# zenithfang/supervised_dispnet

Measured on AMD Instinct MI355X. Metric: images/sec fwd+bwd Disp_vgg_BN 128x416 b32 @1/2/4/8 GPU, higher is better.
Workload: dtype f32 (Winograd forward / input gradient / weight gradient form each f32 product from three exact bf16 pieces per operand on the bf16 matrix cores, six partial products, f32 accumulate; error vs fp64 at or below the f32 matrix instruction's)

## Files before the change

### include/dispnet_hip.h

```cpp
#ifndef DISPNET_HIP_H_
#define DISPNET_HIP_H_

#include <stddef.h>
#include <stdint.h>

#ifdef __cplusplus
extern "C" {
#endif

typedef void* dn_stream_t;

enum dn_status {
  DN_OK = 0,
  DN_ERR_BAD_ARG = -1,
  DN_ERR_UNSUPPORTED = -2,
  DN_ERR_WORKSPACE = -3,
  DN_ERR_LAUNCH = -4
};

void dn_reload_knobs(void);
int dn_version(void);
const char* dn_last_error(void);
const char* dn_last_kernel(void);
int dn_device_arch_ok(void);

#define DN_MAX_OPERANDS 3

enum dn_activation {
  DN_ACT_NONE = 0,
  DN_ACT_RELU = 1,
  DN_ACT_LEAKY = 2,
  DN_ACT_ELU = 3,
  DN_ACT_SIGMOID_AFFINE = 4
};

enum dn_conv_kind {
  DN_CONV_FWD = 0,
  DN_CONV_DGRAD = 1,
  DN_CONVT_FWD = 2,
  DN_CONVT_DGRAD = 3
};

typedef struct dn_operand {
  const float* data;
  int32_t C;
  int32_t up_shift;
  int64_t stride_n, stride_h, stride_w, stride_c;
  const float* scale;
  const float* shift;
} dn_operand;

typedef struct dn_result {
  float* data;
  int32_t C;
  int32_t accumulate;
  int64_t stride_n, stride_h, stride_w;
} dn_result;

typedef struct dn_conv_desc {
  int32_t kind;
  int32_t N;
  int32_t IH, IW;
  int32_t OH, OW;
  int32_t R, S, stride, pad;
  int32_t n_in;
  dn_operand in[DN_MAX_OPERANDS];
  int32_t n_out;
  dn_result out[DN_MAX_OPERANDS];
  const float* w_packed;
  const float* bias;
  int32_t act;
  float act_p0, act_p1;
  float* bn_partial;
  int32_t pad_mode;
  int32_t compute;
  int32_t dilation;
  const float* bnb_y;
  const float* bnb_scale;
  const float* bnb_shift;
  const float* bnb_mean;
  const float* bnb_invstd;
  float* bnb_partial;
  void* splitk_ws;
  int64_t splitk_ws_bytes;
  float* recip_out;
  const float* bnf_gamma;
  const float* bnf_beta;
  float* bnf_running_mean;
  float* bnf_running_var;
  int64_t* bnf_num_batches_tracked;
  float bnf_momentum, bnf_eps;
  float* bnf_mean;
  float* bnf_invstd;
  float* bnf_scale;
  float* bnf_shift;
  float* bnb_dgamma;
  float* bnb_dbeta;
} dn_conv_desc;

enum { DN_COMPUTE_DEFAULT = 0, DN_COMPUTE_BF16 = 1, DN_COMPUTE_F32X3 = 2, DN_COMPUTE_F32 = 3 };

int64_t dn_conv_packed_weight_elems(const dn_conv_desc* d);
int dn_conv_pack_weights(const dn_conv_desc* d, const float* w, float* w_packed, dn_stream_t stream);
int64_t dn_pack_entry_bytes(void);
int dn_pack_entry_fill(const dn_conv_desc* d, const float* w, float* w_packed, void* entry_host);
int dn_pack_many(const void* entries_dev, int32_t n_direct, int32_t n_wino, int32_t n_wino_bf16, int32_t n_wino_x3, dn_stream_t stream);
int32_t dn_conv_weight_layout(const dn_conv_desc* d);
int32_t dn_conv_bn_partial_rows(const dn_conv_desc* d);
int64_t dn_conv_splitk_workspace_bytes(const dn_conv_desc* d);
int32_t dn_conv_fwd_folds_bn_finalize(const dn_conv_desc* d);
int32_t dn_conv_dgrad_folds_bn_sums(const dn_conv_desc* d);
int32_t dn_conv_dgrad_fuses_bn_sums(const dn_conv_desc* d);
int32_t dn_conv_fwd_fuses_reciprocal(const dn_conv_desc* d);
int dn_conv2d_fwd(const dn_conv_desc* d, dn_stream_t stream);
int dn_conv2d_dgrad(const dn_conv_desc* d, dn_stream_t stream);
int dn_convT2d_fwd(const dn_conv_desc* d, dn_stream_t stream);
int dn_convT2d_dgrad(const dn_conv_desc* d, dn_stream_t stream);

size_t dn_conv_wgrad_workspace_bytes(const dn_conv_desc* fwd);
int dn_conv2d_wgrad(const dn_conv_desc* fwd, const float* dy, float* dw, void* workspace, size_t workspace_bytes,
                    dn_stream_t stream);

int dn_bn_finalize(const float* partial, int32_t rows, int32_t C, int64_t count, const float* conv_bias,
                   const float* gamma, const float* beta, float* running_mean, float* running_var, float momentum,
                   float eps, float* mean, float* invstd, float* scale, float* shift, int64_t* num_batches_tracked,
                   dn_stream_t stream);
int dn_bn_eval_affine(int32_t C, const float* gamma, const float* beta, const float* running_mean,
                      const float* running_var, float eps, float* scale, float* shift, dn_stream_t stream);
int dn_bn_relu_pool_fwd(const float* y, const float* scale, const float* shift, int32_t N, int32_t H, int32_t W,
                        int32_t C, float* pooled, uint8_t* idx, dn_stream_t stream);
int dn_bn_relu_pool_bwd(const float* dpooled, const uint8_t* idx, const float* y, const float* mean,
                        const float* invstd, int32_t N, int32_t H, int32_t W, int32_t C, float* dz, float* partial,
                        dn_stream_t stream);
int dn_maxpool2_bwd(const float* dpooled, const uint8_t* idx, int32_t N, int32_t H, int32_t W, int32_t C, float* dx, int32_t accumulate,
                    dn_stream_t stream);
int dn_bn_relu_bwd_reduce(float* da_dz, const float* y, const float* scale, const float* shift, const float* mean,
                          const float* invstd, int64_t rows, int32_t C, float* partial, dn_stream_t stream);
int dn_bn_bwd_apply(float* dz_dy, const float* y, const float* mean, const float* invstd, const float* gamma,
                    const float* partial, int32_t partial_rows, int32_t partial_stride, int32_t partial_offset, int64_t rows,
                    int32_t C, float* dgamma, float* dbeta, dn_stream_t stream);
int dn_bn_relu_bwd_sums(const float* da, const float* y, const float* scale, const float* shift, const float* mean, const float* invstd,
                        int64_t rows, int32_t C, float* partial, dn_stream_t stream);
int dn_bn_relu_pool_bwd_sums(const float* dpooled, const uint8_t* idx, const float* y, const float* mean, const float* invstd, int32_t N,
                             int32_t H, int32_t W, int32_t C, float* partial, dn_stream_t stream);
int dn_bn_bwd_apply_relu(float* da_dy, const float* y, const float* scale, const float* shift, const float* mean, const float* invstd,
                         const float* gamma, const float* partial, int32_t partial_rows, int32_t partial_stride, int32_t partial_offset,
                         int64_t rows, int32_t C, float* dgamma, float* dbeta, dn_stream_t stream);
int dn_bn_bwd_apply_pool(const float* dpooled, const uint8_t* idx, const float* y, const float* mean, const float* invstd, const float* gamma,
                         const float* partial, int32_t partial_rows, int32_t partial_stride, int32_t partial_offset, int32_t N, int32_t H,
                         int32_t W, int32_t C, float* dy, float* dgamma, float* dbeta, dn_stream_t stream);
int32_t dn_reduce_blocks(int64_t rows, int32_t C);

int dn_act_bwd_reduce_from(const float* g_in, float* g_out, const float* y_post, int32_t act, float p0, float p1, int64_t rows, int32_t C,
                           float* partial, dn_stream_t stream);
int dn_act_bwd_reduce(float* g, const float* y_post, int32_t act, float p0, float p1, int64_t rows, int32_t C,
                      float* partial, dn_stream_t stream);
int dn_colsum_finalize(const float* partial, int32_t rows, int32_t C, int32_t stride, int32_t offset, float* out,
                       dn_stream_t stream);
int dn_upsample2x_nearest_bwd(const float* dfull, int32_t N, int32_t h, int32_t w, float* dlow, int32_t accumulate,
                              dn_stream_t stream);
int dn_upsample2x_nearest_bwd_nhwc(const float* dfull, int32_t N, int32_t h, int32_t w, int32_t C, float* dlow, int32_t accumulate,
                                   dn_stream_t stream);
int dn_reflect_fold(const float* dxp, int32_t N, int32_t H, int32_t W, int32_t C, int32_t pad, float* dx, int32_t accumulate,
                    dn_stream_t stream);
int dn_bn_add_relu_fwd(const float* y, const float* scale, const float* shift, const float* r, const float* r_scale, const float* r_shift,
                       int64_t rows, int32_t C, float* out, dn_stream_t stream);
int dn_bn_add_relu_bwd(const float* gout, const float* out, const float* y, const float* mean, const float* invstd, const float* r,
                       const float* r_mean, const float* r_invstd, int64_t rows, int32_t C, float* dz_y, float* dr, int32_t dr_accumulate,
                       float* partial, dn_stream_t stream);
int32_t dn_maxpool3s2_out(int32_t H, int32_t ceil_mode);
int dn_maxpool3s2_fwd(const float* x, int32_t N, int32_t H, int32_t W, int32_t C, int32_t ceil_mode, float* out, uint8_t* idx, dn_stream_t stream);
int dn_maxpool3s2_bwd(const float* dout, const uint8_t* idx, int32_t N, int32_t H, int32_t W, int32_t C, int32_t ceil_mode, float* dx,
                      int32_t accumulate, dn_stream_t stream);
int dn_sub_div(const float* x, int64_t n, float sub, float div, float* out, dn_stream_t stream);
int dn_upsample2x_bilinear_fwd(const float* low, int32_t N, int32_t h, int32_t w, int32_t OH, int32_t OW, float* out,
                               dn_stream_t stream);
int dn_upsample2x_bilinear_bwd(const float* dout, int32_t N, int32_t h, int32_t w, int32_t OH, int32_t OW, float* dlow,
                               int32_t accumulate, dn_stream_t stream);
int32_t dn_bn_stats_rows(int64_t rows);
int dn_bn_stats_partial(const float* x, int64_t rows, int32_t C, float* partial, dn_stream_t stream);
int dn_bn_apply_fwd(const float* y, const float* scale, const float* shift, int64_t rows, int32_t C, float* out, dn_stream_t stream);
int dn_phase_bias_add(float* x, int32_t N, int32_t H2, int32_t W2, int32_t C, const float* bias4, dn_stream_t stream);
size_t dn_phase_colsum_workspace_bytes(int32_t C);
int dn_phase_colsum(const float* g, int32_t N, int32_t H, int32_t W, int32_t C, float* workspace, float* out4, dn_stream_t stream);
int dn_act_fwd(const float* x, int64_t n, int32_t act, float p0, float p1, float* out, dn_stream_t stream);
int dn_resize_bilinear_fwd(const float* in, int32_t N, int32_t IH, int32_t IW, int32_t OH, int32_t OW, int32_t align_corners, float* out,
                           dn_stream_t stream);
int dn_resize_bilinear_bwd(const float* dout, int32_t N, int32_t IH, int32_t IW, int32_t OH, int32_t OW, int32_t align_corners, float* din,
                           int32_t accumulate, dn_stream_t stream);
int dn_spatial_mean_fwd(const float* x, int32_t N, int64_t HW, int32_t C, float scale, float* out, dn_stream_t stream);
int dn_spatial_mean_bwd(const float* dout, int32_t N, int64_t HW, int32_t C, float scale, float* dx, dn_stream_t stream);
int dn_reciprocal_fwd(const float* x, float* y, int64_t n, dn_stream_t stream);
int dn_reciprocal_bwd(const float* dy, const float* y, float* dx, int64_t n, dn_stream_t stream);

enum dn_masked_loss_kind { DN_LOSS_L1 = 0, DN_LOSS_L2 = 1, DN_LOSS_BERHU = 2, DN_LOSS_SCALE_INV = 3 };
#define DN_LOSS_STATS 8
size_t dn_masked_loss_workspace_bytes(int32_t G, int64_t pixels);
int dn_masked_loss_fwd(const float* gt, const float* pred, int32_t G, int64_t pixels, float max_depth, int32_t kind, float weight,
                       int32_t accumulate, float* stats, void* workspace, size_t workspace_bytes, float* loss, dn_stream_t stream);
int dn_masked_loss_fwd_fused(const float* gt, const float* pred, int32_t G, int64_t pixels, float max_depth, int32_t kind, float weight,
                             int32_t accumulate, float* stats, void* workspace, size_t workspace_bytes, float* loss, int32_t* counter,
                             dn_stream_t stream);
int dn_masked_loss_stats(const float* gt, const float* pred, int32_t G, int64_t pixels, float max_depth, int32_t kind, int32_t pass,
                         float* stats, void* workspace, size_t workspace_bytes, dn_stream_t stream);
int dn_masked_loss_finalize(float* stats, int32_t G, int32_t kind, float weight, int32_t accumulate, float* loss, dn_stream_t stream);
int dn_masked_loss_bwd(const float* gt, const float* pred, const float* stats, const float* dloss, int32_t G, int64_t pixels,
                       float max_depth, int32_t kind, float weight, float* dpred, dn_stream_t stream);
int dn_pyramid_down2(const float* in, int32_t N, int32_t H, int32_t W, int32_t mode, float* out, dn_stream_t stream);
int dn_upsample_int_fwd(const float* low, int32_t N, int32_t h, int32_t w, int32_t scale, int32_t mode, float* out, dn_stream_t stream);
int dn_upsample_int_bwd(const float* dout, int32_t N, int32_t h, int32_t w, int32_t scale, int32_t mode, float* dlow, dn_stream_t stream);
int32_t dn_reduce1d_blocks(int64_t n);
int dn_explainability_fwd(const float* mask, int64_t n, float weight, int32_t accumulate, float* partial, float* loss, dn_stream_t stream);
int dn_explainability_bwd(const float* mask, const float* dloss, int64_t n, float* dmask, dn_stream_t stream);
int32_t dn_smooth_blocks(int32_t B, int32_t H, int32_t W);
int dn_smooth2_fwd(const float* map, int32_t B, int32_t H, int32_t W, float weight, float* partial, float* loss,
                   dn_stream_t stream);
int dn_smooth2_bwd(const float* map, const float* dloss, int32_t B, int32_t H, int32_t W, float weight, float* dmap,
                   dn_stream_t stream);
int dn_compute_errors(const float* gt, const float* pred, int32_t B, int32_t H, int32_t W, float max_depth, int32_t y1,
                      int32_t y2, int32_t x1, int32_t x2, int32_t median_scaling, float* scratch, float* out8,
                      dn_stream_t stream);

int dn_pose_proj_fwd(const float* pose, int64_t pose_stride_b, const float* K, const float* Kinv, int32_t B, int32_t rotation_mode,
                     float downscale, float* proj, float* kinv_scaled, dn_stream_t stream);
int32_t dn_warp_blocks(int32_t h, int32_t w);
int dn_pose_proj_bwd(const float* pose, int64_t pose_stride_b, const float* K, int32_t B, int32_t rotation_mode, float downscale,
                     const float* dproj_partial, int32_t nblk, float* dpose, int64_t dpose_stride_b, int32_t accumulate,
                     dn_stream_t stream);
int dn_inverse_warp_fwd(const float* img, const float* depth, const float* proj, const float* kinv, int32_t B, int32_t h, int32_t w,
                        int32_t padding_mode, int32_t align_corners, float* warped, dn_stream_t stream);
// ... 108 lines not shown
```

### supervised_dispnet_amd/_lib.py

```python
import ctypes as C
import os
import pathlib

_PKG = pathlib.Path(__file__).resolve().parent
LIB_PATH = pathlib.Path(os.environ.get("DISPNET_HIP_LIB", _PKG / "libdispnet_hip.so"))

EXPECTED_ABI = 21

DN_MAX_OPERANDS = 3
ACT_NONE, ACT_RELU, ACT_LEAKY, ACT_ELU, ACT_SIGMOID_AFFINE = 0, 1, 2, 3, 4
COMPUTE_DEFAULT, COMPUTE_BF16, COMPUTE_F32X3, COMPUTE_F32 = 0, 1, 2, 3
CONV_FWD, CONV_DGRAD, CONVT_FWD, CONVT_DGRAD = 0, 1, 2, 3
LOSS_L1, LOSS_L2, LOSS_BERHU, LOSS_SCALE_INV = 0, 1, 2, 3
LOSS_STATS = 8

_f32p = C.c_void_p


class Operand(C.Structure):
    _fields_ = [("data", _f32p), ("C", C.c_int32), ("up_shift", C.c_int32),
                ("stride_n", C.c_int64), ("stride_h", C.c_int64), ("stride_w", C.c_int64), ("stride_c", C.c_int64),
                ("scale", _f32p), ("shift", _f32p)]


class Result(C.Structure):
    _fields_ = [("data", _f32p), ("C", C.c_int32), ("accumulate", C.c_int32),
                ("stride_n", C.c_int64), ("stride_h", C.c_int64), ("stride_w", C.c_int64)]


class ConvDesc(C.Structure):
    _fields_ = [("kind", C.c_int32), ("N", C.c_int32), ("IH", C.c_int32), ("IW", C.c_int32), ("OH", C.c_int32),
                ("OW", C.c_int32), ("R", C.c_int32), ("S", C.c_int32), ("stride", C.c_int32), ("pad", C.c_int32),
                ("n_in", C.c_int32), ("in_", Operand * DN_MAX_OPERANDS),
                ("n_out", C.c_int32), ("out", Result * DN_MAX_OPERANDS),
                ("w_packed", _f32p), ("bias", _f32p), ("act", C.c_int32), ("act_p0", C.c_float), ("act_p1", C.c_float),
                ("bn_partial", _f32p), ("pad_mode", C.c_int32), ("compute", C.c_int32), ("dilation", C.c_int32),
                ("bnb_y", _f32p), ("bnb_scale", _f32p), ("bnb_shift", _f32p), ("bnb_mean", _f32p), ("bnb_invstd", _f32p), ("bnb_partial", _f32p),
                ("splitk_ws", _f32p), ("splitk_ws_bytes", C.c_int64), ("recip_out", _f32p),
                ("bnf_gamma", _f32p), ("bnf_beta", _f32p), ("bnf_running_mean", _f32p), ("bnf_running_var", _f32p),
                ("bnf_num_batches_tracked", C.c_void_p), ("bnf_momentum", C.c_float), ("bnf_eps", C.c_float),
                ("bnf_mean", _f32p), ("bnf_invstd", _f32p), ("bnf_scale", _f32p), ("bnf_shift", _f32p),
                ("bnb_dgamma", _f32p), ("bnb_dbeta", _f32p)]


_P = C.POINTER
_i32, _i64, _f, _d, _vp, _sz = C.c_int32, C.c_int64, C.c_float, C.c_double, C.c_void_p, C.c_size_t

SIGNATURES = {
    "dn_version": (C.c_int, []),
    "dn_reload_knobs": (None, []),
    "dn_last_error": (C.c_char_p, []),
    "dn_last_kernel": (C.c_char_p, []),
    "dn_device_arch_ok": (C.c_int, []),
    "dn_conv_packed_weight_elems": (_i64, [_P(ConvDesc)]),
    "dn_conv_pack_weights": (C.c_int, [_P(ConvDesc), _vp, _vp, _vp]),
    "dn_pack_entry_bytes": (_i64, []),
    "dn_pack_entry_fill": (C.c_int, [_P(ConvDesc), _vp, _vp, _vp]),
    "dn_pack_many": (C.c_int, [_vp, _i32, _i32, _i32, _i32, _vp]),
    "dn_conv_weight_layout": (_i32, [_P(ConvDesc)]),
    "dn_conv_bn_partial_rows": (_i32, [_P(ConvDesc)]),
    "dn_conv_dgrad_fuses_bn_sums": (_i32, [_P(ConvDesc)]),
    "dn_conv_fwd_fuses_reciprocal": (_i32, [_P(ConvDesc)]),
    "dn_conv_splitk_workspace_bytes": (_i64, [_P(ConvDesc)]),
    "dn_conv_fwd_folds_bn_finalize": (_i32, [_P(ConvDesc)]),
    "dn_conv_dgrad_folds_bn_sums": (_i32, [_P(ConvDesc)]),
    "dn_conv2d_fwd": (C.c_int, [_P(ConvDesc), _vp]),
    "dn_conv2d_dgrad": (C.c_int, [_P(ConvDesc), _vp]),
    "dn_convT2d_fwd": (C.c_int, [_P(ConvDesc), _vp]),
    "dn_convT2d_dgrad": (C.c_int, [_P(ConvDesc), _vp]),
    "dn_conv_wgrad_workspace_bytes": (_sz, [_P(ConvDesc)]),
    "dn_conv2d_wgrad": (C.c_int, [_P(ConvDesc), _vp, _vp, _vp, _sz, _vp]),
    "dn_bn_finalize": (C.c_int, [_vp, _i32, _i32, _i64, _vp, _vp, _vp, _vp, _vp, _f, _f, _vp, _vp, _vp, _vp, _vp, _vp]),
    "dn_bn_eval_affine": (C.c_int, [_i32, _vp, _vp, _vp, _vp, _f, _vp, _vp, _vp]),
    "dn_bn_relu_pool_fwd": (C.c_int, [_vp, _vp, _vp, _i32, _i32, _i32, _i32, _vp, _vp, _vp]),
    "dn_bn_relu_bwd_sums": (C.c_int, [_vp, _vp, _vp, _vp, _vp, _vp, _i64, _i32, _vp, _vp]),
    "dn_bn_relu_pool_bwd_sums": (C.c_int, [_vp, _vp, _vp, _vp, _vp, _i32, _i32, _i32, _i32, _vp, _vp]),
    "dn_bn_bwd_apply_relu": (C.c_int, [_vp, _vp, _vp, _vp, _vp, _vp, _vp, _vp, _i32, _i32, _i32, _i64, _i32, _vp, _vp, _vp]),
    "dn_bn_bwd_apply_pool": (C.c_int, [_vp, _vp, _vp, _vp, _vp, _vp, _vp, _i32, _i32, _i32, _i32, _i32, _i32, _i32, _vp, _vp, _vp, _vp]),
    "dn_maxpool2_bwd": (C.c_int, [_vp, _vp, _i32, _i32, _i32, _i32, _vp, _i32, _vp]),
    "dn_bn_relu_pool_bwd": (C.c_int, [_vp, _vp, _vp, _vp, _vp, _i32, _i32, _i32, _i32, _vp, _vp, _vp]),
    "dn_bn_relu_bwd_reduce": (C.c_int, [_vp, _vp, _vp, _vp, _vp, _vp, _i64, _i32, _vp, _vp]),
    "dn_bn_bwd_apply": (C.c_int, [_vp, _vp, _vp, _vp, _vp, _vp, _i32, _i32, _i32, _i64, _i32, _vp, _vp, _vp]),
    "dn_reduce_blocks": (_i32, [_i64, _i32]),
    "dn_act_bwd_reduce": (C.c_int, [_vp, _vp, _i32, _f, _f, _i64, _i32, _vp, _vp]),
    "dn_act_bwd_reduce_from": (C.c_int, [_vp, _vp, _vp, _i32, _f, _f, _i64, _i32, _vp, _vp]),
    "dn_colsum_finalize": (C.c_int, [_vp, _i32, _i32, _i32, _i32, _vp, _vp]),
    "dn_upsample2x_nearest_bwd": (C.c_int, [_vp, _i32, _i32, _i32, _vp, _i32, _vp]),
    "dn_upsample2x_nearest_bwd_nhwc": (C.c_int, [_vp, _i32, _i32, _i32, _i32, _vp, _i32, _vp]),
    "dn_reflect_fold": (C.c_int, [_vp, _i32, _i32, _i32, _i32, _i32, _vp, _i32, _vp]),
    "dn_bn_add_relu_fwd": (C.c_int, [_vp, _vp, _vp, _vp, _vp, _vp, _i64, _i32, _vp, _vp]),
    "dn_bn_add_relu_bwd": (C.c_int, [_vp, _vp, _vp, _vp, _vp, _vp, _vp, _vp, _i64, _i32, _vp, _vp, _i32, _vp, _vp]),
    "dn_maxpool3s2_out": (_i32, [_i32, _i32]),
    "dn_maxpool3s2_fwd": (C.c_int, [_vp, _i32, _i32, _i32, _i32, _i32, _vp, _vp, _vp]),
    "dn_maxpool3s2_bwd": (C.c_int, [_vp, _vp, _i32, _i32, _i32, _i32, _i32, _vp, _i32, _vp]),
    "dn_bn_stats_rows": (_i32, [_i64]),
    "dn_bn_stats_partial": (C.c_int, [_vp, _i64, _i32, _vp, _vp]),
    "dn_bn_apply_fwd": (C.c_int, [_vp, _vp, _vp, _i64, _i32, _vp, _vp]),
    "dn_act_fwd": (C.c_int, [_vp, _i64, _i32, _f, _f, _vp, _vp]),
    "dn_phase_bias_add": (C.c_int, [_vp, _i32, _i32, _i32, _i32, _vp, _vp]),
    "dn_phase_colsum_workspace_bytes": (_sz, [_i32]),
    "dn_phase_colsum": (C.c_int, [_vp, _i32, _i32, _i32, _i32, _vp, _vp, _vp]),
    "dn_resize_bilinear_fwd": (C.c_int, [_vp, _i32, _i32, _i32, _i32, _i32, _i32, _vp, _vp]),
    "dn_resize_bilinear_bwd": (C.c_int, [_vp, _i32, _i32, _i32, _i32, _i32, _i32, _vp, _i32, _vp]),
    "dn_sub_div": (C.c_int, [_vp, _i64, _f, _f, _vp, _vp]),
    "dn_spatial_mean_fwd": (C.c_int, [_vp, _i32, _i64, _i32, _f, _vp, _vp]),
    "dn_spatial_mean_bwd": (C.c_int, [_vp, _i32, _i64, _i32, _f, _vp, _vp]),
    "dn_upsample2x_bilinear_fwd": (C.c_int, [_vp, _i32, _i32, _i32, _i32, _i32, _vp, _vp]),
    "dn_upsample2x_bilinear_bwd": (C.c_int, [_vp, _i32, _i32, _i32, _i32, _i32, _vp, _i32, _vp]),
    "dn_reciprocal_fwd": (C.c_int, [_vp, _vp, _i64, _vp]),
    "dn_reciprocal_bwd": (C.c_int, [_vp, _vp, _vp, _i64, _vp]),
    "dn_masked_loss_workspace_bytes": (_sz, [_i32, _i64]),
    "dn_masked_loss_fwd": (C.c_int, [_vp, _vp, _i32, _i64, _f, _i32, _f, _i32, _vp, _vp, _sz, _vp, _vp]),
    "dn_masked_loss_fwd_fused": (C.c_int, [_vp, _vp, _i32, _i64, _f, _i32, _f, _i32, _vp, _vp, _sz, _vp, _vp, _vp]),
    "dn_masked_loss_stats": (C.c_int, [_vp, _vp, _i32, _i64, _f, _i32, _i32, _vp, _vp, _sz, _vp]),
    "dn_masked_loss_finalize": (C.c_int, [_vp, _i32, _i32, _f, _i32, _vp, _vp]),
    "dn_masked_loss_bwd": (C.c_int, [_vp, _vp, _vp, _vp, _i32, _i64, _f, _i32, _f, _vp, _vp]),
    "dn_pyramid_down2": (C.c_int, [_vp, _i32, _i32, _i32, _i32, _vp, _vp]),
    "dn_upsample_int_fwd": (C.c_int, [_vp, _i32, _i32, _i32, _i32, _i32, _vp, _vp]),
    "dn_upsample_int_bwd": (C.c_int, [_vp, _i32, _i32, _i32, _i32, _i32, _vp, _vp]),
    "dn_reduce1d_blocks": (_i32, [_i64]),
    "dn_explainability_fwd": (C.c_int, [_vp, _i64, _f, _i32, _vp, _vp, _vp]),
    "dn_explainability_bwd": (C.c_int, [_vp, _vp, _i64, _vp, _vp]),
    "dn_smooth_blocks": (_i32, [_i32, _i32, _i32]),
    "dn_smooth2_fwd": (C.c_int, [_vp, _i32, _i32, _i32, _f, _vp, _vp, _vp]),
    "dn_smooth2_bwd": (C.c_int, [_vp, _vp, _i32, _i32, _i32, _f, _vp, _vp]),
    "dn_compute_errors": (C.c_int, [_vp, _vp, _i32, _i32, _i32, _f, _i32, _i32, _i32, _i32, _i32, _vp, _vp, _vp]),
    "dn_pose_proj_fwd": (C.c_int, [_vp, _i64, _vp, _vp, _i32, _i32, _f, _vp, _vp, _vp]),
    "dn_warp_blocks": (_i32, [_i32, _i32]),
    "dn_pose_proj_bwd": (C.c_int, [_vp, _i64, _vp, _i32, _i32, _f, _vp, _i32, _vp, _i64, _i32, _vp]),
    "dn_inverse_warp_fwd": (C.c_int, [_vp, _vp, _vp, _vp, _i32, _i32, _i32, _i32, _i32, _vp, _vp]),
    "dn_inverse_warp_bwd": (C.c_int, [_vp, _vp, _vp, _vp, _i32, _i32, _i32, _i32, _i32, _vp, _vp, _i32, _vp, _vp]),
    "dn_photometric_fwd": (C.c_int, [_vp, _vp, _vp, _vp, _vp, _vp, _i64, _i32, _i32, _i32, _i32, _i32, _f, _i32, _vp, _vp, _vp]),
    "dn_photometric_bwd": (C.c_int, [_vp, _vp, _vp, _vp, _vp, _vp, _i64, _i32, _i32, _i32, _i32, _i32, _f, _vp, _vp, _i32, _vp, _vp,
                                     _i64, _vp]),
    "dn_area_down": (C.c_int, [_vp, _i64, _i32, _i32, _i32, _vp, _vp]),
    "dn_ssim_fwd": (C.c_int, [_vp, _vp, _i64, _i32, _i32, _vp, _vp]),
    "dn_ssim_bwd": (C.c_int, [_vp, _vp, _vp, _i64, _i32, _i32, _vp, _vp, _vp, _vp]),
    "dn_edge_smooth_blocks": (_i32, [_i32, _i32, _i32]),
    "dn_edge_smooth_fwd": (C.c_int, [_vp, _vp, _i32, _i32, _i32, _i32, _vp, _vp, _vp]),
    "dn_edge_smooth_bwd": (C.c_int, [_vp, _vp, _vp, _i32, _i32, _i32, _i32, _vp, _vp]),
    "dn_ordinal_fwd": (C.c_int, [_vp, _i64, _i64, _i64, _i32, _i64, _i32, _vp, _vp, _vp]),
    "dn_ordinal_bwd": (C.c_int, [_vp, _i64, _i64, _i64, _vp, _vp, _i32, _i64, _i32, _vp, _vp]),
    "dn_ordinal_loss_blocks": (_i32, [_i32, _i64]),
    "dn_ordinal_loss_fwd": (C.c_int, [_vp, _vp, _vp, _i32, _i64, _i32, _f, _vp, _vp, _vp, _vp]),
    "dn_ordinal_loss_finalize": (C.c_int, [_vp, _vp, _vp]),
    "dn_ordinal_loss_bwd": (C.c_int, [_vp, _vp, _vp, _vp, _vp, _i32, _i64, _i32, _f, _f, _vp, _vp]),
    "dn_ord_head_supported": (_i32, [_i32, _i64, _i32]),
    "dn_ord_head_bwd_blocks": (_i32, [_i32, _i64]),
    "dn_ord_head_fwd": (C.c_int, [_vp, _vp, _vp, _vp, _i32, _i64, _i32, _vp, _vp, _vp]),
    "dn_ord_head_bwd": (C.c_int, [_vp, _vp, _vp, _vp, _vp, _i32, _i64, _i32, _vp, _i32, _vp, _vp, _vp, _vp]),
    "dn_sid_labels": (C.c_int, [_vp, _i64, _f, _f, _vp, _vp]),
    "dn_sid_depth": (C.c_int, [_vp, _i64, _f, _f, _vp, _vp]),
    "dn_channel_scale": (C.c_int, [_vp, _vp, _i32, _i64, _i32, _vp, _vp]),
    "dn_adam_step": (C.c_int, [_vp, _vp, _vp, _vp, _i64, _d, _d, _d, _d, _d, _i32, _d, _vp]),
    "dn_adam_step_dev": (C.c_int, [_vp, _vp, _vp, _vp, _i64, _vp, _d, _d, _vp, _vp, _d, _vp]),
    "dn_adam_tick": (C.c_int, [_vp, _vp, _vp, _vp]),
    "dn_fill": (C.c_int, [_vp, _f, _i64, _vp]),
    "dn_copy": (C.c_int, [_vp, _vp, _i64, _vp]),
    "dn_tape_begin": (_vp, []),
    "dn_tape_end": (C.c_int, [_vp]),
# ... 89 lines not shown
```

### supervised_dispnet_amd/csrc/dn_conv.hip

```cpp
#include <stdlib.h>

#include "dn_internal.h"

namespace dn {

template <auto Launch> static int plan_only(const dn_conv_desc*, IgemmParams& p, hipStream_t s) { return Launch(p, s); }
template <auto Launch> static int with_desc(const dn_conv_desc* d, IgemmParams& p, hipStream_t s) { return Launch(d, p, s); }
static bool heads_off() { return knobs().no_direct; }
constexpr auto x3_upper = conv_x3_splitk_workspace_upper_bytes;
static const ConvFamily kConvFamilies[] = {
    {"head_fwd", head_fwd_eligible, heads_off, plan_only<launch_head_fwd>, nullptr, x3_upper, head_fwd_fuses_reciprocal},
    {"head_dgrad", head_dgrad_eligible, heads_off, plan_only<launch_head_dgrad>, nullptr, x3_upper},
    {"winograd", wino_eligible, nullptr, plan_only<launch_wino_conv>, wino_layout,
     [](const IgemmParams& p) { return wino_layout(p) == 3 ? wino_splitk_workspace_bytes(p) : (size_t)0; }, nullptr,
     [](const dn_conv_desc* d) {
       const dn_result& r = d->out[0];
       return d->kind == DN_CONV_DGRAD && d->n_out == 1 && !r.accumulate && (r.C & 3) == 0 && r.stride_w == r.C &&
              r.stride_h == (int64_t)d->OW * r.C && r.stride_n == (int64_t)d->OH * d->OW * r.C && d->bias == nullptr && d->act == DN_ACT_NONE;
     },
     [](IgemmParams& p) { wino_prepare(p); return wino_folds_bn_finalize(p); }, [](IgemmParams& p) { wino_prepare(p); return wino_folds_bn_sums(p); }},
    {"stem3", stem3_conv_eligible, nullptr, plan_only<launch_stem3_conv>, nullptr, x3_upper},
    {"stemk", stemk_conv_eligible, nullptr, with_desc<launch_stemk_conv>, nullptr, x3_upper},
    {"stem", stem_eligible, nullptr, plan_only<launch_stem>, nullptr, x3_upper},
    {"lds3", lds3_conv_eligible, nullptr, with_desc<launch_lds3_conv>, nullptr, x3_upper},
// ... 8 lines not shown
  return f;
}

static int run_conv(const dn_conv_desc* d, int expect_kind, dn_stream_t stream) {
  DN_REQUIRE(d != nullptr && d->kind == expect_kind, DN_ERR_BAD_ARG, "descriptor kind mismatch (want %d)", expect_kind);
  IgemmParams p;
  int rc = build_plan(d, false, &p);
  if (rc != DN_OK) return rc;
  DN_REQUIRE(p.w != nullptr, DN_ERR_BAD_ARG, "w_packed is null");
  for (int i = 0; i < p.n_in; ++i) DN_REQUIRE(p.in[i].p != nullptr, DN_ERR_BAD_ARG, "operand %d has no data", i);
  for (int i = 0; i < p.n_out; ++i) {
    const dn_result& o = d->out[i];
    DN_REQUIRE(o.stride_h == (int64_t)d->OW * o.stride_w && o.stride_n == (int64_t)d->OH * o.stride_h, DN_ERR_UNSUPPORTED,
               "result %d must be pixel-dense (NHWC with a channel stride)", i);
  }
  return conv_route(d, p)->launch(d, p, as_stream(stream));
}

}

using namespace dn;

static bool wgrad_split_plans(const dn_conv_desc* fwd, dn_conv_desc* d1, dn_conv_desc* d2, IgemmParams* p1, IgemmParams* p2, size_t* w1,
                              size_t* w2) {
  if (fwd->kind != DN_CONV_FWD || fwd->n_in < 2 || fwd->in[fwd->n_in - 1].C != 1) return false;
  *d1 = *fwd;
  d1->n_in = fwd->n_in - 1;
  *d2 = *fwd;
  d2->n_in = 1;
  d2->in[0] = fwd->in[fwd->n_in - 1];
  if (build_plan(d1, true, p1) != DN_OK || build_plan(d2, true, p2) != DN_OK) return false;
  int cin_total = 0;
  for (int i = 0; i < fwd->n_in; ++i) cin_total += fwd->in[i].C;
  if (wino_wgrad_eligible(d1, *p1)) {
    p1->dw_cin_total = cin_total;
    *w1 = (wino_wgrad_workspace_bytes(*p1) + 255) / 256 * 256;
  } else {
    return false;
  }
  p2->in[0].ch_off = cin_total - 1;
  p2->D1 = cin_total;
  choose_splits(p2);
  *w2 = generic_wgrad_workspace_bytes(*p2);
  return true;
}

static int tap_windows(const IgemmParams& p) {
  const int nt = p.ph[0].ntaps;
  if (nt <= 32 || p.reflect || p.nphases != 1 || knobs().no_tap_windows) return 1;
  return (nt + 31) / 32;
}

static void tap_window_plan(const IgemmParams& full, int w, int nw, IgemmParams* q) {
  *q = full;
  const int nt = full.ph[0].ntaps, per = (nt + nw - 1) / nw;
  const int t0 = w * per, t1 = t0 + per < nt ? t0 + per : nt;
  for (int t = t0; t < t1; ++t) {
    q->tdy[t - t0] = full.tdy[full.ph[0].tap0 + t];
    q->tdx[t - t0] = full.tdx[full.ph[0].tap0 + t];
    q->tr[t - t0] = full.tr[full.ph[0].tap0 + t];
    q->ts[t - t0] = full.ts[full.ph[0].tap0 + t];
  }
  q->ph[0].tap0 = 0;
  q->ph[0].ntaps = t1 - t0;
  int nch = 0;
  for (int i = 0; i < q->n_in; ++i) nch += (q->ph[0].ntaps * q->in[i].C + kChunk - 1) / kChunk;
  q->ph[0].nchunks = nch;
  q->uni32 = 1;
  q->wg_uniform = 1;
  for (int i = 0; i < q->n_in; ++i) {
    const KOperand& o = q->in[i];
    if (!o.small) q->uni32 = 0;
    if (!o.small || (!o.vec && o.scale != nullptr) || o.C >= 32768) q->wg_uniform = 0;
  }
}

struct WgradFamily {
  const char* name;
  bool (*eligible)(const dn_conv_desc* fwd, const IgemmParams& p);
  size_t (*workspace_bytes)(const dn_conv_desc* fwd, const IgemmParams& p);
  bool dy_aligned16;
  bool (*switched_off)();
  int (*launch)(const dn_conv_desc* fwd, IgemmParams& p, float* dw, hipStream_t s);
};
static const WgradFamily kWgradFamilies[] = {
    {"head", head_wgrad_eligible, [](const dn_conv_desc*, const IgemmParams& p) { return head_wgrad_workspace_bytes(p); }, false,
     [] { return knobs().no_direct; },
     [](const dn_conv_desc*, IgemmParams& p, float* dw, hipStream_t s) { return launch_head_wgrad(p, dw, p.ws, s); }},
    {"winograd", wino_wgrad_eligible, [](const dn_conv_desc*, const IgemmParams& p) { return wino_wgrad_workspace_bytes(p); }, false, nullptr,
     [](const dn_conv_desc*, IgemmParams& p, float* dw, hipStream_t s) { return launch_wino_wgrad(p, dw, s); }},
    {"lds3", lds3_wgrad_eligible, [](const dn_conv_desc*, const IgemmParams& p) { return lds3_wgrad_workspace_bytes(p); }, true, nullptr,
     launch_lds3_wgrad},
    {"lds3k", lds3k_wgrad_eligible, [](const dn_conv_desc*, const IgemmParams& p) { return lds3k_wgrad_workspace_bytes(p); }, true, nullptr,
     launch_lds3k_wgrad},
    {"stemk", stemk_wgrad_eligible, stemk_wgrad_workspace_bytes, true, nullptr, launch_stemk_wgrad},
    {"thin", thin_wgrad_eligible, [](const dn_conv_desc*, const IgemmParams& p) { return thin_wgrad_workspace_bytes(p); }, false, nullptr,
     [](const dn_conv_desc*, IgemmParams& p, float* dw, hipStream_t s) { return launch_thin_wgrad(p, dw, s); }},
};

extern "C" {

int64_t dn_pack_entry_bytes(void) { return (int64_t)sizeof(PackEntry); }

int dn_pack_entry_fill(const dn_conv_desc* d, const float* w, float* w_packed, void* entry_host) {
  DN_REQUIRE(d && w && w_packed && entry_host, DN_ERR_BAD_ARG, "dn_pack_entry_fill: null pointer");
  PackEntry* e = reinterpret_cast<PackEntry*>(entry_host);
  int rc = build_plan(d, false, &e->p);
  if (rc != DN_OK) return rc;
  e->w = w;
  e->wp = w_packed;
  const ConvFamily* f = conv_route(d, e->p);
  e->wino = f->weight_layout ? f->weight_layout(e->p) : 0;
  if (e->wino) {
    e->total = wino_packed_elems(e->p);
    e->NS = ((e->p.Ntot + 63) / 64 * 64) / 32;
  } else {
    e->total = direct_packed_elems(e->p);
    e->NS = 0;
  }
  return e->wino;
}

int dn_pack_many(const void* entries_dev, int32_t n_direct, int32_t n_wino, int32_t n_wino16, int32_t n_wino_x3, dn_stream_t stream) {
  DN_REQUIRE(entries_dev && n_direct >= 0 && n_wino >= 0 && n_wino16 >= 0 && n_wino_x3 >= 0, DN_ERR_BAD_ARG, "dn_pack_many: bad argument");
  const PackEntry* tab = reinterpret_cast<const PackEntry*>(entries_dev);
  hipStream_t s = as_stream(stream);
  if (n_direct > 0) {
    int rc = launch_direct_pack_many(tab, n_direct, s);
    if (rc != DN_OK) return rc;
  }
  if (n_wino > 0) {
    int rc = launch_wino_pack_many(tab, n_direct, n_wino, s);
    if (rc != DN_OK) return rc;
  }
  if (n_wino16 > 0) {
    int rc = launch_wino_pack16_many(tab, n_direct + n_wino, n_wino16, 1, s);
    if (rc != DN_OK) return rc;
  }
  if (n_wino_x3 > 0) return launch_wino_pack16_many(tab, n_direct + n_wino + n_wino16, n_wino_x3, 3, s);
  return DN_OK;
}

int dn_conv_pack_weights(const dn_conv_desc* d, const float* w, float* w_packed, dn_stream_t stream) {
  IgemmParams p;
  int rc = build_plan(d, false, &p);
  if (rc != DN_OK) return rc;
  DN_REQUIRE(w != nullptr && w_packed != nullptr, DN_ERR_BAD_ARG, "null weight pointer");
  const ConvFamily* f = conv_route(d, p);
  if (const int wl = f->weight_layout ? f->weight_layout(p) : 0)
    return wl == 1 ? launch_wino_pack(p, w, w_packed, as_stream(stream)) : launch_wino_pack16(p, w, w_packed, wl == 3 ? 3 : 1, as_stream(stream));
  return launch_direct_pack(p, w, w_packed, as_stream(stream));
}

int dn_conv2d_fwd(const dn_conv_desc* d, dn_stream_t stream) { return run_conv(d, DN_CONV_FWD, stream); }
int dn_conv2d_dgrad(const dn_conv_desc* d, dn_stream_t stream) { return run_conv(d, DN_CONV_DGRAD, stream); }
int dn_convT2d_fwd(const dn_conv_desc* d, dn_stream_t stream) { return run_conv(d, DN_CONVT_FWD, stream); }
int dn_convT2d_dgrad(const dn_conv_desc* d, dn_stream_t stream) { return run_conv(d, DN_CONVT_DGRAD, stream); }

size_t dn_conv_wgrad_workspace_bytes(const dn_conv_desc* fwd) {
  IgemmParams p;
  if (build_plan(fwd, true, &p) != DN_OK) return 0;
  choose_splits(&p);
  size_t need = generic_wgrad_workspace_bytes(p);
  for (const WgradFamily& f : kWgradFamilies)
    if (f.eligible(fwd, p) && f.workspace_bytes(fwd, p) > need) need = f.workspace_bytes(fwd, p);
  {
    dn_conv_desc d1, d2;
    IgemmParams p1, p2;
    size_t w1 = 0, w2 = 0;
    if (wgrad_split_plans(fwd, &d1, &d2, &p1, &p2, &w1, &w2) && w1 + w2 > need) need = w1 + w2;
  }
  const int nw = tap_windows(p);
  for (int w = 0; w < nw && nw > 1; ++w) {
    IgemmParams q;
    tap_window_plan(p, w, nw, &q);
    choose_splits(&q);
    if (generic_wgrad_workspace_bytes(q) > need) need = generic_wgrad_workspace_bytes(q);
  }
  return need;
}

int dn_conv2d_wgrad(const dn_conv_desc* fwd, const float* dy, float* dw, void* workspace, size_t workspace_bytes,
                    dn_stream_t stream) {
  IgemmParams p;
  int rc = build_plan(fwd, true, &p);
  if (rc != DN_OK) return rc;
  DN_REQUIRE(dy != nullptr && dw != nullptr && workspace != nullptr, DN_ERR_BAD_ARG, "null pointer");
  const hipStream_t s = as_stream(stream);
  for (const WgradFamily& f : kWgradFamilies) {
    if (!f.eligible(fwd, p) || (f.switched_off && f.switched_off()) || workspace_bytes < f.workspace_bytes(fwd, p)) continue;
    if (f.dy_aligned16 && (reinterpret_cast<uintptr_t>(dy) & 15) != 0) continue;
    for (int i = 0; i < p.n_in; ++i) DN_REQUIRE(p.in[i].p != nullptr, DN_ERR_BAD_ARG, "operand %d has no data", i);
    p.g = dy;
    p.ws = reinterpret_cast<float*>(workspace);
    return f.launch(fwd, p, dw, s);
  }
  {
    dn_conv_desc d1, d2;
    IgemmParams p1, p2;
    size_t w1 = 0, w2 = 0;
    if (wgrad_split_plans(fwd, &d1, &d2, &p1, &p2, &w1, &w2) && workspace_bytes >= w1 + w2) {
      for (int i = 0; i < fwd->n_in; ++i) DN_REQUIRE(fwd->in[i].data != nullptr, DN_ERR_BAD_ARG, "operand %d has no data", i);
      if (wino_wgrad_eligible(&d1, p1)) {
        p1.g = dy;
        p1.ws = reinterpret_cast<float*>(workspace);
        rc = launch_wino_wgrad(p1, dw, s);
      } else {
        rc = generic_wgrad(&d1, p1, dy, dw, workspace, w1, s);
      }
      if (rc != DN_OK) return rc;
      return generic_wgrad(&d2, p2, dy, dw, reinterpret_cast<char*>(workspace) + w1, w2, s);
    }
  }
  if (const int nw = tap_windows(p); nw > 1 && fwd->kind == DN_CONV_FWD) {
    for (int w = 0; w < nw; ++w) {
      IgemmParams q;
      tap_window_plan(p, w, nw, &q);
      rc = generic_wgrad(fwd, q, dy, dw, workspace, workspace_bytes, s);
      if (rc != DN_OK) return rc;
    }
    return DN_OK;
  }
  return generic_wgrad(fwd, p, dy, dw, workspace, workspace_bytes, s);
}

}
```

### supervised_dispnet_amd/csrc/dn_internal.h

```cpp
#pragma once
#include <hip/hip_runtime.h>
#include <hip/hip_ext.h>
#include <stdint.h>
#include <stdio.h>

#include <atomic>
#include <functional>
#include <tuple>
#include <type_traits>

#include "dispnet_hip.h"

namespace dn {

void set_error(const char* fmt, ...);
void set_last_kernel(const char* fmt, ...);
int check_launch(const char* what);

static inline hipStream_t as_stream(dn_stream_t s) { return reinterpret_cast<hipStream_t>(s); }

struct LaunchTape;
extern std::atomic<LaunchTape*> g_tape_rec;
void tape_push(LaunchTape* t, std::function<void(hipEvent_t)>&& op, const void* kernel, hipStream_t stream);

template <typename... KArgs, typename... Args>
static inline void launch(void (*kernel)(KArgs...), dim3 grid, dim3 block, size_t lds, hipStream_t stream, Args... args) {
  kernel<<<grid, block, lds, stream>>>(args...);
  if (LaunchTape* t = g_tape_rec.load(std::memory_order_relaxed)) {
    std::tuple<std::decay_t<KArgs>...> held(args...);
    tape_push(t, [=](hipEvent_t stop) mutable {
      if (stop == nullptr) {
        std::apply([&](auto&... a) { kernel<<<grid, block, lds, stream>>>(a...); }, held);
      } else {
        std::apply([&](auto&... a) {
          void* argv[] = {static_cast<void*>(&a)...};
          if (hipExtLaunchKernel(reinterpret_cast<const void*>(kernel), grid, block, argv, lds, stream, nullptr, stop, 0) != hipSuccess) {
            (void)hipGetLastError();
            kernel<<<grid, block, lds, stream>>>(a...);
            (void)hipEventRecord(stop, stream);
          }
        }, held);
      }
    }, reinterpret_cast<const void*>(kernel), stream);
  }
}
#define DN_LAUNCH(...) ::dn::launch(__VA_ARGS__)

struct Knobs {
  bool no_winograd, no_winograd_wgrad;
  bool no_direct;
  bool no_thin, no_thin_conv;
  bool no_lds3;
  bool no_wino_splitk, no_x3_splitk, no_wino8_tail;
  bool no_x3_direct, no_x3_wgrad;
  bool no_tap_windows;
  int wino_wgw;
  int wino_min_tiles;
  int wino_splitk_target, wino_splitk_maxblocks;
  int pack_blocks;
  bool no_riding_fences;
  int wino_nmajor;
  int wino_wg_target;
  int wino8;
};
const Knobs& knobs();

inline int norm_compute(int c) {
  return c == DN_COMPUTE_BF16 ? DN_COMPUTE_BF16 : ((c == DN_COMPUTE_F32X3 || c == DN_COMPUTE_DEFAULT) ? DN_COMPUTE_F32X3 : DN_COMPUTE_F32);
}

#define DN_REQUIRE(cond, code, ...)      \
  do {                                   \
    if (!(cond)) {                       \
      ::dn::set_error(__VA_ARGS__);      \
      return (code);                     \
    }                                    \
  } while (0)

constexpr int kMaxTaps = 64;
constexpr int kMaxPhases = 4;
constexpr int kChunk = 32;

struct KOperand {
  const float* p;
  const float* scale;
  const float* shift;
  long long sn, sh, sw, sc;
  int C;
  int up;
  int vec;
  int ch_off;
  unsigned mC;
  int small;
};

struct KResult {
  float* p;
  long long sn, sh, sw;
  int C;
  int n_begin;
  int accumulate;
  int linear;
};

struct KPhase {
  int ntaps;
  int tap0;
  int ooy, oox;
  int nchunks;
  long long w_off;
};

struct BnFinalizeArgs {
  const float* conv_bias;
  const float* gamma;
  const float* beta;
  float* running_mean;
  float* running_var;
  long long* num_batches_tracked;
  float momentum, eps;
  float* mean;
  float* invstd;
  float* scale;
  float* shift;
};

struct IgemmParams {
  KOperand in[DN_MAX_OPERANDS];
  KResult out[DN_MAX_OPERANDS];
  KPhase ph[kMaxPhases];
  int8_t tdy[kMaxTaps], tdx[kMaxTaps], tr[kMaxTaps], ts[kMaxTaps];
  int n_in, n_out, nphases;
  int N, GH, GW, M;
  int sy, sx;
  int osy, osx;
  int IH, IW, OH, OW;
  int Ntot, Npad;
  int BN;
// ... 31 lines not shown
  int* fold_cnt;
  int fold_bn, fold_bnb;
  int nmajor;
};

static inline unsigned fastdiv_magic(unsigned d) { return d <= 1 ? 0xFFFFFFFFu : (unsigned)(0x100000000ull / d); }

int build_plan(const dn_conv_desc* d, bool for_wgrad, IgemmParams* p);

inline long long direct_packed_elems(const IgemmParams& p) {
  const KPhase& last = p.ph[p.nphases - 1];
  return last.w_off + (long long)p.Npad * last.nchunks * kChunk;
}

struct PackEntry {
  IgemmParams p;
  const float* w;
  float* wp;
  long long total;
  int wino;
  int NS;
};
int launch_wino_pack_many(const PackEntry* tab_dev, int first, int n, hipStream_t stream);
int launch_wino_pack16_many(const PackEntry* tab_dev, int first, int n, int pieces, hipStream_t stream);
int launch_wino_pack16(const IgemmParams& p, const float* w, float* wp, int pieces, hipStream_t stream);
long long wino_packed_floats(const IgemmParams& p, int layout);
int wino_layout(const IgemmParams& p);

struct ConvFamily {
  const char* name;
  bool (*eligible)(const dn_conv_desc* d, const IgemmParams& p);
  bool (*switched_off)();
  int (*launch)(const dn_conv_desc* d, IgemmParams& p, hipStream_t s);
  int (*weight_layout)(const IgemmParams& p);
  size_t (*splitk_workspace_bytes)(const IgemmParams& p);
  bool (*fuses_reciprocal)(const IgemmParams& p);
  bool (*takes_bn_sums)(const dn_conv_desc* d);
  bool (*folds_bn_finalize)(IgemmParams& p);
  bool (*folds_bn_sums)(IgemmParams& p);
};
const ConvFamily* conv_route(const dn_conv_desc* d, const IgemmParams& p);

bool stem_eligible(const dn_conv_desc* d, const IgemmParams& p);
int launch_stem(const IgemmParams& p, hipStream_t stream);
int launch_tiled_conv(const IgemmParams& p, hipStream_t stream);
void choose_splits(IgemmParams* p);
size_t generic_wgrad_workspace_bytes(const IgemmParams& p);
int generic_wgrad(const dn_conv_desc* fwd, IgemmParams& p, const float* dy, float* dw, void* workspace, size_t workspace_bytes, hipStream_t s);
int launch_direct_pack(const IgemmParams& p, const float* w, float* wp, hipStream_t stream);
int launch_direct_pack_many(const PackEntry* tab_dev, int n, hipStream_t stream);

bool head_fwd_eligible(const dn_conv_desc* d, const IgemmParams& p);
int launch_head_fwd(const IgemmParams& p, hipStream_t stream);
bool head_fwd_fuses_reciprocal(const IgemmParams& p);
bool head_dgrad_eligible(const dn_conv_desc* d, const IgemmParams& p);
int launch_head_dgrad(const IgemmParams& p, hipStream_t stream);
bool head_wgrad_eligible(const dn_conv_desc* fwd, const IgemmParams& p);
size_t head_wgrad_workspace_bytes(const IgemmParams& p);
int launch_head_wgrad(const IgemmParams& p, float* dw, float* workspace, hipStream_t stream);

bool wino_eligible(const dn_conv_desc* d, const IgemmParams& p);
long long wino_packed_elems(const IgemmParams& p);
int launch_wino_pack(const IgemmParams& p, const float* w, float* wp, hipStream_t stream);
int launch_wino_conv(IgemmParams& p, hipStream_t stream);
void wino_prepare(IgemmParams& p);
bool wino_folds_bn_finalize(const IgemmParams& p);
bool wino_folds_bn_sums(const IgemmParams& p);
int wino_splitk_choice(const IgemmParams& p);
size_t conv_x3_splitk_workspace_upper_bytes(const IgemmParams& p);
size_t wino_splitk_workspace_bytes(const IgemmParams& p);
bool wino_wgrad_eligible(const dn_conv_desc* fwd, const IgemmParams& p);
size_t wino_wgrad_workspace_bytes(const IgemmParams& p);
int launch_wino_wgrad(IgemmParams& p, float* dw, hipStream_t stream);

bool thin_wgrad_eligible(const dn_conv_desc* fwd, const IgemmParams& p);
size_t thin_wgrad_workspace_bytes(const IgemmParams& p);
int launch_thin_wgrad(IgemmParams& p, float* dw, hipStream_t stream);
bool thin_conv_eligible(const dn_conv_desc* d, const IgemmParams& p);
int launch_thin_conv(const IgemmParams& p, hipStream_t stream);

bool lds3_conv_eligible(const dn_conv_desc* d, const IgemmParams& p);
int launch_lds3_conv(const dn_conv_desc* d, const IgemmParams& p, hipStream_t stream);
bool lds3_wgrad_eligible(const dn_conv_desc* fwd, const IgemmParams& p);
size_t lds3_wgrad_workspace_bytes(const IgemmParams& p);
int launch_lds3_wgrad(const dn_conv_desc* fwd, IgemmParams& p, float* dw, hipStream_t stream);
bool lds3k_wgrad_eligible(const dn_conv_desc* fwd, const IgemmParams& p);
size_t lds3k_wgrad_workspace_bytes(const IgemmParams& p);
int launch_lds3k_wgrad(const dn_conv_desc* fwd, IgemmParams& p, float* dw, hipStream_t stream);
int launch_wgrad_reduce(const IgemmParams& p, float* dw, hipStream_t stream);
bool wgrad_x3_eligible(const IgemmParams& p);
int launch_wgrad_x3(const IgemmParams& p, hipStream_t stream);
bool lds3k_conv_eligible(const dn_conv_desc* d, const IgemmParams& p);
int launch_lds3k_conv(const dn_conv_desc* d, const IgemmParams& p, hipStream_t stream);
bool stem3_conv_eligible(const dn_conv_desc* d, const IgemmParams& p);
bool stemk_conv_eligible(const dn_conv_desc* d, const IgemmParams& p);
int launch_stemk_conv(const dn_conv_desc* d, const IgemmParams& p, hipStream_t stream);
bool stemk_wgrad_eligible(const dn_conv_desc* d, const IgemmParams& p);
size_t stemk_wgrad_workspace_bytes(const dn_conv_desc* d, const IgemmParams& p);
int launch_stemk_wgrad(const dn_conv_desc* d, IgemmParams& p, float* dw, hipStream_t stream);
int launch_stem3_conv(const IgemmParams& p, hipStream_t stream);

}
```

### supervised_dispnet_amd/csrc/dn_lds3_wgrad.hip

```cpp
#include <stdlib.h>

#include "dn_device.h"

namespace dn {

struct WgGeo {
  int tilesX, tilesY, ntiles, per_xcd;
  long long slab;
};

constexpr int WG_TH = 8, WG_TW = 32;
constexpr int WG_GSTR = 528;
constexpr int WG_GPIECE = 16 * WG_GSTR;
constexpr int WG_XROWB = 96;
constexpr int WG_XSTR = 10 * WG_XROWB + 16;
constexpr int WG_XPIECE = 16 * WG_XSTR;
constexpr int WG_DCOLS = 36;
constexpr int WG16_LDS = 3 * WG_GPIECE + 3 * WG_XPIECE + 10 * WG_DCOLS * 4;

template <bool HAS1>
__global__ void __launch_bounds__(256, 2) lds3_wgrad16_kernel(const IgemmParams p, const WgGeo geo) {
  extern __shared__ __align__(16) char lds[];
  char* Gp = lds;
  char* Xp = lds + 3 * WG_GPIECE;
  float* Dp = reinterpret_cast<float*>(lds + 3 * WG_GPIECE + 3 * WG_XPIECE);
  constexpr int NT = HAS1 ? 10 : 9;
  const int tid = threadIdx.x, lane = tid & 63, wave = tid >> 6;
  const int j = lane & 15, g = lane >> 4;
  const KOperand& S = p.in[0];
  const __amdgpu_buffer_rsrc_t rg = __builtin_amdgcn_make_buffer_rsrc(const_cast<float*>(p.g), 0, 0x80000000u, 0x00020000);
  const __amdgpu_buffer_rsrc_t rx = __builtin_amdgcn_make_buffer_rsrc(const_cast<float*>(S.p), 0, 0x80000000u, 0x00020000);
  __amdgpu_buffer_rsrc_t r1 = rx;
  if constexpr (HAS1) r1 = __builtin_amdgcn_make_buffer_rsrc(const_cast<float*>(p.in[1].p), 0, 0x80000000u, 0x00020000);

  f32x4 acc[NT];
#pragma unroll
  for (int t = 0; t < NT; ++t) acc[t] = f32x4{0.f, 0.f, 0.f, 0.f};
  const int dtap = j < 9 ? j : 0;
  const int doff = (dtap / 3) * WG_DCOLS + (dtap % 3);

  f32x4 vg[8], vx[8];
  float dv[2] = {0.f, 0.f};
  auto issue_loads = [&](int t) __attribute__((always_inline)) {
    const int txb = t % geo.tilesX, q1 = t / geo.tilesX;
    const int tyb = q1 % geo.tilesY, n = q1 / geo.tilesY;
    const int gy0 = tyb * WG_TH, gx0 = txb * WG_TW;
    {
      const int cq = tid & 3, pxg = tid >> 2, row = pxg >> 2, cgp = pxg & 3;
      const int gy = gy0 + row;
#pragma unroll
      for (int i = 0; i < 8; ++i) {
        const int gx = gx0 + 8 * cgp + i;
        const bool ok = tid < 128 && gy < p.GH && gx < p.GW;
        const int off = (((n * p.GH + gy) * p.GW + gx) * p.Ntot + 4 * cq) * 4;
        vg[i] = __builtin_bit_cast(f32x4, __builtin_amdgcn_raw_buffer_load_b128(rg, ok ? off : -1, 0, 0));
      }
    }
    {
      const int cq = tid & 3, grp = tid >> 2, row = grp / 6, cgp = grp - row * 6;
      const int iy = gy0 - 1 + row;
#pragma unroll
      for (int i = 0; i < 8; ++i) {
        const int ix = gx0 + 8 * cgp - 8 + i;
        const bool need = cgp == 0 ? i == 7 : (cgp == 5 ? i == 0 : true);
        const bool ok = tid < 240 && need && (unsigned)iy < (unsigned)p.IH && (unsigned)ix < (unsigned)p.IW;
        const int off = (n * (int)S.sn + iy * (int)S.sh + ix * (int)S.sw + 4 * cq) * 4;
        vx[i] = __builtin_bit_cast(f32x4, __builtin_amdgcn_raw_buffer_load_b128(rx, ok ? off : -1, 0, 0));
      }
    }
    if constexpr (HAS1) {
      const KOperand& S1 = p.in[1];
#pragma unroll
      for (int r = 0; r < 2; ++r) {
        const int it = tid + 256 * r;
        const int row = it / 34, col = it - row * 34;
        const int iy = gy0 - 1 + row, ix = gx0 - 1 + col;
        const bool ok = it < 340 && (unsigned)iy < (unsigned)p.IH && (unsigned)ix < (unsigned)p.IW;
        const int off = (n * (int)S1.sn + (iy >> S1.up) * (int)S1.sh + (ix >> S1.up) * (int)S1.sw) * 4;
        dv[r] = __builtin_bit_cast(float, __builtin_amdgcn_raw_buffer_load_b32(r1, ok ? off : -1, 0, 0));
      }
    }
  };
  auto store_lds = [&]() __attribute__((always_inline)) {
    if (tid < 128) {
      const int cq = tid & 3, pxg = tid >> 2;
// ... 29 lines not shown
        if (it < 340) Dp[row * WG_DCOLS + col] = dv[r];
      }
    }
  };

  const int xcd = (int)blockIdx.x & 7, local = (int)blockIdx.x >> 3, nlocal = (int)gridDim.x >> 3;
  const int band_lo = xcd * geo.per_xcd, band_hi = min(band_lo + geo.per_xcd, geo.ntiles);
  constexpr int AS[6] = {0, 0, 1, 0, 1, 2}, BS[6] = {2, 1, 1, 0, 0, 0};
  if (band_lo + local < band_hi) issue_loads(band_lo + local);
  for (int t = band_lo + local; t < band_hi; t += nlocal) {
    store_lds();
    __syncthreads();
    if (t + nlocal < band_hi) issue_loads(t + nlocal);
#pragma unroll 1
    for (int rr = 0; rr < 2; ++rr) {
      const int r = 2 * wave + rr;
      bf16x8 a[3];
#pragma unroll
      for (int P = 0; P < 3; ++P) a[P] = *reinterpret_cast<const bf16x8*>(Gp + P * WG_GPIECE + j * WG_GSTR + (r * 32 + 8 * g) * 2);
#pragma unroll
      for (int ty = 0; ty < 3; ++ty) {
        const char* rowb = Xp + j * WG_XSTR + (r + ty) * WG_XROWB + (8 * g + 8) * 2;
        u32x4 c[3];
        unsigned lf[3], rt[3];
#pragma unroll
        for (int P = 0; P < 3; ++P) {
          c[P] = *reinterpret_cast<const u32x4*>(rowb + P * WG_XPIECE);
          lf[P] = *reinterpret_cast<const unsigned*>(rowb + P * WG_XPIECE - 4);
          rt[P] = *reinterpret_cast<const unsigned*>(rowb + P * WG_XPIECE + 16);
        }
        bf16x8 bm[3], bz[3], bp[3];
#pragma unroll
        for (int P = 0; P < 3; ++P) {
          const u32x4 m4 = u32x4{__builtin_amdgcn_alignbit(c[P][0], lf[P], 16), __builtin_amdgcn_alignbit(c[P][1], c[P][0], 16),
                                 __builtin_amdgcn_alignbit(c[P][2], c[P][1], 16), __builtin_amdgcn_alignbit(c[P][3], c[P][2], 16)};
          const u32x4 p4 = u32x4{__builtin_amdgcn_alignbit(c[P][1], c[P][0], 16), __builtin_amdgcn_alignbit(c[P][2], c[P][1], 16),
                                 __builtin_amdgcn_alignbit(c[P][3], c[P][2], 16), __builtin_amdgcn_alignbit(rt[P], c[P][3], 16)};
          bm[P] = __builtin_bit_cast(bf16x8, m4);
          bz[P] = __builtin_bit_cast(bf16x8, c[P]);
          bp[P] = __builtin_bit_cast(bf16x8, p4);
        }
#pragma unroll
        for (int q = 0; q < 6; ++q) {
          acc[3 * ty + 0] = __builtin_amdgcn_mfma_f32_16x16x32_bf16(a[AS[q]], bm[BS[q]], acc[3 * ty + 0], 0, 0, 0);
          acc[3 * ty + 1] = __builtin_amdgcn_mfma_f32_16x16x32_bf16(a[AS[q]], bz[BS[q]], acc[3 * ty + 1], 0, 0, 0);
          acc[3 * ty + 2] = __builtin_amdgcn_mfma_f32_16x16x32_bf16(a[AS[q]], bp[BS[q]], acc[3 * ty + 2], 0, 0, 0);
        }
      }
      if constexpr (HAS1) {
        float v[8];
#pragma unroll
        for (int e = 0; e < 8; ++e) {
          const float x = Dp[r * WG_DCOLS + 8 * g + e + doff];
          v[e] = j < 9 ? x : 0.f;
        }
        bf16x8 b[3];
        split3(v, b[0], b[1], b[2]);
#pragma unroll
        for (int q = 0; q < 6; ++q) acc[9] = __builtin_amdgcn_mfma_f32_16x16x32_bf16(a[AS[q]], b[BS[q]], acc[9], 0, 0, 0);
      }
    }
    __syncthreads();
  }

  f32x4* red = reinterpret_cast<f32x4*>(lds);
#pragma unroll
  for (int t = 0; t < NT; ++t) red[(wave * NT + t) * 64 + lane] = acc[t];
  __syncthreads();
  const int Kp = p.ph[0].nchunks * kChunk;
  const int kbase1 = ((9 * 16 + kChunk - 1) / kChunk) * kChunk;
  float* slab = p.ws + (long long)blockIdx.x * geo.slab;
  for (int it = tid; it < NT * 64; it += 256) {
    const int t = it >> 6, l = it & 63;
    const f32x4 s = (red[(0 * NT + t) * 64 + l] + red[(1 * NT + t) * 64 + l]) + (red[(2 * NT + t) * 64 + l] + red[(3 * NT + t) * 64 + l]);
    const int jj = l & 15, gg = l >> 4;
    const int k = t < 9 ? t * 16 + jj : kbase1 + jj;
    if (t < 9 || jj < 9) {
#pragma unroll
      for (int e = 0; e < 4; ++e) slab[(long long)(4 * gg + e) * Kp + k] = s[e];
    }
  }
}

constexpr int WS_GSTR = 272;
constexpr int WS_GPIECE = 64 * WS_GSTR;
constexpr int WS_ICOLS = 36;
constexpr int WS_IPLANE = 10 * WS_ICOLS;
constexpr int WGS_LDS = 3 * WS_GPIECE + 3 * WS_IPLANE * 4;

__global__ void __launch_bounds__(256, 2) lds3_wgrad_stem_kernel(const IgemmParams p, const WgGeo geo) {
  extern __shared__ __align__(16) char lds[];
  char* Gp = lds;
  float* Ip = reinterpret_cast<float*>(lds + 3 * WS_GPIECE);
  const int tid = threadIdx.x, lane = tid & 63, wave = tid >> 6;
  const int j = lane & 15, g = lane >> 4;
  const KOperand& S = p.in[0];
  const int C = S.C, K = 9 * C;
  const __amdgpu_buffer_rsrc_t rg = __builtin_amdgcn_make_buffer_rsrc(const_cast<float*>(p.g), 0, 0x80000000u, 0x00020000);
  const __amdgpu_buffer_rsrc_t rx = __builtin_amdgcn_make_buffer_rsrc(const_cast<float*>(S.p), 0, 0x80000000u, 0x00020000);

  f32x4 acc[4][2];
#pragma unroll
  for (int m = 0; m < 4; ++m)
#pragma unroll
    for (int nt = 0; nt < 2; ++nt) acc[m][nt] = f32x4{0.f, 0.f, 0.f, 0.f};
  int ioff[2];
  bool ilive[2];
#pragma unroll
  for (int nt = 0; nt < 2; ++nt) {
    const int col = 16 * nt + j;
    ilive[nt] = col < K;
    const int tap = ilive[nt] ? col / C : 0, ci = ilive[nt] ? col - tap * C : 0;
    ioff[nt] = ci * WS_IPLANE + (tap / 3) * WS_ICOLS + (tap % 3);
  }

  f32x4 vg[8];
  float vi[4];
  auto issue_g = [&](int t, int h) __attribute__((always_inline)) {
    const int txb = t % geo.tilesX, q1 = t / geo.tilesX;
    const int tyb = q1 % geo.tilesY, n = q1 / geo.tilesY;
    const int pxg = tid & 15, cq = tid >> 4, row = pxg >> 2, cgp = pxg & 3;
    const int gy = tyb * WG_TH + 4 * h + row;
#pragma unroll
    for (int i = 0; i < 8; ++i) {
      const int gx = txb * WG_TW + 8 * cgp + i;
      const bool ok = gy < p.GH && gx < p.GW;
      const int off = (((n * p.GH + gy) * p.GW + gx) * p.Ntot + 4 * cq) * 4;
      vg[i] = __builtin_bit_cast(f32x4, __builtin_amdgcn_raw_buffer_load_b128(rg, ok ? off : -1, 0, 0));
    }
  };
  auto issue_img = [&](int t) __attribute__((always_inline)) {
    const int txb = t % geo.tilesX, q1 = t / geo.tilesX;
    const int tyb = q1 % geo.tilesY, n = q1 / geo.tilesY;
#pragma unroll
    for (int r = 0; r < 4; ++r) {
      const int it = tid + 256 * r;
      const int c = it / 340, px = it - c * 340;
      const int row = px / 34, col = px - row * 34;
      const int iy = tyb * WG_TH - 1 + row, ix = txb * WG_TW - 1 + col;
      const bool ok = c < C && (unsigned)iy < (unsigned)p.IH && (unsigned)ix < (unsigned)p.IW;
      const int off = (n * (int)S.sn + iy * (int)S.sh + ix * (int)S.sw + c * (int)S.sc) * 4;
      vi[r] = __builtin_bit_cast(float, __builtin_amdgcn_raw_buffer_load_b32(rx, ok ? off : -1, 0, 0));
    }
  };
  auto store_g = [&]() __attribute__((always_inline)) {
    const int pxg = tid & 15, cq = tid >> 4;
#pragma unroll
    for (int e = 0; e < 4; ++e) {
      const float v[8] = {vg[0][e], vg[1][e], vg[2][e], vg[3][e], vg[4][e], vg[5][e], vg[6][e], vg[7][e]};
      bf16x8 h, m, l;
      split3(v, h, m, l);
      char* dst = Gp + (4 * cq + e) * WS_GSTR + pxg * 16;
      *reinterpret_cast<bf16x8*>(dst) = h;
      *reinterpret_cast<bf16x8*>(dst + WS_GPIECE) = m;
      *reinterpret_cast<bf16x8*>(dst + 2 * WS_GPIECE) = l;
    }
  };
  auto store_img = [&]() __attribute__((always_inline)) {
#pragma unroll
    for (int r = 0; r < 4; ++r) {
      const int it = tid + 256 * r;
      const int c = it / 340, px = it - c * 340;
      const int row = px / 34, col = px - row * 34;
      if (c < 3) Ip[c * WS_IPLANE + row * WS_ICOLS + col] = vi[r];
    }
  };

  const int xcd = (int)blockIdx.x & 7, local = (int)blockIdx.x >> 3, nlocal = (int)gridDim.x >> 3;
  const int band_lo = xcd * geo.per_xcd, band_hi = min(band_lo + geo.per_xcd, geo.ntiles);
  constexpr int AS[6] = {0, 0, 1, 0, 1, 2}, BS[6] = {2, 1, 1, 0, 0, 0};
  if (band_lo + local < band_hi) {
    issue_g(band_lo + local, 0);
    issue_img(band_lo + local);
  }
  for (int t = band_lo + local; t < band_hi; t += nlocal) {
#pragma unroll 1
    for (int h = 0; h < 2; ++h) {
      store_g();
      if (h == 0) store_img();
      __syncthreads();
      if (h == 0) issue_g(t, 1);
      else if (t + nlocal < band_hi) {
        issue_g(t + nlocal, 0);
        issue_img(t + nlocal);
      }
      const int r = 4 * h + wave;
      bf16x8 b[2][3];
#pragma unroll
      for (int nt = 0; nt < 2; ++nt) {
        float v[8];
#pragma unroll
        for (int e = 0; e < 8; ++e) {
          const float x = Ip[r * WS_ICOLS + 8 * g + e + ioff[nt]];
          v[e] = ilive[nt] ? x : 0.f;
        }
        split3(v, b[nt][0], b[nt][1], b[nt][2]);
      }
#pragma unroll
      for (int m = 0; m < 4; ++m) {
        bf16x8 a[3];
#pragma unroll
        for (int P = 0; P < 3; ++P) a[P] = *reinterpret_cast<const bf16x8*>(Gp + P * WS_GPIECE + (16 * m + j) * WS_GSTR + (wave * 32 + 8 * g) * 2);
#pragma unroll
        for (int q = 0; q < 6; ++q)
#pragma unroll
          for (int nt = 0; nt < 2; ++nt) acc[m][nt] = __builtin_amdgcn_mfma_f32_16x16x32_bf16(a[AS[q]], b[nt][BS[q]], acc[m][nt], 0, 0, 0);
      }
      __syncthreads();
    }
  }

  f32x4* red = reinterpret_cast<f32x4*>(lds);
#pragma unroll
  for (int m = 0; m < 4; ++m)
#pragma unroll
    for (int nt = 0; nt < 2; ++nt) red[((wave * 4 + m) * 2 + nt) * 64 + lane] = acc[m][nt];
  __syncthreads();
  const int Kp = p.ph[0].nchunks * kChunk;
  float* slab = p.ws + (long long)blockIdx.x * geo.slab;
  for (int it = tid; it < 8 * 64; it += 256) {
    const int mn = it >> 6, l = it & 63, m = mn >> 1, nt = mn & 1;
    const f32x4 s = (red[((0 * 4 + m) * 2 + nt) * 64 + l] + red[((1 * 4 + m) * 2 + nt) * 64 + l]) +
                    (red[((2 * 4 + m) * 2 + nt) * 64 + l] + red[((3 * 4 + m) * 2 + nt) * 64 + l]);
    const int jj = l & 15, gg = l >> 4, k = 16 * nt + jj;
    if (k < K) {
#pragma unroll
      for (int e = 0; e < 4; ++e) slab[(long long)(16 * m + 4 * gg + e) * Kp + k] = s[e];
    }
  }
}

static int lds3_wgrad_form(const dn_conv_desc* d, const IgemmParams& p) {
  if (knobs().no_lds3 || norm_compute(d->compute) != DN_COMPUTE_F32X3) return 0;
  if (d->kind != DN_CONV_FWD || d->R != 3 || d->S != 3 || d->stride != 1 || d->pad != 1 || d->pad_mode != 0 || d->dilation > 1) return 0;
  if (d->IH != d->OH || d->IW != d->OW) return 0;
  if ((long long)p.M * p.Ntot * 4 + 64 >= (1ll << 31) || (reinterpret_cast<uintptr_t>(p.g) & 15)) return 0;
  for (int t = 0; t < 9; ++t)
    if (p.tdy[t] != t / 3 - 1 || p.tdx[t] != t % 3 - 1) return 0;
  const KOperand& a = p.in[0];
  if (!a.small || a.scale != nullptr || a.up != 0) return 0;
  if (p.Ntot == 16 && a.C == 16 && a.vec) {
    if (p.n_in == 1) return 1;
    const KOperand& b = p.in[1];
    if (p.n_in == 2 && b.C == 1 && b.small && b.scale == nullptr) return 2;
    return 0;
  }
  if (p.Ntot == 64 && p.n_in == 1 && a.C >= 1 && a.C <= 3) return 3;
  return 0;
}

static int lds3_wgrad_blocks(const IgemmParams& p) {
  const int ntiles = p.N * ((p.GH + WG_TH - 1) / WG_TH) * ((p.GW + WG_TW - 1) / WG_TW);
  int blocks = ntiles < 512 ? ntiles : 512;
  return (blocks + 7) / 8 * 8;
}

bool lds3_wgrad_eligible(const dn_conv_desc* d, const IgemmParams& p) { return lds3_wgrad_form(d, p) != 0; }

size_t lds3_wgrad_workspace_bytes(const IgemmParams& p) {
  return (size_t)lds3_wgrad_blocks(p) * p.Npad * p.ph[0].nchunks * kChunk * sizeof(float);
}

int launch_lds3_wgrad(const dn_conv_desc* d, IgemmParams& p, float* dw, hipStream_t stream) {
  const int form = lds3_wgrad_form(d, p);
  WgGeo geo;
  geo.tilesX = (p.GW + WG_TW - 1) / WG_TW;
  geo.tilesY = (p.GH + WG_TH - 1) / WG_TH;
  geo.ntiles = p.N * geo.tilesX * geo.tilesY;
  geo.per_xcd = (geo.ntiles + 7) / 8;
  geo.slab = (long long)p.Npad * p.ph[0].nchunks * kChunk;
  const int blocks = lds3_wgrad_blocks(p);
  hipError_t e = hipSuccess;
  if (form == 3) {
    e = hipFuncSetAttribute(reinterpret_cast<const void*>(lds3_wgrad_stem_kernel), hipFuncAttributeMaxDynamicSharedMemorySize, WGS_LDS);
    if (e == hipSuccess) DN_LAUNCH(lds3_wgrad_stem_kernel, dim3(blocks), dim3(256), (size_t)WGS_LDS, stream, p, geo);
    set_last_kernel("dn::lds3_wgrad_stem_kernel");
  } else if (form == 2) {
    e = hipFuncSetAttribute(reinterpret_cast<const void*>(lds3_wgrad16_kernel<true>), hipFuncAttributeMaxDynamicSharedMemorySize, WG16_LDS);
    if (e == hipSuccess) DN_LAUNCH(lds3_wgrad16_kernel<true>, dim3(blocks), dim3(256), (size_t)WG16_LDS, stream, p, geo);
    set_last_kernel("dn::lds3_wgrad16_kernel<true>");
  } else if (form == 1) {
    e = hipFuncSetAttribute(reinterpret_cast<const void*>(lds3_wgrad16_kernel<false>), hipFuncAttributeMaxDynamicSharedMemorySize, WG16_LDS);
    if (e == hipSuccess) DN_LAUNCH(lds3_wgrad16_kernel<false>, dim3(blocks), dim3(256), (size_t)WG16_LDS, stream, p, geo);
    set_last_kernel("dn::lds3_wgrad16_kernel<false>");
  } else {
    set_error("launch_lds3_wgrad: no form");
    return DN_ERR_UNSUPPORTED;
  }
  if (e != hipSuccess) {
    set_error("lds3 wgrad: hipFuncSetAttribute: %s", hipGetErrorString(e));
    return DN_ERR_LAUNCH;
  }
  int rc = check_launch("lds3_wgrad_kernel");
  if (rc != DN_OK) return rc;
  p.splits = blocks;
  return launch_wgrad_reduce(p, dw, stream);
}

}

namespace dn {

constexpr int WK_TH = 2;
constexpr int WK_GSTR = WK_TH * 32 * 2 + 16;
constexpr int WK_GPIECE = 32 * WK_GSTR;
constexpr int WK_XROWS = WK_TH + 2;
constexpr int WK_XSTR = WK_XROWS * WG_XROWB + 16;
constexpr int WK_NCI = 96;
constexpr int WK_XPIECE = WK_NCI * WK_XSTR;
constexpr int WK_LDS = 3 * WK_GPIECE + 3 * WK_XPIECE + WK_XROWS * WG_DCOLS * 4;

template <bool HAS1>
__global__ void __launch_bounds__(512, 2) lds3k_wgrad_kernel(const IgemmParams p, const WgGeo geo, int c0) {
  extern __shared__ __align__(16) char lds[];
  char* Gp = lds;
  char* Xp = lds + 3 * WK_GPIECE;
  float* Dp = reinterpret_cast<float*>(lds + 3 * WK_GPIECE + 3 * WK_XPIECE);
  const int tid = threadIdx.x, lane = tid & 63, wave = tid >> 6;
  const int j = lane & 15, g = lane >> 4;
  const KOperand& S0 = p.in[0];
  const bool two = p.n_in - (HAS1 ? 1 : 0) == 2;
  const KOperand& S1 = p.in[two ? 1 : 0];
  const __amdgpu_buffer_rsrc_t rg = __builtin_amdgcn_make_buffer_rsrc(const_cast<float*>(p.g), 0, 0x80000000u, 0x00020000);
  const __amdgpu_buffer_rsrc_t r0 = __builtin_amdgcn_make_buffer_rsrc(const_cast<float*>(S0.p), 0, 0x80000000u, 0x00020000);
  const __amdgpu_buffer_rsrc_t r1 = __builtin_amdgcn_make_buffer_rsrc(const_cast<float*>(S1.p), 0, 0x80000000u, 0x00020000);
  const KOperand& SD = p.in[HAS1 ? p.n_in - 1 : 0];
  const __amdgpu_buffer_rsrc_t rd = __builtin_amdgcn_make_buffer_rsrc(const_cast<float*>(SD.p), 0, 0x80000000u, 0x00020000);

  const int nunits = wave < 2 ? 3 : 2;
  f32x4 acc[3][3][2];
#pragma unroll
  for (int u = 0; u < 3; ++u)
#pragma unroll
    for (int x = 0; x < 3; ++x)
#pragma unroll
      for (int m = 0; m < 2; ++m) acc[u][x][m] = f32x4{0.f, 0.f, 0.f, 0.f};
  f32x4 accd[2] = {f32x4{0.f, 0.f, 0.f, 0.f}, f32x4{0.f, 0.f, 0.f, 0.f}};
  const int dtap = j < 9 ? j : 0;
  const int doff = (dtap / 3) * WG_DCOLS + (dtap % 3);

  f32x4 va[8], vb[8];
  float dv = 0.f;
  const int nq0 = two ? c0 >> 2 : 24, n0jobs = 24 * nq0;
  auto decode = [&](int job, int& quad, int& rc, bool& second) __attribute__((always_inline)) {
    second = job >= n0jobs;
    const int jj = second ? job - n0jobs : job, nqh = (second ? 24 - nq0 : nq0) >> 2;
    const int rc_lo = jj & 3, q_lo = (jj >> 2) & 3, hi = jj >> 4;
    const int rc_hi = hi / nqh, q_hi = hi - rc_hi * nqh;
    rc = 4 * rc_hi + rc_lo;
    quad = (second ? nq0 : 0) + 4 * q_hi + q_lo;
  };
  int quadA, rcA, quadB, rcB;
  bool secA, secB;
  decode(tid, quadA, rcA, secA);
  decode(512 + (tid & 63), quadB, rcB, secB);
  const bool secAu = __builtin_amdgcn_readfirstlane((int)secA) != 0, secBu = __builtin_amdgcn_readfirstlane((int)secB) != 0;
  const int waveu = __builtin_amdgcn_readfirstlane(wave);
  const bool hasB = waveu == 2 || waveu == 3;
  const __amdgpu_buffer_rsrc_t rA = secAu ? r1 : r0;
// ... 284 lines not shown
```

### supervised_dispnet_amd/csrc/dn_plan.hip

```cpp
#include <stdarg.h>
#include <stdlib.h>
#include <string.h>

#include <atomic>
#include <mutex>

#include "dn_internal.h"

namespace dn {

static thread_local char g_err[512] = "";

void set_error(const char* fmt, ...) {
  va_list ap;
  va_start(ap, fmt);
  vsnprintf(g_err, sizeof(g_err), fmt, ap);
  va_end(ap);
}

static thread_local char g_kernel[160] = "";

void set_last_kernel(const char* fmt, ...) {
  va_list ap;
  va_start(ap, fmt);
  vsnprintf(g_kernel, sizeof(g_kernel), fmt, ap);
  va_end(ap);
}

int check_launch(const char* what) {
  hipError_t e = hipGetLastError();
  if (e != hipSuccess) {
    set_error("%s: %s", what, hipGetErrorString(e));
    return DN_ERR_LAUNCH;
  }
  return DN_OK;
}

static int pick_bn(int ntot) { return ntot <= 32 ? 32 : (ntot <= 64 ? 64 : 128); }

static int ceil_div(int a, int b) { return (a + b - 1) / b; }

static int floor_div(int a, int b) {
  int q = a / b, r = a % b;
  return (r != 0 && ((r < 0) != (b < 0))) ? q - 1 : q;
}

static void fill_operand(KOperand* k, const dn_operand* o, int ch_off) {
  k->p = o->data;
  k->scale = o->scale;
  k->shift = o->shift;
  k->sn = o->stride_n;
  k->sh = o->stride_h;
  k->sw = o->stride_w;
  k->sc = o->stride_c;
  k->C = o->C;
  k->up = o->up_shift;
  bool aligned = ((reinterpret_cast<uintptr_t>(o->data) & 15) == 0) && (o->stride_n % 4 == 0) &&
                 (o->stride_h % 4 == 0) && (o->stride_w % 4 == 0);
  k->vec = (o->C % 4 == 0 && o->stride_c == 1 && aligned) ? 1 : 0;
  k->ch_off = ch_off;
  k->mC = fastdiv_magic((unsigned)o->C);
}

static bool offsets_fit_int32(const KOperand& k, int N, int IH, int IW) {
  const long long hs = (IH >> k.up) + 1, ws = (IW >> k.up) + 1;
  const long long span = (long long)N * (k.sn < 0 ? -k.sn : k.sn) + hs * (k.sh < 0 ? -k.sh : k.sh) +
                         ws * (k.sw < 0 ? -k.sw : k.sw) + (long long)k.C * (k.sc < 0 ? -k.sc : k.sc);
  return span < (1ll << 31);
}

static Knobs g_knobs;
static std::atomic<int> g_knobs_state{0};
static std::mutex g_knobs_mu;

static void read_knobs(Knobs* k) {
  auto on = [](const char* n) { return getenv(n) != nullptr; };
  auto num = [](const char* n, int dflt) { const char* e = getenv(n); return e ? atoi(e) : dflt; };
  k->no_winograd = on("DN_NO_WINOGRAD");
  k->no_winograd_wgrad = on("DN_NO_WINOGRAD_WGRAD");
  k->no_direct = on("DN_NO_DIRECT");
  k->no_thin = on("DN_NO_THIN");
  k->no_thin_conv = on("DN_NO_THIN_CONV");
  k->wino_wgw = num("DN_WINO_WGW", 1);
  k->wino_min_tiles = num("DN_WINO_MIN_TILES", 192);
  k->no_x3_direct = on("DN_NO_X3_DIRECT");
  k->no_wino_splitk = on("DN_NO_WINO_SPLITK");
  k->wino_splitk_target = num("DN_WINO_SPLITK_TARGET", 512);
  k->wino_splitk_maxblocks = num("DN_WINO_SPLITK_MAXBLOCKS", 208);
  k->no_wino8_tail = on("DN_NO_WINO8_TAIL");
  k->no_x3_splitk = on("DN_NO_X3_SPLITK");
  k->pack_blocks = num("DN_PACK_BLOCKS", 512);
  if (k->pack_blocks < 1) k->pack_blocks = 1;
  k->no_lds3 = on("DN_NO_LDS3");
  k->no_x3_wgrad = on("DN_NO_X3_WGRAD");
  k->no_tap_windows = on("DN_NO_TAP_WINDOWS");
  k->wino_wg_target = num("DN_WINO_WG_TARGET", 0);
  k->wino_nmajor = num("DN_WINO_NMAJOR", 1);
  k->no_riding_fences = on("DN_NO_RIDING_FENCES");
  k->wino8 = num("DN_WINO8", -1);
}

const Knobs& knobs() {
  if (g_knobs_state.load(std::memory_order_acquire) == 0) {
    std::lock_guard<std::mutex> lock(g_knobs_mu);
    if (g_knobs_state.load(std::memory_order_relaxed) == 0) {
      read_knobs(&g_knobs);
      g_knobs_state.store(1, std::memory_order_release);
    }
  }
  return g_knobs;
}

int build_plan(const dn_conv_desc* d, bool for_wgrad, IgemmParams* p) {
  memset(p, 0, sizeof(*p));
  DN_REQUIRE(d != nullptr, DN_ERR_BAD_ARG, "null conv descriptor");
  DN_REQUIRE(d->kind >= DN_CONV_FWD && d->kind <= DN_CONVT_DGRAD, DN_ERR_BAD_ARG, "bad conv kind %d", d->kind);
  DN_REQUIRE(d->R >= 1 && d->S >= 1 && d->R * d->S <= 49, DN_ERR_UNSUPPORTED, "kernel %dx%d unsupported", d->R, d->S);
  DN_REQUIRE(d->stride >= 1 && d->stride <= 2, DN_ERR_UNSUPPORTED, "stride %d unsupported", d->stride);
  DN_REQUIRE(d->n_in >= 1 && d->n_in <= DN_MAX_OPERANDS, DN_ERR_BAD_ARG, "n_in %d", d->n_in);
  DN_REQUIRE(d->N > 0 && d->IH > 0 && d->IW > 0 && d->OH > 0 && d->OW > 0, DN_ERR_BAD_ARG, "bad sizes");
  int cin_total = 0;
  for (int i = 0; i < d->n_in; ++i) {
    DN_REQUIRE(d->in[i].C > 0 && (d->in[i].up_shift == 0 || d->in[i].up_shift == 1), DN_ERR_BAD_ARG, "operand %d", i);
    cin_total += d->in[i].C;
  }
  p->N = d->N;
  p->R = d->R;
  p->S = d->S;
  p->act = d->act;
  p->act_p0 = d->act_p0;
  p->act_p1 = d->act_p1;
  p->bias = d->bias;
  p->w = d->w_packed;
  p->bn_partial = d->bn_partial;
  if (d->kind == DN_CONV_DGRAD && !for_wgrad && d->bnb_y != nullptr && d->bnb_partial != nullptr) {
    DN_REQUIRE(d->bnb_scale && d->bnb_shift && d->bnb_mean && d->bnb_invstd, DN_ERR_BAD_ARG, "bnb_y needs scale / shift / mean / invstd");
    p->bnb_y = d->bnb_y;
    p->bnb_scale = d->bnb_scale;
    p->bnb_shift = d->bnb_shift;
    p->bnb_mean = d->bnb_mean;
    p->bnb_invstd = d->bnb_invstd;
    p->bnb_partial = d->bnb_partial;
  }
  if (!for_wgrad && d->kind == DN_CONV_FWD) p->recip_out = d->recip_out;
  if (!for_wgrad && d->splitk_ws != nullptr && d->splitk_ws_bytes > 0) {
    p->ks_ws = reinterpret_cast<float*>(d->splitk_ws);
    p->ks_ws_bytes = (size_t)d->splitk_ws_bytes;
    if (d->splitk_ws_bytes >= 8192 && (d->splitk_ws_bytes & 3) == 0) {
      p->ks_ws_bytes -= 256;
      p->fold_cnt = reinterpret_cast<int*>(reinterpret_cast<char*>(d->splitk_ws) + d->splitk_ws_bytes - 256);
    }
  }
  if (!for_wgrad && d->kind == DN_CONV_FWD && d->bn_partial != nullptr && d->bnf_scale != nullptr) {
    DN_REQUIRE(d->bnf_gamma && d->bnf_beta && d->bnf_mean && d->bnf_invstd && d->bnf_shift, DN_ERR_BAD_ARG,
               "bnf_scale needs gamma / beta / mean / invstd / shift");
    DN_REQUIRE((d->bnf_running_mean == nullptr) == (d->bnf_running_var == nullptr), DN_ERR_BAD_ARG, "bnf_running_mean and bnf_running_var go together");
    p->bnf.conv_bias = d->bias;
    p->bnf.gamma = d->bnf_gamma;
    p->bnf.beta = d->bnf_beta;
    p->bnf.running_mean = d->bnf_running_mean;
    p->bnf.running_var = d->bnf_running_var;
    p->bnf.num_batches_tracked = reinterpret_cast<long long*>(d->bnf_num_batches_tracked);
    p->bnf.momentum = d->bnf_momentum;
    p->bnf.eps = d->bnf_eps;
    p->bnf.mean = d->bnf_mean;
    p->bnf.invstd = d->bnf_invstd;
    p->bnf.scale = d->bnf_scale;
    p->bnf.shift = d->bnf_shift;
  }
  if (!for_wgrad && d->kind == DN_CONV_DGRAD && p->bnb_y != nullptr && d->bnb_dgamma != nullptr && d->bnb_dbeta != nullptr) {
    p->bnb_dgamma = d->bnb_dgamma;
    p->bnb_dbeta = d->bnb_dbeta;
  }
  const int st = d->stride, pad = d->pad;
  const int dil = d->dilation > 1 ? d->dilation : 1;
  DN_REQUIRE(d->pad_mode == 0 || d->pad_mode == 1, DN_ERR_BAD_ARG, "bad pad_mode %d", d->pad_mode);
  if (dil > 1) {
    DN_REQUIRE(st == 1 && d->pad_mode == 0 && (d->kind == DN_CONV_FWD || d->kind == DN_CONV_DGRAD), DN_ERR_UNSUPPORTED,
// ... 112 lines not shown
          ph.ooy = py;
          ph.oox = px;
          for (int r = 0; r < d->R; ++r) {
            if (((py + pad - r * dil) % st + st) % st != 0) continue;
            for (int s = 0; s < d->S; ++s) {
              if (((px + pad - s * dil) % st + st) % st != 0) continue;
              DN_REQUIRE(nt < kMaxTaps, DN_ERR_UNSUPPORTED, "too many taps");
              p->tdy[nt] = (int8_t)floor_div(py + pad - r * dil, st);
              p->tdx[nt] = (int8_t)floor_div(px + pad - s * dil, st);
              p->tr[nt] = (int8_t)r;
              p->ts[nt] = (int8_t)s;
              ++nt;
            }
          }
          ph.ntaps = nt - ph.tap0;
        }
    }
    for (int i = 0; i < d->n_out; ++i) {
      KResult& r = p->out[i];
      r.p = d->out[i].data;
      r.C = d->out[i].C;
      r.accumulate = d->out[i].accumulate;
      r.sn = d->out[i].stride_n;
      r.sh = d->out[i].stride_h;
      r.sw = d->out[i].stride_w;
      r.n_begin = (i == 0) ? 0 : p->out[i - 1].n_begin + p->out[i - 1].C;
      r.linear = (p->nphases == 1 && r.sh == (long long)d->OW * r.sw && r.sn == (long long)d->OH * r.sh) ? 1 : 0;
    }
    DN_REQUIRE(d->bn_partial == nullptr || (d->n_out == 1 && p->nphases == 1), DN_ERR_UNSUPPORTED,
               "bn_partial needs a single un-phased result");
  }
  long long m = (long long)p->N * p->GH * p->GW;
  DN_REQUIRE(m > 0 && m < (1ll << 31), DN_ERR_UNSUPPORTED, "grid too large");
  p->M = (int)m;
  p->mGW = fastdiv_magic((unsigned)p->GW);
  p->mGH = fastdiv_magic((unsigned)p->GH);
  p->allvec = 1;
  p->uni32 = 1;
  p->any_affine = 0;
  for (int z = 0; z < p->nphases; ++z)
    if (p->ph[z].ntaps > 32) p->uni32 = 0;
  int n_fast = 0, n_uniform = 0;
  for (int i = 0; i < p->n_in; ++i) {
    const KOperand& o = p->in[i];
    if (o.scale != nullptr) p->any_affine = 1;
    p->in[i].small = offsets_fit_int32(p->in[i], p->N, p->IH, p->IW) && ((long long)p->N * (o.sn < 0 ? -o.sn : o.sn) + 16) * 4 < (1ll << 31) ? 1 : 0;
    if (!(p->in[i].vec && p->in[i].small)) p->allvec = 0;
    if (p->in[i].vec && p->in[i].small && o.up == 0 && (o.C % 32 == 0 || o.C == 4 || o.C == 8 || o.C == 16)) ++n_fast;
    if (p->in[i].vec && p->in[i].small && o.up == 0 && o.C % 32 == 0) ++n_uniform;
  }
  (void)n_fast;
  if (p->reflect) p->uni32 = 0;
  for (int i = 0; i < p->n_in; ++i)
    if (!p->in[i].small) p->uni32 = 0;
  p->wg_uniform = (!p->reflect && p->ph[0].ntaps <= 32) ? 1 : 0;
  for (int i = 0; i < p->n_in; ++i) {
    const KOperand& o = p->in[i];
    if (!o.small || (!o.vec && o.scale != nullptr) || o.C >= 32768) p->wg_uniform = 0;
  }
  (void)n_uniform;
  p->tile_store = false ? 0 : (false ? 1 : 2);
  p->compute = norm_compute(d->compute);
  p->BN = pick_bn(p->Ntot);
  p->Npad = ceil_div(p->Ntot, p->BN) * p->BN;
  long long woff = 0;
  for (int z = 0; z < p->nphases; ++z) {
    int nch = 0;
    for (int i = 0; i < p->n_in; ++i) nch += ceil_div(p->ph[z].ntaps * p->in[i].C, kChunk);
    p->ph[z].nchunks = nch;
    p->ph[z].w_off = woff;
    woff += (long long)p->Npad * nch * kChunk;
  }
  return DN_OK;
}

static const ConvFamily* plan_route(const dn_conv_desc* d, IgemmParams* p) {
  return build_plan(d, false, p) == DN_OK ? conv_route(d, *p) : nullptr;
}

}

extern "C" {

int dn_version(void) { return 21; }

void dn_reload_knobs(void) {
  std::lock_guard<std::mutex> lock(dn::g_knobs_mu);
  dn::read_knobs(&dn::g_knobs);
  dn::g_knobs_state.store(1, std::memory_order_release);
}

const char* dn_last_error(void) { return dn::g_err; }

const char* dn_last_kernel(void) { return dn::g_kernel; }

int dn_device_arch_ok(void) {
  int dev = 0;
  if (hipGetDevice(&dev) != hipSuccess) {
    dn::set_error("hipGetDevice failed (no HIP device?)");
    return DN_ERR_LAUNCH;
  }
  hipDeviceProp_t prop;
  if (hipGetDeviceProperties(&prop, dev) != hipSuccess) {
    dn::set_error("hipGetDeviceProperties failed");
    return DN_ERR_LAUNCH;
  }
  return strncmp(prop.gcnArchName, "gfx950", 6) == 0 ? 1 : 0;
}

int64_t dn_conv_packed_weight_elems(const dn_conv_desc* d) {
  dn::IgemmParams p;
  const dn::ConvFamily* f = dn::plan_route(d, &p);
  if (f == nullptr) return -1;
  return f->weight_layout ? dn::wino_packed_floats(p, f->weight_layout(p)) : dn::direct_packed_elems(p);
}

int32_t dn_conv_weight_layout(const dn_conv_desc* d) {
  dn::IgemmParams p;
  const dn::ConvFamily* f = dn::plan_route(d, &p);
  return f == nullptr ? -1 : (f->weight_layout ? f->weight_layout(p) : 0);
}

int32_t dn_conv_bn_partial_rows(const dn_conv_desc* d) {
  dn::IgemmParams p;
  if (dn::build_plan(d, false, &p) != DN_OK) return -1;
  return (p.M + 127) / 128;
}

int32_t dn_conv_fwd_fuses_reciprocal(const dn_conv_desc* d) {
  dn::IgemmParams p;
  const dn::ConvFamily* f = dn::plan_route(d, &p);
  return (f != nullptr && f->fuses_reciprocal && f->fuses_reciprocal(p)) ? 1 : 0;
}

int32_t dn_conv_dgrad_fuses_bn_sums(const dn_conv_desc* d) {
  dn::IgemmParams p;
  const dn::ConvFamily* f = dn::plan_route(d, &p);
  return f == nullptr ? -1 : ((f->takes_bn_sums && f->takes_bn_sums(d)) ? 1 : 0);
}

int32_t dn_conv_fwd_folds_bn_finalize(const dn_conv_desc* d) {
  dn::IgemmParams p;
  const dn::ConvFamily* f = dn::plan_route(d, &p);
  return f == nullptr ? -1 : ((f->folds_bn_finalize && f->folds_bn_finalize(p)) ? 1 : 0);
}

int32_t dn_conv_dgrad_folds_bn_sums(const dn_conv_desc* d) {
  dn::IgemmParams p;
  const dn::ConvFamily* f = dn::plan_route(d, &p);
  return (f != nullptr && f->takes_bn_sums && f->takes_bn_sums(d) && f->folds_bn_sums(p)) ? 1 : 0;
}

int64_t dn_conv_splitk_workspace_bytes(const dn_conv_desc* d) {
  dn::IgemmParams p;
  const dn::ConvFamily* f = dn::plan_route(d, &p);
  return f != nullptr ? (int64_t)f->splitk_workspace_bytes(p) : -1;
}

int dn_debug_conv_plan(const dn_conv_desc* d, int for_wgrad, int32_t* out, int cap) {
  dn::IgemmParams p;
  int rc = dn::build_plan(d, for_wgrad != 0, &p);
  if (rc != DN_OK) return rc;
  int n = 0;
  auto put = [&](long long v) {
    if (n < cap) out[n] = (int32_t)v;
    ++n;
  };
// ... 20 lines not shown
```

### supervised_dispnet_amd/csrc/dn_pointwise.hip

```cpp
#include "dn_device.h"
#include "dn_fold.h"

namespace dn {

constexpr int kThreads = 256;
constexpr int kMaxReduceBlocks = 4096;

static inline int ew_blocks(long long n_items) {
  long long b = (n_items + kThreads - 1) / kThreads;
  if (b > 4096) b = 4096;
  if (b < 1) b = 1;
  return (int)b;
}

static inline int reduce_blocks(long long rows, int C) {
  int V = (C % 4 == 0) ? 4 : 1;
  int groups = C / V;
  int tpr = 1;
  while (tpr < groups && tpr < kThreads) tpr <<= 1;
  int rpi = kThreads / tpr;
  const int rpt = 2;
  long long b = (rows + (long long)rpi * rpt - 1) / ((long long)rpi * rpt);
  const int cap = 1024 < kMaxReduceBlocks ? 1024 : kMaxReduceBlocks;
  if (b > cap) b = cap;
  if (b < 1) b = 1;
  return (int)b;
}

template <class Op, int V>
__global__ void __launch_bounds__(kThreads) colreduce_kernel(Op op, long long rows, int C, float* __restrict__ partial) {
  constexpr int NACC = Op::NACC;
  const int groups = C / V;
  int tpr = 1;
  while (tpr < groups && tpr < kThreads) tpr <<= 1;
  const int rpi = kThreads / tpr;
  const int rl = threadIdx.x / tpr, gi = threadIdx.x % tpr;
  const long long per = (rows + gridDim.x - 1) / gridDim.x;
  const long long rbeg = blockIdx.x * per;
  const long long rend = (rbeg + per < rows) ? rbeg + per : rows;
  __shared__ float red[kThreads * V * NACC];
  for (int g0 = 0; g0 < groups; g0 += tpr) {
    const int grp = g0 + gi;
    float acc[V][NACC];
#pragma unroll
    for (int v = 0; v < V; ++v)
#pragma unroll
      for (int a = 0; a < NACC; ++a) acc[v][a] = 0.f;
    if (grp < groups)
      for (long long r = rbeg + rl; r < rend; r += rpi) op.template apply<V>(r, grp * V, acc);
#pragma unroll
    for (int v = 0; v < V; ++v)
#pragma unroll
      for (int a = 0; a < NACC; ++a) red[(threadIdx.x * V + v) * NACC + a] = acc[v][a];
    __syncthreads();
    if (rl == 0 && grp < groups) {
#pragma unroll
      for (int v = 0; v < V; ++v)
#pragma unroll
        for (int a = 0; a < NACC; ++a) {
          float s = 0.f;
          for (int q = 0; q < rpi; ++q) s += red[((q * tpr + gi) * V + v) * NACC + a];
          partial[((long long)blockIdx.x * C + grp * V + v) * NACC + a] = s;
        }
    }
    __syncthreads();
  }
}

template <class Op>
static int launch_colreduce(const Op& op, long long rows, int C, float* partial, hipStream_t s, const char* what) {
  const int blocks = reduce_blocks(rows, C);
  if (C % 4 == 0)
    DN_LAUNCH((colreduce_kernel<Op, 4>), dim3(blocks), dim3(kThreads), 0, s, op, rows, C, partial);
  else
    DN_LAUNCH((colreduce_kernel<Op, 1>), dim3(blocks), dim3(kThreads), 0, s, op, rows, C, partial);
  return check_launch(what);
}

template <int V>
struct Vec {
  float v[V];
};
template <int V>
// ... 238 lines not shown
      g.v[e] = dz;
      acc[e][0] += dz;
      acc[e][1] += dz * (yv.v[e] - mu.v[e]) * is.v[e];
    }
    if (write) stv<V>(da_dz + o, g);
  }
};

struct ActBwdOp {
  static constexpr int NACC = 1;
  const float* src;
  float* g;
  const float* y_post;
  int act;
  float p0, p1;
  int C;
  template <int V>
  __device__ __forceinline__ void apply(long long row, int c0, float (&acc)[V][1]) const {
    const long long o = row * C + c0;
    Vec<V> gv = ldv<V>(src + o);
    if (act == DN_ACT_NONE) {
      if (src != g) stv<V>(g + o, gv);
    } else {
      const Vec<V> yv = ldv<V>(y_post + o);
#pragma unroll
      for (int e = 0; e < V; ++e) {
        const float yp = yv.v[e];
        float d = 1.f;
        if (act == DN_ACT_RELU) d = yp > 0.f ? 1.f : 0.f;
        else if (act == DN_ACT_LEAKY) d = yp > 0.f ? 1.f : p0;
        else if (act == DN_ACT_ELU) d = yp > 0.f ? 1.f : (yp + 1.f);
        else if (act == DN_ACT_SIGMOID_AFFINE) {
          const float sg = (yp - p1) / p0;
          d = p0 * sg * (1.f - sg);
        }
        gv.v[e] *= d;
      }
      stv<V>(g + o, gv);
    }
#pragma unroll
    for (int e = 0; e < V; ++e) acc[e][0] += gv.v[e];
  }
};

__global__ void __launch_bounds__(256) colsum_finalize_kernel(const float* __restrict__ partial, int rows, int C, int stride, int offset,
                                                              float* __restrict__ out) {
  const int lane = threadIdx.x & 63;
  const int c = blockIdx.x * 4 + (threadIdx.x >> 6);
  if (c >= C) return;
  double s = 0.0;
  for (int r = lane; r < rows; r += 64) s += (double)partial[((long long)r * C + c) * stride + offset];
#pragma unroll
  for (int o = 32; o > 0; o >>= 1) s += __shfl_xor(s, o);
  if (lane == 0) out[c] = (float)s;
}

__global__ void __launch_bounds__(256) colsum2_finalize_kernel(const float* __restrict__ partial, int rows, int C, int stride, int offset,
                                                               float* __restrict__ out0, float* __restrict__ out1) {
  const int c = blockIdx.x;
  double s0 = 0.0, s1 = 0.0;
#pragma unroll 4
  for (int r = threadIdx.x; r < rows; r += 256) {
    const float* q = partial + ((long long)r * C + c) * stride + offset;
    s0 += (double)q[0];
    s1 += (double)q[1];
  }
#pragma unroll
  for (int o = 32; o > 0; o >>= 1) {
    s0 += __shfl_xor(s0, o);
    s1 += __shfl_xor(s1, o);
  }
  __shared__ double red[2][4];
  if ((threadIdx.x & 63) == 0) {
    red[0][threadIdx.x >> 6] = s0;
    red[1][threadIdx.x >> 6] = s1;
  }
  __syncthreads();
  if (threadIdx.x == 0) {
    out0[c] = (float)((red[0][0] + red[0][1]) + (red[0][2] + red[0][3]));
    out1[c] = (float)((red[1][0] + red[1][1]) + (red[1][2] + red[1][3]));
  }
}

__device__ __forceinline__ float bn_bwd_value(float z, float yv, float mu, float is, float ga, float dg, float db, float inv_count) {
#pragma clang fp contract(off)
  const float xhat = (yv - mu) * is;
  float t = __builtin_fmaf(-db, inv_count, z);
  t = __builtin_fmaf(-(xhat * dg), inv_count, t);
  return (ga * is) * t;
}

__global__ void __launch_bounds__(kThreads) bn_bwd_apply_kernel(float* __restrict__ dz_dy, const float* __restrict__ y,
                                                                const float* __restrict__ mean, const float* __restrict__ invstd,
                                                                const float* __restrict__ gamma, const float* __restrict__ dgamma,
                                                                const float* __restrict__ dbeta, long long rows, int C, float inv_count) {
  const int G = C / 4;
  const long long total = rows * G;
  for (long long i = blockIdx.x * (long long)kThreads + threadIdx.x; i < total; i += (long long)gridDim.x * kThreads) {
    const int c = (int)(i % G) * 4;
    const long long o = i * 4;
    f32x4 dz = *reinterpret_cast<const f32x4*>(dz_dy + o);
    const f32x4 yv = *reinterpret_cast<const f32x4*>(y + o);
    const f32x4 mu = *reinterpret_cast<const f32x4*>(mean + c), is = *reinterpret_cast<const f32x4*>(invstd + c);
    const f32x4 ga = *reinterpret_cast<const f32x4*>(gamma + c), dg = *reinterpret_cast<const f32x4*>(dgamma + c),
                db = *reinterpret_cast<const f32x4*>(dbeta + c);
#pragma unroll
    for (int e = 0; e < 4; ++e) {
      dz[e] = bn_bwd_value(dz[e], yv[e], mu[e], is[e], ga[e], dg[e], db[e], inv_count);
    }
    *reinterpret_cast<f32x4*>(dz_dy + o) = dz;
  }
}

__global__ void __launch_bounds__(kThreads) bn_bwd_apply_relu_kernel(float* __restrict__ da_dy, const float* __restrict__ y,
                                                                     const float* __restrict__ scale, const float* __restrict__ shift,
                                                                     const float* __restrict__ mean, const float* __restrict__ invstd,
                                                                     const float* __restrict__ gamma, const float* __restrict__ dgamma,
                                                                     const float* __restrict__ dbeta, long long rows, int C, float inv_count) {
  const int G = C / 4;
  const long long total = rows * G;
  for (long long i = blockIdx.x * (long long)kThreads + threadIdx.x; i < total; i += (long long)gridDim.x * kThreads) {
    const int c = (int)(i % G) * 4;
    const long long o = i * 4;
    f32x4 dz = *reinterpret_cast<const f32x4*>(da_dy + o);
    const f32x4 yv = *reinterpret_cast<const f32x4*>(y + o);
    const f32x4 sc = *reinterpret_cast<const f32x4*>(scale + c), sh = *reinterpret_cast<const f32x4*>(shift + c);
    const f32x4 mu = *reinterpret_cast<const f32x4*>(mean + c), is = *reinterpret_cast<const f32x4*>(invstd + c);
    const f32x4 ga = *reinterpret_cast<const f32x4*>(gamma + c), dg = *reinterpret_cast<const f32x4*>(dgamma + c),
                db = *reinterpret_cast<const f32x4*>(dbeta + c);
#pragma unroll
    for (int e = 0; e < 4; ++e) {
      const float z = (yv[e] * sc[e] + sh[e] > 0.f) ? dz[e] : 0.f;
      dz[e] = bn_bwd_value(z, yv[e], mu[e], is[e], ga[e], dg[e], db[e], inv_count);
    }
    *reinterpret_cast<f32x4*>(da_dy + o) = dz;
  }
}

__global__ void __launch_bounds__(kThreads) bn_bwd_apply_relu_hoisted_kernel(float* __restrict__ da_dy, const float* __restrict__ y,
                                                                             const float* __restrict__ scale, const float* __restrict__ shift,
                                                                             const float* __restrict__ mean, const float* __restrict__ invstd,
                                                                             const float* __restrict__ gamma, const float* __restrict__ dgamma,
                                                                             const float* __restrict__ dbeta, long long rows, int C, float inv_count) {
  const int G = C / 4;
  const long long total = rows * G;
  const int c = (int)(threadIdx.x % (unsigned)G) * 4;
  const f32x4 sc = *reinterpret_cast<const f32x4*>(scale + c), sh = *reinterpret_cast<const f32x4*>(shift + c);
  const f32x4 mu = *reinterpret_cast<const f32x4*>(mean + c), is = *reinterpret_cast<const f32x4*>(invstd + c);
  const f32x4 ga = *reinterpret_cast<const f32x4*>(gamma + c), dg = *reinterpret_cast<const f32x4*>(dgamma + c),
              db = *reinterpret_cast<const f32x4*>(dbeta + c);
  const long long step = (long long)gridDim.x * kThreads;
  for (long long i0 = blockIdx.x * (long long)kThreads + threadIdx.x; i0 < total; i0 += 4 * step) {
    f32x4 dz[4], yv[4];
#pragma unroll
    for (int u = 0; u < 4; ++u) {
      const long long i = i0 + u * step;
      if (i < total) {
        dz[u] = __builtin_nontemporal_load(reinterpret_cast<const f32x4*>(da_dy + i * 4));
        yv[u] = __builtin_nontemporal_load(reinterpret_cast<const f32x4*>(y + i * 4));
      }
    }
#pragma unroll
    for (int u = 0; u < 4; ++u) {
      const long long i = i0 + u * step;
      if (i < total) {
#pragma unroll
        for (int e = 0; e < 4; ++e) {
          const float z = (yv[u][e] * sc[e] + sh[e] > 0.f) ? dz[u][e] : 0.f;
          dz[u][e] = bn_bwd_value(z, yv[u][e], mu[e], is[e], ga[e], dg[e], db[e], inv_count);
        }
        *reinterpret_cast<f32x4*>(da_dy + i * 4) = dz[u];
      }
    }
  }
}

__global__ void __launch_bounds__(kThreads) bn_bwd_apply_hoisted_kernel(float* __restrict__ dz_dy, const float* __restrict__ y,
                                                                        const float* __restrict__ mean, const float* __restrict__ invstd,
                                                                        const float* __restrict__ gamma, const float* __restrict__ dgamma,
                                                                        const float* __restrict__ dbeta, long long rows, int C, float inv_count) {
  const int G = C / 4;
  const long long total = rows * G;
  const long long first = blockIdx.x * (long long)kThreads + threadIdx.x;
  const int c = (int)(first % G) * 4;
  const f32x4 mu = *reinterpret_cast<const f32x4*>(mean + c), is = *reinterpret_cast<const f32x4*>(invstd + c);
  const f32x4 ga = *reinterpret_cast<const f32x4*>(gamma + c), dg = *reinterpret_cast<const f32x4*>(dgamma + c),
              db = *reinterpret_cast<const f32x4*>(dbeta + c);
  const long long step = (long long)gridDim.x * kThreads;
  for (long long i0 = first; i0 < total; i0 += 4 * step) {
    f32x4 dz[4], yv[4];
#pragma unroll
    for (int u = 0; u < 4; ++u) {
      const long long i = i0 + u * step;
      if (i < total) {
        dz[u] = __builtin_nontemporal_load(reinterpret_cast<const f32x4*>(dz_dy + i * 4));
        yv[u] = __builtin_nontemporal_load(reinterpret_cast<const f32x4*>(y + i * 4));
      }
    }
#pragma unroll
    for (int u = 0; u < 4; ++u) {
      const long long i = i0 + u * step;
      if (i < total) {
#pragma unroll
        for (int e = 0; e < 4; ++e) dz[u][e] = bn_bwd_value(dz[u][e], yv[u][e], mu[e], is[e], ga[e], dg[e], db[e], inv_count);
        *reinterpret_cast<f32x4*>(dz_dy + i * 4) = dz[u];
      }
    }
  }
}

__global__ void __launch_bounds__(kThreads) bn_bwd_apply_pool_kernel(const float* __restrict__ dpooled, const uint8_t* __restrict__ idx,
                                                                     const float* __restrict__ y, const float* __restrict__ mean,
                                                                     const float* __restrict__ invstd, const float* __restrict__ gamma,
                                                                     const float* __restrict__ dgamma, const float* __restrict__ dbeta, int N,
                                                                     int H, int W, int C, float inv_count, float* __restrict__ dy) {
  const int G = C / 4, PH = H / 2, PW = W / 2;
  const long long total = (long long)N * PH * PW * G;
  for (long long i = blockIdx.x * (long long)kThreads + threadIdx.x; i < total; i += (long long)gridDim.x * kThreads) {
    const int g = (int)(i % G);
    long long pix = i / G;
    const int px = (int)(pix % PW);
    pix /= PW;
    const int py = (int)(pix % PH), n = (int)(pix / PH);
    const int c = g * 4;
    const f32x4 dp = *reinterpret_cast<const f32x4*>(dpooled + i * 4);
    const uchar4 code = *reinterpret_cast<const uchar4*>(idx + i * 4);
    const int cd[4] = {code.x, code.y, code.z, code.w};
    const f32x4 mu = *reinterpret_cast<const f32x4*>(mean + c), is = *reinterpret_cast<const f32x4*>(invstd + c);
    const f32x4 ga = *reinterpret_cast<const f32x4*>(gamma + c), dg = *reinterpret_cast<const f32x4*>(dgamma + c),
                db = *reinterpret_cast<const f32x4*>(dbeta + c);
    const long long base = (((long long)n * H + 2 * py) * W + 2 * px) * C + c;
#pragma unroll
    for (int q = 0; q < 4; ++q) {
      const long long o = base + ((long long)(q >> 1) * W + (q & 1)) * C;
      const f32x4 yv = *reinterpret_cast<const f32x4*>(y + o);
      f32x4 out;
#pragma unroll
      for (int e = 0; e < 4; ++e) {
        const float z = ((cd[e] & 4) && (cd[e] & 3) == q) ? dp[e] : 0.f;
        out[e] = bn_bwd_value(z, yv[e], mu[e], is[e], ga[e], dg[e], db[e], inv_count);
      }
      *reinterpret_cast<f32x4*>(dy + o) = out;
    }
  }
}

__global__ void __launch_bounds__(kThreads) bn_add_relu_fwd_kernel(const float* __restrict__ y, const float* __restrict__ scale,
                                                                   const float* __restrict__ shift, const float* __restrict__ r,
                                                                   const float* __restrict__ r_scale, const float* __restrict__ r_shift,
                                                                   long long rows, int C, float* __restrict__ out) {
  const int G = C / 4;
// ... 369 lines not shown
  DN_LAUNCH(bn_finalize_kernel, dim3(C), dim3(kThreads), 0, as_stream(stream), partial, rows, C, (double)count, conv_bias, gamma,
                     beta, running_mean, running_var, momentum, eps, mean, invstd, scale, shift,
                     reinterpret_cast<long long*>(num_batches_tracked));
  return check_launch("bn_finalize_kernel");
}

int dn_bn_eval_affine(int32_t C, const float* gamma, const float* beta, const float* running_mean, const float* running_var, float eps,
                      float* scale, float* shift, dn_stream_t stream) {
  DN_REQUIRE(C > 0 && gamma && beta && running_mean && running_var && scale && shift, DN_ERR_BAD_ARG, "dn_bn_eval_affine: bad argument");
  DN_LAUNCH(bn_eval_affine_kernel, dim3((C + 255) / 256), dim3(256), 0, as_stream(stream), C, gamma, beta, running_mean,
                     running_var, eps, scale, shift);
  return check_launch("bn_eval_affine_kernel");
}

int dn_bn_relu_pool_fwd(const float* y, const float* scale, const float* shift, int32_t N, int32_t H, int32_t W, int32_t C, float* pooled,
                        uint8_t* idx, dn_stream_t stream) {
  DN_REQUIRE(y && pooled && idx && ((scale == nullptr) == (shift == nullptr)), DN_ERR_BAD_ARG, "dn_bn_relu_pool_fwd: null pointer");
  DN_REQUIRE(C % 4 == 0 && H % 2 == 0 && W % 2 == 0 && N > 0, DN_ERR_UNSUPPORTED, "dn_bn_relu_pool_fwd: need C%%4==0 and even H,W");
  const long long total = (long long)N * (H / 2) * (W / 2) * (C / 4);
  DN_LAUNCH(bn_relu_pool_fwd_kernel, dim3(ew_blocks(total)), dim3(kThreads), 0, as_stream(stream), y, scale, shift, N, H, W, C,
                     pooled, idx);
  return check_launch("bn_relu_pool_fwd_kernel");
}

int dn_maxpool2_bwd(const float* dpooled, const uint8_t* idx, int32_t N, int32_t H, int32_t W, int32_t C, float* dx, int32_t accumulate,
                    dn_stream_t stream) {
  DN_REQUIRE(dpooled && idx && dx && N > 0, DN_ERR_BAD_ARG, "dn_maxpool2_bwd: bad argument");
  DN_REQUIRE(C % 4 == 0 && H % 2 == 0 && W % 2 == 0, DN_ERR_UNSUPPORTED, "dn_maxpool2_bwd: need C%%4==0 and even H,W");
  const long long total = (long long)N * (H / 2) * (W / 2) * (C / 4);
  DN_LAUNCH(maxpool2_bwd_kernel, dim3(ew_blocks(total)), dim3(kThreads), 0, as_stream(stream), dpooled, idx, N, H, W, C, dx, accumulate);
  return check_launch("maxpool2_bwd_kernel");
}

int dn_bn_relu_pool_bwd(const float* dpooled, const uint8_t* idx, const float* y, const float* mean, const float* invstd, int32_t N,
                        int32_t H, int32_t W, int32_t C, float* dz, float* partial, dn_stream_t stream) {
  DN_REQUIRE(dpooled && idx && y && mean && invstd && dz && partial, DN_ERR_BAD_ARG, "dn_bn_relu_pool_bwd: null pointer");
  DN_REQUIRE(C % 4 == 0 && H % 2 == 0 && W % 2 == 0, DN_ERR_UNSUPPORTED, "dn_bn_relu_pool_bwd: need C%%4==0 and even H,W");
  PoolBwdOp op{dpooled, idx, y, mean, invstd, dz, H / 2, W / 2, H, W, C};
  return launch_colreduce(op, (long long)N * (H / 2) * (W / 2), C, partial, as_stream(stream), "bn_relu_pool_bwd");
}

int dn_bn_relu_pool_bwd_sums(const float* dpooled, const uint8_t* idx, const float* y, const float* mean, const float* invstd, int32_t N,
                             int32_t H, int32_t W, int32_t C, float* partial, dn_stream_t stream) {
  DN_REQUIRE(dpooled && idx && y && mean && invstd && partial, DN_ERR_BAD_ARG, "dn_bn_relu_pool_bwd_sums: null pointer");
  DN_REQUIRE(C % 4 == 0 && H % 2 == 0 && W % 2 == 0, DN_ERR_UNSUPPORTED, "dn_bn_relu_pool_bwd_sums: need C%%4==0 and even H,W");
  PoolBwdOp op{dpooled, idx, y, mean, invstd, nullptr, H / 2, W / 2, H, W, C};
  return launch_colreduce(op, (long long)N * (H / 2) * (W / 2), C, partial, as_stream(stream), "bn_relu_pool_bwd_sums");
}

int dn_bn_relu_bwd_reduce(float* da_dz, const float* y, const float* scale, const float* shift, const float* mean, const float* invstd,
                          int64_t rows, int32_t C, float* partial, dn_stream_t stream) {
  DN_REQUIRE(da_dz && y && scale && shift && mean && invstd && partial && rows > 0 && C > 0, DN_ERR_BAD_ARG,
             "dn_bn_relu_bwd_reduce: bad argument");
  BnReluBwdOp op{1, da_dz, y, scale, shift, mean, invstd, C};
  return launch_colreduce(op, rows, C, partial, as_stream(stream), "bn_relu_bwd_reduce");
}

int dn_bn_relu_bwd_sums(const float* da, const float* y, const float* scale, const float* shift, const float* mean, const float* invstd,
                        int64_t rows, int32_t C, float* partial, dn_stream_t stream) {
  DN_REQUIRE(da && y && scale && shift && mean && invstd && partial && rows > 0 && C > 0, DN_ERR_BAD_ARG, "dn_bn_relu_bwd_sums: bad argument");
  BnReluBwdOp op{0, const_cast<float*>(da), y, scale, shift, mean, invstd, C};
  return launch_colreduce(op, rows, C, partial, as_stream(stream), "bn_relu_bwd_sums");
}

static void launch_colsum2(const float* partial, int32_t partial_rows, int32_t C, int32_t partial_stride, int32_t partial_offset, float* out0,
                           float* out1, hipStream_t s) {
  if (partial_rows <= kFoldMaxRows && (partial_stride & 1) == 0 && (partial_offset & 1) == 0 && (reinterpret_cast<uintptr_t>(partial) & 7) == 0)
    DN_LAUNCH(colsum2_sliced_kernel, dim3((C + 63) / 64), dim3(256), 0, s, partial, partial_rows, C, partial_stride, partial_offset, out0, out1);
  else
    DN_LAUNCH(colsum2_finalize_kernel, dim3(C), dim3(256), 0, s, partial, partial_rows, C, partial_stride, partial_offset, out0, out1);
}

static int bn_bwd_sums_to_params(const float* partial, int32_t partial_rows, int32_t partial_stride, int32_t partial_offset, int32_t C,
                                 float* dgamma, float* dbeta, hipStream_t s, const char* who) {
  DN_REQUIRE(dgamma && dbeta, DN_ERR_BAD_ARG, "%s: bad argument", who);
  DN_REQUIRE(C % 4 == 0, DN_ERR_UNSUPPORTED, "%s: need C%%4==0", who);
  if (partial == nullptr) return DN_OK;
  DN_REQUIRE(partial_rows > 0, DN_ERR_BAD_ARG, "%s: bad argument", who);
  DN_REQUIRE(partial_stride >= 2 && partial_offset >= 0 && partial_offset + 1 < partial_stride, DN_ERR_BAD_ARG, "%s: partial layout", who);
  launch_colsum2(partial, partial_rows, C, partial_stride, partial_offset, dbeta, dgamma, s);
  return DN_OK;
}

int dn_bn_bwd_apply_relu(float* da_dy, const float* y, const float* scale, const float* shift, const float* mean, const float* invstd,
                         const float* gamma, const float* partial, int32_t partial_rows, int32_t partial_stride, int32_t partial_offset,
                         int64_t rows, int32_t C, float* dgamma, float* dbeta, dn_stream_t stream) {
  DN_REQUIRE(da_dy && y && scale && shift && mean && invstd && gamma && rows > 0, DN_ERR_BAD_ARG, "dn_bn_bwd_apply_relu: bad argument");
  hipStream_t s = as_stream(stream);
  int rc = bn_bwd_sums_to_params(partial, partial_rows, partial_stride, partial_offset, C, dgamma, dbeta, s, "dn_bn_bwd_apply_relu");
  if (rc != DN_OK) return rc;
  const bool hoisted = C % 4 == 0 && kThreads % (C / 4) == 0;
  set_last_kernel(hoisted ? "dn::bn_bwd_apply_relu_hoisted_kernel" : "dn::bn_bwd_apply_relu_kernel");
  if (hoisted)
    DN_LAUNCH(bn_bwd_apply_relu_hoisted_kernel, dim3(ew_blocks((rows * (C / 4) + 3) / 4)), dim3(kThreads), 0, s, da_dy, y, scale, shift, mean,
              invstd, gamma, dgamma, dbeta, (long long)rows, C, (float)(1.0 / (double)rows));
  else
    DN_LAUNCH(bn_bwd_apply_relu_kernel, dim3(ew_blocks(rows * (C / 4))), dim3(kThreads), 0, s, da_dy, y, scale, shift, mean, invstd, gamma,
                     dgamma, dbeta, (long long)rows, C, (float)(1.0 / (double)rows));
  return check_launch("bn_bwd_apply_relu");
}

int dn_bn_bwd_apply_pool(const float* dpooled, const uint8_t* idx, const float* y, const float* mean, const float* invstd, const float* gamma,
                         const float* partial, int32_t partial_rows, int32_t partial_stride, int32_t partial_offset, int32_t N, int32_t H,
                         int32_t W, int32_t C, float* dy, float* dgamma, float* dbeta, dn_stream_t stream) {
  DN_REQUIRE(dpooled && idx && y && mean && invstd && gamma && dy && N > 0, DN_ERR_BAD_ARG, "dn_bn_bwd_apply_pool: bad argument");
  DN_REQUIRE(H % 2 == 0 && W % 2 == 0, DN_ERR_UNSUPPORTED, "dn_bn_bwd_apply_pool: need even H, W");
  hipStream_t s = as_stream(stream);
  int rc = bn_bwd_sums_to_params(partial, partial_rows, partial_stride, partial_offset, C, dgamma, dbeta, s, "dn_bn_bwd_apply_pool");
  if (rc != DN_OK) return rc;
  const long long total = (long long)N * (H / 2) * (W / 2) * (C / 4);
  DN_LAUNCH(bn_bwd_apply_pool_kernel, dim3(ew_blocks(total)), dim3(kThreads), 0, s, dpooled, idx, y, mean, invstd, gamma, dgamma, dbeta, N,
                     H, W, C, (float)(1.0 / ((double)N * H * W)), dy);
  return check_launch("bn_bwd_apply_pool");
}

int dn_bn_bwd_apply(float* dz_dy, const float* y, const float* mean, const float* invstd, const float* gamma, const float* partial,
                    int32_t partial_rows, int32_t partial_stride, int32_t partial_offset, int64_t rows, int32_t C, float* dgamma,
                    float* dbeta, dn_stream_t stream) {
  DN_REQUIRE(dz_dy && y && mean && invstd && gamma && partial && dgamma && dbeta && rows > 0, DN_ERR_BAD_ARG, "dn_bn_bwd_apply: bad argument");
  DN_REQUIRE(C % 4 == 0, DN_ERR_UNSUPPORTED, "dn_bn_bwd_apply: need C%%4==0");
  DN_REQUIRE(partial_stride >= 2 && partial_offset >= 0 && partial_offset + 1 < partial_stride, DN_ERR_BAD_ARG, "dn_bn_bwd_apply: partial layout");
  hipStream_t s = as_stream(stream);
  launch_colsum2(partial, partial_rows, C, partial_stride, partial_offset, dbeta, dgamma, s);
  const int G = C / 4;
  int blocks = ew_blocks((rows * (long long)G + 3) / 4);
  int ga = G, gb = kThreads;
  while (gb != 0) {
    const int t = ga % gb;
    ga = gb;
    gb = t;
  }
  const int per = G / ga;
  if (per <= 64) {
    blocks = (blocks + per - 1) / per * per;
    set_last_kernel("dn::bn_bwd_apply_hoisted_kernel");
    DN_LAUNCH(bn_bwd_apply_hoisted_kernel, dim3(blocks), dim3(kThreads), 0, s, dz_dy, y, mean, invstd, gamma, dgamma, dbeta, (long long)rows, C,
              (float)(1.0 / (double)rows));
  } else {
    set_last_kernel("dn::bn_bwd_apply_kernel");
    DN_LAUNCH(bn_bwd_apply_kernel, dim3(ew_blocks(rows * (C / 4))), dim3(kThreads), 0, s, dz_dy, y, mean, invstd, gamma, dgamma, dbeta,
              (long long)rows, C, (float)(1.0 / (double)rows));
  }
  return check_launch("bn_bwd_apply");
}

int dn_act_bwd_reduce(float* g, const float* y_post, int32_t act, float p0, float p1, int64_t rows, int32_t C, float* partial,
                      dn_stream_t stream) {
  DN_REQUIRE(g && partial && rows > 0 && C > 0 && (act == DN_ACT_NONE || y_post), DN_ERR_BAD_ARG, "dn_act_bwd_reduce: bad argument");
  ActBwdOp op{g, g, y_post, act, p0, p1, C};
  return launch_colreduce(op, rows, C, partial, as_stream(stream), "act_bwd_reduce");
}

int dn_act_bwd_reduce_from(const float* g_in, float* g_out, const float* y_post, int32_t act, float p0, float p1, int64_t rows, int32_t C,
                           float* partial, dn_stream_t stream) {
  DN_REQUIRE(g_in && g_out && partial && rows > 0 && C > 0 && (act == DN_ACT_NONE || y_post), DN_ERR_BAD_ARG, "dn_act_bwd_reduce_from: bad argument");
  ActBwdOp op{g_in, g_out, y_post, act, p0, p1, C};
  return launch_colreduce(op, rows, C, partial, as_stream(stream), "act_bwd_reduce_from");
}

int dn_colsum_finalize(const float* partial, int32_t rows, int32_t C, int32_t stride, int32_t offset, float* out, dn_stream_t stream) {
  DN_REQUIRE(partial && out && rows > 0 && C > 0 && stride > 0 && offset >= 0 && offset < stride, DN_ERR_BAD_ARG, "dn_colsum_finalize: bad argument");
  DN_LAUNCH(colsum_finalize_kernel, dim3((C + 3) / 4), dim3(256), 0, as_stream(stream), partial, rows, C, stride, offset, out);
  return check_launch("colsum_finalize_kernel");
}

int dn_upsample2x_nearest_bwd(const float* dfull, int32_t N, int32_t h, int32_t w, float* dlow, int32_t accumulate, dn_stream_t stream) {
// ... 161 lines not shown
```

### supervised_dispnet_amd/engine.py

```python
import ctypes as C
import math
import os
import threading
import weakref

import torch

from . import _lib
from ._lib import (ACT_LEAKY, ACT_NONE, ACT_RELU, ACT_SIGMOID_AFFINE, CONV_DGRAD, CONV_FWD, CONVT_DGRAD, CONVT_FWD,
                   ConvDesc)

BN_EPS = 1e-5
BN_MOMENTUM = 0.1

PARAM_EPOCH = 0


PROFILE = None

SPLITK = True
PACK_ON_SIDE_STREAM = True
PACK_LATE_MIN_ELEMS = 400000
BN_SUMS_FUSION = True
FOLD_FINALIZE = True
# ... 214 lines not shown
            self.e0.record()
        return self

    def __exit__(self, *exc):
        if PROFILE is not None:
            self.e1.record()
            launched = _lib.load().dn_last_kernel().decode(errors="replace")
            PROFILE.append((launched or self.name, self.flops, self.e0, self.e1, self.tag, 0, int(self.abytes)))
        return False


def hbm_call(kernel, nbytes, entry, *args):
    if PROFILE is None:
        return _lib.call(entry, *args)
    e0 = torch.cuda.Event(enable_timing=True)
    e1 = torch.cuda.Event(enable_timing=True)
    e0.record()
    _lib.call(entry, *args)
    e1.record()
    if kernel is None:
        kernel = _lib.load().dn_last_kernel().decode(errors="replace")
    PROFILE.append((kernel, 0, e0, e1, entry, int(nbytes), int(nbytes)))


def bump_param_epoch():
    global PARAM_EPOCH
    PARAM_EPOCH += 1


_TLS = threading.local()


def _stream():
    h = getattr(_TLS, "handle", None)
    return h if h is not None else torch.cuda.current_stream().cuda_stream


class stream_scope(object):

    def __init__(self, stream=None):
        self.stream = stream

    def __enter__(self):
        self.prev = getattr(_TLS, "handle", None)
        if self.stream is not None:
            self.ctx = torch.cuda.stream(self.stream)
            self.ctx.__enter__()
            _TLS.handle = self.stream.cuda_stream
        else:
            self.ctx = None
            _TLS.handle = torch.cuda.current_stream().cuda_stream
        return self

    def __exit__(self, *exc):
        _TLS.handle = self.prev
        if self.ctx is not None:
            self.ctx.__exit__(*exc)
        return False


def _nbt_ptr(bn):
    t = getattr(bn, "num_batches_tracked", None)
    if t is None:
        return None
    if not t.is_cuda or t.dtype != torch.int64:
        t += 1
        return None
    return t.data_ptr()


def _ptr(t):
    return t.data_ptr() if t is not None else None


def require_cuda(t, what):
    if not t.is_cuda:
        raise RuntimeError("%s must live on the MI355X (got a %s tensor); this package is the HIP path only and has no "
                           "CPU fallback" % (what, t.device))


class Act:
    __slots__ = ("t", "N", "H", "W", "C", "scale", "shift", "mean", "invstd", "grad", "grad_is_dz", "partial",
                 "partial_rows", "partial_stride", "partial_offset", "needs_grad", "strides", "no_relu", "planar", "pool_src", "sums_ready",
                 "recip_t", "bn_owner", "sums_final", "seed_borrow", "grad_borrowed")

    def __init__(self, t, N, H, W, C, strides=None, needs_grad=True):
        self.t = t
        self.N, self.H, self.W, self.C = N, H, W, C
        self.scale = self.shift = self.mean = self.invstd = None
        self.grad = None
        self.grad_is_dz = False
        self.partial = None
        self.partial_rows = 0
        self.partial_stride, self.partial_offset = 2, 0
        self.no_relu = False
        self.sums_ready = False
        self.pool_src = None
        self.planar = False
        self.recip_t = None
        self.bn_owner = None
        self.sums_final = None
        self.seed_borrow = False
        self.grad_borrowed = False
        self.needs_grad = needs_grad
        self.strides = strides or (H * W * C, W * C, C, 1)

    @property
    def rows(self):
        return self.N * self.H * self.W

    @staticmethod
    def from_nchw(x, needs_grad=False):
        a = Act.from_nchw_image(x)
        a.needs_grad = needs_grad
        return a

    @staticmethod
    def from_nchw_image(x):
        n, c, h, w = x.shape
        sn, sc, sh, sw = x.stride()
        return Act(x, n, h, w, c, strides=(sn, sh, sw, sc), needs_grad=False)

    def new_like(self):
        return torch.empty((self.N, self.H, self.W, self.C), dtype=torch.float32, device=self.t.device)


class Tape:
    def __init__(self, recording):
        self.recording = recording
        self.steps = []
        self.last_out = None

    def push(self, fn, out=None):
        self.last_out = out
        if self.recording:
            self.steps.append(fn)

    def run_backward(self):
        for fn in reversed(self.steps):
            fn()
        self.steps = []


class Piece:
    __slots__ = ("act", "up")

    def __init__(self, act, up=False):
        self.act, self.up = act, up

    @property
    def C(self):
        return self.act.C


def _fill_operand(op, piece):
    a = piece.act
    if a.no_relu:
        raise RuntimeError("an activation with a pending ReLU-less BatchNorm can only feed block_bn_add_relu")
    op.data = a.t.data_ptr()
    op.C = a.C
    op.up_shift = 1 if piece.up else 0
    op.stride_n, op.stride_h, op.stride_w, op.stride_c = a.strides
    op.scale = _ptr(a.scale)
    op.shift = _ptr(a.shift)


def _fill_result(res, tensor, C_, H, W, accumulate, ld=None):
    ld = ld or C_
    res.data = tensor.data_ptr()
    res.C = C_
    res.accumulate = 1 if accumulate else 0
    res.stride_w = ld
    res.stride_h = W * ld
    res.stride_n = H * W * ld


class ConvLayer:

    def __init__(self, module, transposed=False, in_channels_split=None, reflect_pad=0):
        self.m = module
        self.transposed = transposed
        self.R, self.S = module.kernel_size
        self.stride = module.stride[0]
        self.pad = module.padding[0]
        self.dil = module.dilation[0] if not transposed else 1
        self.reflect = reflect_pad > 0
# ... 148 lines not shown
        h = _stream()
        if h == side.cuda_stream:
            return
        stream_wait(main if h == main.cuda_stream else torch.cuda.current_stream(), side, device_scope=True)
        self.pending = None


_PACK_TABLES = {}


def pack_table(device):
    t = _PACK_TABLES.get(device)
    if t is None:
        t = _PACK_TABLES[device] = PackTable(device)
    return t


def prepack_all(device):
    t = _PACK_TABLES.get(device)
    if t is not None:
        t.run(PARAM_EPOCH)


FUSE_RECIP = True


def conv_forward(layer, pieces, act=ACT_NONE, p0=0.0, p1=0.0, bn_stats=False, out_hw=None, out_view=None, recip=None, bn_fold=None):
    a0 = pieces[0].act
    N = a0.N
    IH = a0.H * (2 if pieces[0].up else 1)
    IW = a0.W * (2 if pieces[0].up else 1)
    OH, OW = out_hw or layer.out_size(IH, IW)
    kind = CONVT_FWD if layer.transposed else CONV_FWD
    d = layer._desc(kind, N, IH, IW, OH, OW)
    d.n_in = len(pieces)
    for i, p in enumerate(pieces):
        _fill_operand(d.in_[i], p)
    d.n_out = 1
    if out_view is None:
        y = torch.empty((N, OH, OW, layer.Cout), dtype=torch.float32, device=a0.t.device)
        _fill_result(d.out[0], y, layer.Cout, OH, OW, False)
    else:
        y, off, (vsn, vsh, vsw), vacc = out_view
        r = d.out[0]
        r.data = y.data_ptr() + 4 * off
        r.C = layer.Cout
        r.accumulate = 1 if vacc else 0
        r.stride_n, r.stride_h, r.stride_w = vsn, vsh, vsw
    d.w_packed = layer.packed(kind, d).data_ptr()
    b = layer.m.bias
    d.bias = _ptr(b.detach()) if b is not None else None
    d.act, d.act_p0, d.act_p1 = act, p0, p1
    _splitk_workspace(d, a0.t.device)
    partial, rows = None, 0
    if recip is not None and out_view is None and layer.Cout == 1 and _lib.load().dn_conv_fwd_fuses_reciprocal(C.byref(d)) == 1:
        recip.append(torch.empty((N, OH, OW, 1), dtype=torch.float32, device=a0.t.device))
        d.recip_out = recip[0].data_ptr()
    if bn_stats:
        rows = _lib.load().dn_conv_bn_partial_rows(C.byref(d))
        partial = torch.empty((rows, layer.Cout, 2), dtype=torch.float32, device=y.device)
        d.bn_partial = partial.data_ptr()
        if bn_fold is not None and FOLD_FINALIZE and d.splitk_ws:
            bn = bn_fold[0]
            d.bnf_gamma, d.bnf_beta = bn.weight.data_ptr(), bn.bias.data_ptr()
            d.bnf_running_mean, d.bnf_running_var = _ptr(bn.running_mean), _ptr(bn.running_var)
            d.bnf_num_batches_tracked = bn_fold[5]
            d.bnf_momentum = bn.momentum if bn.momentum is not None else BN_MOMENTUM
            d.bnf_eps = bn.eps
            d.bnf_mean, d.bnf_invstd, d.bnf_scale, d.bnf_shift = (t.data_ptr() for t in bn_fold[1:5])
            if _lib.load().dn_conv_fwd_folds_bn_finalize(C.byref(d)) == 1:
                bn_fold[0] = True
            else:
                d.bnf_scale = None
    if bn_fold is not None and bn_fold[0] is not True:
        bn_fold[0] = False
    with _Timed("igemm_conv_kernel<128,%d>" % _pick_bn(layer.Cout), 2 * layer.macs(N, IH, IW, OH, OW),
                "%s %dx%d k%d s%d cin%d cout%d in %dx%dx%d" % ("convT_fwd" if layer.transposed else "conv_fwd", layer.R, layer.S,
                                                               layer.R, layer.stride, layer.Cin, layer.Cout, N, IH, IW),
                4 * (sum(p.act.rows * p.act.C for p in pieces) + N * OH * OW * layer.Cout)):
        _lib.call("dn_convT2d_fwd" if layer.transposed else "dn_conv2d_fwd", C.byref(d), _stream())
    return y, partial, rows


def conv_wgrad(layer, pieces, dy, out_hw, out=None, sink=None, first=None):
    a0 = pieces[0].act
    IH = a0.H * (2 if pieces[0].up else 1)
    IW = a0.W * (2 if pieces[0].up else 1)
    OH, OW = out_hw
    kind = CONVT_FWD if layer.transposed else CONV_FWD
    d = layer._desc(kind, a0.N, IH, IW, OH, OW)
    d.n_in = len(pieces)
    for i, p in enumerate(pieces):
        _fill_operand(d.in_[i], p)
    d.n_out = 1
    d.out[0].C = layer.Cout
    lib = _lib.load()
    nbytes = lib.dn_conv_wgrad_workspace_bytes(C.byref(d))
    if nbytes == 0:
        raise _lib.DispnetHipError("dn_conv_wgrad_workspace_bytes: " + _lib.last_error())

    def launch():
        ws = torch.empty(nbytes // 4, dtype=torch.float32, device=dy.device)
        dw = out if out is not None else torch.empty_like(layer.m.weight, memory_format=torch.contiguous_format)
        with _Timed("igemm_wgrad_kernel<%d>" % _pick_bn(layer.Cin if layer.transposed else layer.Cout),
                    2 * layer.macs(a0.N, IH, IW, OH, OW),
                    "%s k%d s%d cin%d cout%d in %dx%dx%d" % ("convT_wgrad" if layer.transposed else "conv_wgrad", layer.R, layer.stride,
                                                             layer.Cin, layer.Cout, a0.N, IH, IW),
                    4 * (sum(p.act.rows * p.act.C for p in pieces) + dy.numel())):
            _lib.call("dn_conv2d_wgrad", C.byref(d), dy.data_ptr(), dw.data_ptr(), ws.data_ptr(), nbytes, _stream())
        if sink is not None:
            sink.put(layer.m.weight, dw)
        return dw

    if not (dy.is_cuda and wgrad_stream_enabled()):
        if first is not None:
            first[0]()
        return launch()
    st = side_stream()
    main = torch.cuda.current_stream()
    side = st["sides"][st["rr"] % min(len(st["sides"]), max(1, SIDE_STREAMS_ACTIVE))]
    st["rr"] += 1
    st["main"] = main
    stream_wait(side, main, device_scope=True)
    with stream_scope(side):
        if first is not None:
            fresh = first[0]()
            cross_stream_use(first[1], side)
            if fresh is not None:
                cross_stream_use(fresh, main)
        dw = launch()
    cross_stream_use(dy, side)
    for p in pieces:
        cross_stream_use(p.act.t, side)
        if p.act.scale is not None:
            cross_stream_use(p.act.scale, side)
            cross_stream_use(p.act.shift, side)
    if out is None:
        cross_stream_use(dw, main)
    return dw


def conv_dgrad(layer, dy, N, OH, OW, pieces, in_hw):
    targets = [p for p in pieces]
    if not any(p.act.needs_grad for p in targets):
        return
    IH, IW = in_hw
    kind = CONVT_DGRAD if layer.transposed else CONV_DGRAD
    rp = layer.pad if layer.reflect else 0
    GH, GW = IH + 2 * rp, IW + 2 * rp
    d = layer._desc(kind, N, OH, OW, GH, GW)
    if layer.reflect:
        d.pad = 0
    d.n_in = 1
    op = d.in_[0]
    op.data = dy.data_ptr()
    op.C = layer.Cout
    op.up_shift = 0
    op.stride_c, op.stride_w, op.stride_h, op.stride_n = 1, layer.Cout, OW * layer.Cout, OH * OW * layer.Cout
    d.n_out = len(targets)
    post = []
    for i, p in enumerate(targets):
        a = p.act
        if p.up or layer.reflect:
            tmp = torch.empty((N, GH, GW, a.C), dtype=torch.float32, device=dy.device)
            _fill_result(d.out[i], tmp, a.C, GH, GW, False)
            if a.needs_grad:
                post.append((p, tmp))
        elif not a.needs_grad:
            tmp = torch.empty((N, IH, IW, a.C), dtype=torch.float32, device=dy.device)
            _fill_result(d.out[i], tmp, a.C, IH, IW, False)
        else:
            first = a.grad is None
            if first:
                a.grad = a.new_like()
            else:
                a.sums_ready = False
                a.sums_final = None
            _fill_result(d.out[i], a.grad, a.C, IH, IW, not first)
    d.w_packed = layer.packed(kind, d).data_ptr()
    d.bias = None
    d.act = ACT_NONE
    _splitk_workspace(d, dy.device)
    fuse = None
    if BN_SUMS_FUSION and len(targets) == 1 and not layer.transposed and not layer.reflect:
        a = targets[0].act
        if (not targets[0].up and a.needs_grad and a.scale is not None and a.mean is not None and not a.no_relu and not a.grad_is_dz
                and d.out[0].accumulate == 0 and a.strides == (a.H * a.W * a.C, a.W * a.C, a.C, 1)):
            d.bnb_y, d.bnb_scale, d.bnb_shift = a.t.data_ptr(), a.scale.data_ptr(), a.shift.data_ptr()
            d.bnb_mean, d.bnb_invstd = a.mean.data_ptr(), a.invstd.data_ptr()
            rows = _lib.load().dn_conv_bn_partial_rows(C.byref(d))
            scratch = torch.empty((max(rows, 1), a.C, 2), dtype=torch.float32, device=dy.device)
            d.bnb_partial = scratch.data_ptr()
            if _lib.load().dn_conv_dgrad_fuses_bn_sums(C.byref(d)) == 1:
                fuse = (a, scratch, rows, None)
                if FOLD_FINALIZE and a.bn_owner is not None and d.splitk_ws:
                    obn, osink = a.bn_owner
                    dg, db = osink.dest(obn.weight), osink.dest(obn.bias)
                    if dg is None:
                        dg = torch.empty(a.C, dtype=torch.float32, device=dy.device)
                    if db is None:
                        db = torch.empty(a.C, dtype=torch.float32, device=dy.device)
                    d.bnb_dgamma, d.bnb_dbeta = dg.data_ptr(), db.data_ptr()
                    if _lib.load().dn_conv_dgrad_folds_bn_sums(C.byref(d)) == 1:
                        fuse = (a, scratch, rows, (dg, db))
                    else:
                        d.bnb_dgamma = d.bnb_dbeta = None
            else:
                d.bnb_y = d.bnb_partial = None
    with _Timed("igemm_conv_kernel<128,%d>" % _pick_bn(layer.Cin), 2 * layer.macs(N, IH, IW, OH, OW),
                "%s k%d s%d cin%d cout%d in %dx%dx%d" % ("convT_dgrad" if layer.transposed else "conv_dgrad", layer.R, layer.stride,
                                                         layer.Cin, layer.Cout, N, IH, IW),
                4 * (dy.numel() + sum(p.act.rows * p.act.C for p in targets))):
        _lib.call("dn_convT2d_dgrad" if layer.transposed else "dn_conv2d_dgrad", C.byref(d), _stream())
    if fuse is not None:
        a, scratch, rows, final = fuse
        a.partial, a.partial_rows, a.partial_stride, a.partial_offset = scratch, rows, 2, 0
        a.sums_ready = True
        a.sums_final = final
    for p, tmp in post:
        a = p.act
        cur = tmp
        if layer.reflect:
            if p.up:
                cur = torch.empty((N, IH, IW, a.C), dtype=torch.float32, device=dy.device)
                _lib.call("dn_reflect_fold", tmp.data_ptr(), N, IH, IW, a.C, rp, cur.data_ptr(), 0, _stream())
            else:
                first = a.grad is None
                if first:
                    a.grad = a.new_like()
                _lib.call("dn_reflect_fold", tmp.data_ptr(), N, IH, IW, a.C, rp, a.grad.data_ptr(), 0 if first else 1, _stream())
                continue
        first = a.grad is None
        if first:
            a.grad = a.new_like()
        if a.C == 1:
            _lib.call("dn_upsample2x_nearest_bwd", cur.data_ptr(), N, a.H, a.W, a.grad.data_ptr(), 0 if first else 1, _stream())
        else:
            _lib.call("dn_upsample2x_nearest_bwd_nhwc", cur.data_ptr(), N, a.H, a.W, a.C, a.grad.data_ptr(), 0 if first else 1, _stream())


def colsum(partial, rows, Cn, stride=1, offset=0, out=None):
    if out is None:
        out = torch.empty(Cn, dtype=torch.float32, device=partial.device)
    _lib.call("dn_colsum_finalize", partial.data_ptr(), rows, Cn, stride, offset, out.data_ptr(), _stream())
    return out


def act_bwd(g, y_post, act, p0, p1, rows, Cn, out=None, defer=False, src=None):
    nblk = _lib.load().dn_reduce_blocks(rows, Cn)
    partial = torch.empty((nblk, Cn), dtype=torch.float32, device=g.device)
    kname = "dn::colreduce_kernel<dn::ActBwdOp, %d>" % (4 if Cn % 4 == 0 else 1)
    if src is not None:
        hbm_call(kname, rows * Cn * 12, "dn_act_bwd_reduce_from", src.data_ptr(), g.data_ptr(), _ptr(y_post), act, p0, p1, rows, Cn,
                 partial.data_ptr(), _stream())
    else:
        hbm_call(kname, rows * Cn * 12, "dn_act_bwd_reduce", g.data_ptr(), _ptr(y_post), act, p0, p1, rows, Cn, partial.data_ptr(), _stream())
    if defer:
        return (lambda: colsum(partial, nblk, Cn, out=out)), partial
    return colsum(partial, nblk, Cn, out=out)


class GradSink:

    reducer = None

    def __init__(self):
        self.grads = {}

    @staticmethod
    def dest(param):
        return getattr(param, "_dn_grad_view", None)

    def put(self, param, g):
        dst = getattr(param, "_dn_grad_view", None)
        if dst is not None:
            if g.data_ptr() != dst.data_ptr():
                dst.copy_(g.view_as(dst))
            param._dn_zero_grad_slot = False
            self.grads[id(param)] = None
            if GradSink.reducer is not None:
                GradSink.reducer.grad_ready(param)
        else:
            self.grads[id(param)] = g

    def put_zero(self, param):
        dst = getattr(param, "_dn_grad_view", None)
        if dst is not None:
            if not getattr(param, "_dn_zero_grad_slot", False):
                _lib.call("dn_fill", dst.data_ptr(), 0.0, dst.numel(), _stream())
                param._dn_zero_grad_slot = True
            self.grads[id(param)] = None
            if GradSink.reducer is not None:
                GradSink.reducer.grad_ready(param)
        else:
            self.grads[id(param)] = torch.zeros_like(param)

    def put_none(self, param):
        if getattr(param, "_dn_grad_view", None) is not None:
            self.put_zero(param)

    def settle(self, params):
        for p in params:
            if id(p) not in self.grads and getattr(p, "_dn_grad_view", None) is not None and p.requires_grad:
                self.put_zero(p)

    def get(self, param):
        return self.grads.get(id(param))


def bn_backward(y, bn, sink, training):
    g, y_t, Cn, dev = y.grad, y.t, y.C, y.t.device
    if not training:
        raise NotImplementedError("backward through eval-mode BatchNorm (frozen statistics) is not implemented")
    relu_pending = not y.grad_is_dz
    final = None
    if relu_pending and y.sums_ready and not BN_MATERIALIZE_DZ:
        y.sums_ready = False
        final, y.sums_final = y.sums_final, None
    elif relu_pending:
        y.sums_ready = False
        if y.no_relu:
            raise RuntimeError("a ReLU-less BatchNorm output must be consumed by block_bn_add_relu / block_bn_plain")
        nblk = _lib.load().dn_reduce_blocks(y.rows, Cn)
        y.partial = torch.empty((nblk, Cn, 2), dtype=torch.float32, device=dev)
        y.partial_rows = nblk
        if BN_MATERIALIZE_DZ:
            hbm_call("dn::colreduce_kernel<dn::BnReluBwdOp, 4>", y.rows * Cn * 12, "dn_bn_relu_bwd_reduce", g.data_ptr(),
                     y_t.data_ptr(), y.scale.data_ptr(), y.shift.data_ptr(), y.mean.data_ptr(), y.invstd.data_ptr(), y.rows, Cn,
                     y.partial.data_ptr(), _stream())
        else:
            hbm_call("dn::colreduce_kernel<dn::BnReluBwdOp, 4>", y.rows * Cn * 8, "dn_bn_relu_bwd_sums", g.data_ptr(),
                     y_t.data_ptr(), y.scale.data_ptr(), y.shift.data_ptr(), y.mean.data_ptr(), y.invstd.data_ptr(), y.rows, Cn,
                     y.partial.data_ptr(), _stream())
    if final is not None:
        dgamma, dbeta = final
    else:
        dgamma = sink.dest(bn.weight)
        dbeta = sink.dest(bn.bias)
        if dgamma is None:
            dgamma = torch.empty(Cn, dtype=torch.float32, device=dev)
        if dbeta is None:
            dbeta = torch.empty(Cn, dtype=torch.float32, device=dev)
    if y.pool_src is not None:
        dpooled, pidx = y.pool_src
        hbm_call("dn::bn_bwd_apply_pool_kernel", y.rows * Cn * 8 + y.rows * Cn * 5 // 4, "dn_bn_bwd_apply_pool", dpooled.data_ptr(),
                 pidx.data_ptr(), y_t.data_ptr(), y.mean.data_ptr(), y.invstd.data_ptr(), bn.weight.data_ptr(), y.partial.data_ptr(),
                 y.partial_rows, y.partial_stride, y.partial_offset, y.N, y.H, y.W, Cn, g.data_ptr(), dgamma.data_ptr(),
                 dbeta.data_ptr(), _stream())
        y.pool_src = None
    elif relu_pending and not BN_MATERIALIZE_DZ:
        hbm_call(None, y.rows * Cn * 12, "dn_bn_bwd_apply_relu", g.data_ptr(), y_t.data_ptr(),
                 y.scale.data_ptr(), y.shift.data_ptr(), y.mean.data_ptr(), y.invstd.data_ptr(), bn.weight.data_ptr(),
                 None if final is not None else y.partial.data_ptr(), y.partial_rows, y.partial_stride, y.partial_offset, y.rows, Cn,
                 dgamma.data_ptr(), dbeta.data_ptr(), _stream())
    else:
        hbm_call(None, y.rows * Cn * 12, "dn_bn_bwd_apply", g.data_ptr(), y_t.data_ptr(), y.mean.data_ptr(),
                 y.invstd.data_ptr(), bn.weight.data_ptr(), y.partial.data_ptr(), y.partial_rows, y.partial_stride,
                 y.partial_offset, y.rows, Cn, dgamma.data_ptr(), dbeta.data_ptr(), _stream())
    sink.put(bn.weight, dgamma)
    sink.put(bn.bias, dbeta)
    return g


def _bn_pending(y, bn, partial, prow, training, conv_bias=None):
    Cn, dev = y.C, y.t.device
    y.scale = torch.empty(Cn, dtype=torch.float32, device=dev)
    y.shift = torch.empty(Cn, dtype=torch.float32, device=dev)
    if training:
        y.mean = torch.empty(Cn, dtype=torch.float32, device=dev)
        y.invstd = torch.empty(Cn, dtype=torch.float32, device=dev)
        _lib.call("dn_bn_finalize", partial.data_ptr(), prow, Cn, y.rows, _ptr(conv_bias.detach()) if conv_bias is not None else None,
                  bn.weight.data_ptr(), bn.bias.data_ptr(), bn.running_mean.data_ptr(), bn.running_var.data_ptr(),
                  bn.momentum if bn.momentum is not None else BN_MOMENTUM, bn.eps, y.mean.data_ptr(), y.invstd.data_ptr(),
                  y.scale.data_ptr(), y.shift.data_ptr(), _nbt_ptr(bn), _stream())
    else:
        _lib.call("dn_bn_eval_affine", Cn, bn.weight.data_ptr(), bn.bias.data_ptr(), bn.running_mean.data_ptr(),
                  bn.running_var.data_ptr(), bn.eps, y.scale.data_ptr(), y.shift.data_ptr(), _stream())


def block_conv_bn(tape, sink, x_piece, layer, bn, training, relu=True):
    xa = x_piece.act
    dev = xa.t.device
    Cn = layer.Cout
    scale = torch.empty(Cn, dtype=torch.float32, device=dev)
    shift = torch.empty(Cn, dtype=torch.float32, device=dev)
    mean = invstd = fold = nbt = None
    if training:
        mean = torch.empty(Cn, dtype=torch.float32, device=dev)
        invstd = torch.empty(Cn, dtype=torch.float32, device=dev)
        nbt = _nbt_ptr(bn)
        fold = [bn, mean, invstd, scale, shift, nbt]
    y_t, partial, prow = conv_forward(layer, [x_piece], ACT_NONE, bn_stats=training, bn_fold=fold)
    OH, OW = y_t.shape[1], y_t.shape[2]
    y = Act(y_t, xa.N, OH, OW, Cn)
    y.no_relu = not relu
    y.scale, y.shift, y.mean, y.invstd = scale, shift, mean, invstd
    y.bn_owner = (bn, sink)
    if training:
        if fold[0] is not True:
            _lib.call("dn_bn_finalize", partial.data_ptr(), prow, Cn, y.rows, _ptr(layer.m.bias.detach()) if layer.m.bias is not None else None,
                      bn.weight.data_ptr(), bn.bias.data_ptr(), bn.running_mean.data_ptr(), bn.running_var.data_ptr(),
                      bn.momentum if bn.momentum is not None else BN_MOMENTUM, bn.eps, y.mean.data_ptr(), y.invstd.data_ptr(),
                      y.scale.data_ptr(), y.shift.data_ptr(), nbt, _stream())
    else:
        _lib.call("dn_bn_eval_affine", Cn, bn.weight.data_ptr(), bn.bias.data_ptr(), bn.running_mean.data_ptr(),
                  bn.running_var.data_ptr(), bn.eps, y.scale.data_ptr(), y.shift.data_ptr(), _stream())

    def backward():
        if y.grad is None:
            return
        g = bn_backward(y, bn, sink, training)
        if layer.m.bias is not None:
            sink.put_zero(layer.m.bias)
        conv_wgrad(layer, [x_piece], g, (OH, OW), out=sink.dest(layer.m.weight), sink=sink)
        conv_dgrad(layer, g, xa.N, OH, OW, [x_piece], (xa.H, xa.W))
        y.grad = None

    tape.push(backward)
    return y


def block_pool(tape, y):
    dev = y.t.device
    p_t = torch.empty((y.N, y.H // 2, y.W // 2, y.C), dtype=torch.float32, device=dev)
    idx = torch.empty((y.N, y.H // 2, y.W // 2, y.C), dtype=torch.uint8, device=dev)
    hbm_call("dn::bn_relu_pool_fwd_kernel", y.rows * y.C * 4 * 1.25 + y.rows * y.C // 4, "dn_bn_relu_pool_fwd", y.t.data_ptr(),
             y.scale.data_ptr(), y.shift.data_ptr(), y.N, y.H, y.W, y.C, p_t.data_ptr(), idx.data_ptr(), _stream())
    p = Act(p_t, y.N, y.H // 2, y.W // 2, y.C)

    def backward():
        if p.grad is None:
            return
        nblk = _lib.load().dn_reduce_blocks(p.rows, y.C)
        y.partial = torch.empty((nblk, y.C, 2), dtype=torch.float32, device=dev)
        y.partial_rows = nblk
        y.grad = y.new_like()
        y.grad_is_dz = True
        if BN_MATERIALIZE_DZ:
            hbm_call("dn::colreduce_kernel<dn::PoolBwdOp, 4>", y.rows * y.C * 4 * 2.25 + y.rows * y.C // 4, "dn_bn_relu_pool_bwd",
                     p.grad.data_ptr(), idx.data_ptr(), y.t.data_ptr(), y.mean.data_ptr(), y.invstd.data_ptr(), y.N, y.H, y.W, y.C,
                     y.grad.data_ptr(), y.partial.data_ptr(), _stream())
        else:
            hbm_call("dn::colreduce_kernel<dn::PoolBwdOp, 4>", y.rows * y.C * 4 * 1.25 + y.rows * y.C // 4, "dn_bn_relu_pool_bwd_sums",
                     p.grad.data_ptr(), idx.data_ptr(), y.t.data_ptr(), y.mean.data_ptr(), y.invstd.data_ptr(), y.N, y.H, y.W, y.C,
                     y.partial.data_ptr(), _stream())
            y.pool_src = (p.grad, idx)
        p.grad = None

    tape.push(backward)
    return p


def block_conv_act(tape, sink, pieces, layer, act, p0=0.0, p1=0.0, out_hw=None, stat_bn=None):
    a0 = pieces[0].act
    in_hw = (a0.H * (2 if pieces[0].up else 1), a0.W * (2 if pieces[0].up else 1))
    want_recip = [] if (FUSE_RECIP and act == ACT_SIGMOID_AFFINE and layer.Cout == 1 and stat_bn is None and p1 > 0) else None
    y_t, partial, prow = conv_forward(layer, pieces, act, p0, p1, out_hw=out_hw, bn_stats=stat_bn is not None, recip=want_recip)
    OH, OW = y_t.shape[1], y_t.shape[2]
    y = Act(y_t, a0.N, OH, OW, layer.Cout)
    if want_recip:
        y.recip_t = want_recip[0]
    if stat_bn is not None:
        Cn, dev = layer.Cout, y_t.device
        scratch = torch.empty((4, Cn), dtype=torch.float32, device=dev)
        _lib.call("dn_bn_finalize", partial.data_ptr(), prow, Cn, y.rows, _ptr(layer.m.bias.detach()) if layer.m.bias is not None else None,
                  stat_bn.weight.data_ptr(), stat_bn.bias.data_ptr(), stat_bn.running_mean.data_ptr(), stat_bn.running_var.data_ptr(),
                  stat_bn.momentum if stat_bn.momentum is not None else BN_MOMENTUM, stat_bn.eps, scratch[0].data_ptr(),
                  scratch[1].data_ptr(), scratch[2].data_ptr(), scratch[3].data_ptr(), _nbt_ptr(stat_bn), _stream())

    def backward():
        if y.grad is None:
            sink.put_none(layer.m.weight)
            if layer.m.bias is not None:
                sink.put_none(layer.m.bias)
            return
        g, g_src = y.grad, None
        if y.grad_borrowed:
            g_src, g, y.grad_borrowed = g, torch.empty_like(y.grad), False
        finish_db, db_partial = act_bwd(g, y_t, act, p0, p1, y.rows, layer.Cout,
                                        out=sink.dest(layer.m.bias) if layer.m.bias is not None else None, defer=True, src=g_src)

        def bias_grad():
            db = finish_db()
            if layer.m.bias is not None:
                sink.put(layer.m.bias, db)
            return db if (layer.m.bias is None or sink.dest(layer.m.bias) is None) else None

        conv_wgrad(layer, pieces, g, (OH, OW), out=sink.dest(layer.m.weight), sink=sink, first=(bias_grad, db_partial))
        conv_dgrad(layer, g, a0.N, OH, OW, pieces, in_hw)
        y.grad = None

    tape.push(backward, out=y)
    return y


def _not_on_tape(what):
    if TAPE is not None and not TAPE.get("paused"):
        raise RuntimeError("launch tape: %s runs outside libdispnet_hip and would be missing from the replay" % what)
# ... 409 lines not shown
```

Baseline: 2052.

## Fuse BatchNorm backward apply into stem weight-gradient kernel

For the first conv layer, whose input needs no gradient, the BN+ReLU backward apply is deferred. The stem lds3 wgrad kernel reads y, applies the ReLU mask and BN backward formula while staging dy into LDS, so the separate elementwise pass that writes dz over the full-resolution activation is skipped. A small finalize launch computes dgamma/dbeta from the partial sums. The kernel's thread-to-channel mapping changes and a barrier moves after the next loads are issued. Cost: extra y loads and registers in the wgrad kernel, which could lower occupancy.

```diff
diff --git a/include/dispnet_hip.h b/include/dispnet_hip.h
--- a/include/dispnet_hip.h
+++ b/include/dispnet_hip.h
@@ -96,6 +96,7 @@
   float* bnf_shift;
   float* bnb_dgamma;
   float* bnb_dbeta;
+  const float* bnb_gamma;
 } dn_conv_desc;
 
 enum { DN_COMPUTE_DEFAULT = 0, DN_COMPUTE_BF16 = 1, DN_COMPUTE_F32X3 = 2, DN_COMPUTE_F32 = 3 };
@@ -118,6 +119,7 @@
 int dn_convT2d_dgrad(const dn_conv_desc* d, dn_stream_t stream);
 
 size_t dn_conv_wgrad_workspace_bytes(const dn_conv_desc* fwd);
+int32_t dn_conv_wgrad_applies_bn_bwd(const dn_conv_desc* fwd);
 int dn_conv2d_wgrad(const dn_conv_desc* fwd, const float* dy, float* dw, void* workspace, size_t workspace_bytes,
                     dn_stream_t stream);
 
@@ -146,6 +148,8 @@
 int dn_bn_bwd_apply_relu(float* da_dy, const float* y, const float* scale, const float* shift, const float* mean, const float* invstd,
                          const float* gamma, const float* partial, int32_t partial_rows, int32_t partial_stride, int32_t partial_offset,
                          int64_t rows, int32_t C, float* dgamma, float* dbeta, dn_stream_t stream);
+int dn_bn_bwd_sums_finalize(const float* partial, int32_t partial_rows, int32_t partial_stride, int32_t partial_offset, int32_t C,
+                            float* dgamma, float* dbeta, dn_stream_t stream);
 int dn_bn_bwd_apply_pool(const float* dpooled, const uint8_t* idx, const float* y, const float* mean, const float* invstd, const float* gamma,
                          const float* partial, int32_t partial_rows, int32_t partial_stride, int32_t partial_offset, int32_t N, int32_t H,
                          int32_t W, int32_t C, float* dy, float* dgamma, float* dbeta, dn_stream_t stream);
diff --git a/supervised_dispnet_amd/_lib.py b/supervised_dispnet_amd/_lib.py
--- a/supervised_dispnet_amd/_lib.py
+++ b/supervised_dispnet_amd/_lib.py
@@ -5,7 +5,7 @@
 _PKG = pathlib.Path(__file__).resolve().parent
 LIB_PATH = pathlib.Path(os.environ.get("DISPNET_HIP_LIB", _PKG / "libdispnet_hip.so"))
 
-EXPECTED_ABI = 21
+EXPECTED_ABI = 22
 
 DN_MAX_OPERANDS = 3
 ACT_NONE, ACT_RELU, ACT_LEAKY, ACT_ELU, ACT_SIGMOID_AFFINE = 0, 1, 2, 3, 4
@@ -40,7 +40,7 @@
                 ("bnf_gamma", _f32p), ("bnf_beta", _f32p), ("bnf_running_mean", _f32p), ("bnf_running_var", _f32p),
                 ("bnf_num_batches_tracked", C.c_void_p), ("bnf_momentum", C.c_float), ("bnf_eps", C.c_float),
                 ("bnf_mean", _f32p), ("bnf_invstd", _f32p), ("bnf_scale", _f32p), ("bnf_shift", _f32p),
-                ("bnb_dgamma", _f32p), ("bnb_dbeta", _f32p)]
+                ("bnb_dgamma", _f32p), ("bnb_dbeta", _f32p), ("bnb_gamma", _f32p)]
 
 
 _P = C.POINTER
@@ -69,6 +69,7 @@
     "dn_convT2d_fwd": (C.c_int, [_P(ConvDesc), _vp]),
     "dn_convT2d_dgrad": (C.c_int, [_P(ConvDesc), _vp]),
     "dn_conv_wgrad_workspace_bytes": (_sz, [_P(ConvDesc)]),
+    "dn_conv_wgrad_applies_bn_bwd": (_i32, [_P(ConvDesc)]),
     "dn_conv2d_wgrad": (C.c_int, [_P(ConvDesc), _vp, _vp, _vp, _sz, _vp]),
     "dn_bn_finalize": (C.c_int, [_vp, _i32, _i32, _i64, _vp, _vp, _vp, _vp, _vp, _f, _f, _vp, _vp, _vp, _vp, _vp, _vp]),
     "dn_bn_eval_affine": (C.c_int, [_i32, _vp, _vp, _vp, _vp, _f, _vp, _vp, _vp]),
@@ -76,6 +77,7 @@
     "dn_bn_relu_bwd_sums": (C.c_int, [_vp, _vp, _vp, _vp, _vp, _vp, _i64, _i32, _vp, _vp]),
     "dn_bn_relu_pool_bwd_sums": (C.c_int, [_vp, _vp, _vp, _vp, _vp, _i32, _i32, _i32, _i32, _vp, _vp]),
     "dn_bn_bwd_apply_relu": (C.c_int, [_vp, _vp, _vp, _vp, _vp, _vp, _vp, _vp, _i32, _i32, _i32, _i64, _i32, _vp, _vp, _vp]),
+    "dn_bn_bwd_sums_finalize": (C.c_int, [_vp, _i32, _i32, _i32, _i32, _vp, _vp, _vp]),
     "dn_bn_bwd_apply_pool": (C.c_int, [_vp, _vp, _vp, _vp, _vp, _vp, _vp, _i32, _i32, _i32, _i32, _i32, _i32, _i32, _vp, _vp, _vp, _vp]),
     "dn_maxpool2_bwd": (C.c_int, [_vp, _vp, _i32, _i32, _i32, _i32, _vp, _i32, _vp]),
     "dn_bn_relu_pool_bwd": (C.c_int, [_vp, _vp, _vp, _vp, _vp, _i32, _i32, _i32, _i32, _vp, _vp, _vp]),
diff --git a/supervised_dispnet_amd/csrc/dn_bn_bwd.h b/supervised_dispnet_amd/csrc/dn_bn_bwd.h
--- /dev/null
+++ b/supervised_dispnet_amd/csrc/dn_bn_bwd.h
@@ -0,0 +1,16 @@
+#pragma once
+#include "dn_device.h"
+
+namespace dn {
+
+__device__ __forceinline__ bool bn_relu_mask(float yv, float sc, float sh) { return __builtin_fmaf(yv, sc, sh) > 0.f; }
+
+__device__ __forceinline__ float bn_bwd_value(float z, float yv, float mu, float is, float ga, float dg, float db, float inv_count) {
+#pragma clang fp contract(off)
+  const float xhat = (yv - mu) * is;
+  float t = __builtin_fmaf(-db, inv_count, z);
+  t = __builtin_fmaf(-(xhat * dg), inv_count, t);
+  return (ga * is) * t;
+}
+
+}
diff --git a/supervised_dispnet_amd/csrc/dn_conv.hip b/supervised_dispnet_amd/csrc/dn_conv.hip
--- a/supervised_dispnet_amd/csrc/dn_conv.hip
+++ b/supervised_dispnet_amd/csrc/dn_conv.hip
@@ -114,6 +114,7 @@
   bool dy_aligned16;
   bool (*switched_off)();
   int (*launch)(const dn_conv_desc* fwd, IgemmParams& p, float* dw, hipStream_t s);
+  bool (*applies_bn_bwd)(const dn_conv_desc* fwd, const IgemmParams& p) = nullptr;
 };
 static const WgradFamily kWgradFamilies[] = {
     {"head", head_wgrad_eligible, [](const dn_conv_desc*, const IgemmParams& p) { return head_wgrad_workspace_bytes(p); }, false,
@@ -122,7 +123,7 @@
     {"winograd", wino_wgrad_eligible, [](const dn_conv_desc*, const IgemmParams& p) { return wino_wgrad_workspace_bytes(p); }, false, nullptr,
      [](const dn_conv_desc*, IgemmParams& p, float* dw, hipStream_t s) { return launch_wino_wgrad(p, dw, s); }},
     {"lds3", lds3_wgrad_eligible, [](const dn_conv_desc*, const IgemmParams& p) { return lds3_wgrad_workspace_bytes(p); }, true, nullptr,
-     launch_lds3_wgrad},
+     launch_lds3_wgrad, lds3_wgrad_applies_bn_bwd},
     {"lds3k", lds3k_wgrad_eligible, [](const dn_conv_desc*, const IgemmParams& p) { return lds3k_wgrad_workspace_bytes(p); }, true, nullptr,
      launch_lds3k_wgrad},
     {"stemk", stemk_wgrad_eligible, stemk_wgrad_workspace_bytes, true, nullptr, launch_stemk_wgrad},
@@ -189,6 +190,16 @@
 int dn_convT2d_fwd(const dn_conv_desc* d, dn_stream_t stream) { return run_conv(d, DN_CONVT_FWD, stream); }
 int dn_convT2d_dgrad(const dn_conv_desc* d, dn_stream_t stream) { return run_conv(d, DN_CONVT_DGRAD, stream); }
 
+int32_t dn_conv_wgrad_applies_bn_bwd(const dn_conv_desc* fwd) {
+  IgemmParams p;
+  if (build_plan(fwd, true, &p) != DN_OK) return -1;
+  for (const WgradFamily& f : kWgradFamilies) {
+    if (!f.eligible(fwd, p) || (f.switched_off && f.switched_off())) continue;
+    return (f.applies_bn_bwd && f.applies_bn_bwd(fwd, p)) ? 1 : 0;
+  }
+  return 0;
+}
+
 size_t dn_conv_wgrad_workspace_bytes(const dn_conv_desc* fwd) {
   IgemmParams p;
   if (build_plan(fwd, true, &p) != DN_OK) return 0;
@@ -220,8 +231,12 @@
   DN_REQUIRE(dy != nullptr && dw != nullptr && workspace != nullptr, DN_ERR_BAD_ARG, "null pointer");
   const hipStream_t s = as_stream(stream);
   for (const WgradFamily& f : kWgradFamilies) {
-    if (!f.eligible(fwd, p) || (f.switched_off && f.switched_off()) || workspace_bytes < f.workspace_bytes(fwd, p)) continue;
-    if (f.dy_aligned16 && (reinterpret_cast<uintptr_t>(dy) & 15) != 0) continue;
+    if (!f.eligible(fwd, p) || (f.switched_off && f.switched_off())) continue;
+    if (workspace_bytes < f.workspace_bytes(fwd, p) || (f.dy_aligned16 && (reinterpret_cast<uintptr_t>(dy) & 15) != 0)) {
+      DN_REQUIRE(!(f.applies_bn_bwd && f.applies_bn_bwd(fwd, p)), DN_ERR_WORKSPACE,
+                 "dn_conv2d_wgrad: bnb_* set, but the workspace or the alignment of dy keeps the %s row from running", f.name);
+      continue;
+    }
     for (int i = 0; i < p.n_in; ++i) DN_REQUIRE(p.in[i].p != nullptr, DN_ERR_BAD_ARG, "operand %d has no data", i);
     p.g = dy;
     p.ws = reinterpret_cast<float*>(workspace);
diff --git a/supervised_dispnet_amd/csrc/dn_internal.h b/supervised_dispnet_amd/csrc/dn_internal.h
--- a/supervised_dispnet_amd/csrc/dn_internal.h
+++ b/supervised_dispnet_amd/csrc/dn_internal.h
@@ -54,6 +54,7 @@
   bool no_wino_splitk, no_x3_splitk, no_wino8_tail;
   bool no_x3_direct, no_x3_wgrad;
   bool no_tap_windows;
+  bool no_stem_bnb_fuse;
   int wino_wgw;
   int wino_min_tiles;
   int wino_splitk_target, wino_splitk_maxblocks;
@@ -251,6 +252,7 @@
 bool lds3_conv_eligible(const dn_conv_desc* d, const IgemmParams& p);
 int launch_lds3_conv(const dn_conv_desc* d, const IgemmParams& p, hipStream_t stream);
 bool lds3_wgrad_eligible(const dn_conv_desc* fwd, const IgemmParams& p);
+bool lds3_wgrad_applies_bn_bwd(const dn_conv_desc* fwd, const IgemmParams& p);
 size_t lds3_wgrad_workspace_bytes(const IgemmParams& p);
 int launch_lds3_wgrad(const dn_conv_desc* fwd, IgemmParams& p, float* dw, hipStream_t stream);
 bool lds3k_wgrad_eligible(const dn_conv_desc* fwd, const IgemmParams& p);
diff --git a/supervised_dispnet_amd/csrc/dn_lds3_wgrad.hip b/supervised_dispnet_amd/csrc/dn_lds3_wgrad.hip
--- a/supervised_dispnet_amd/csrc/dn_lds3_wgrad.hip
+++ b/supervised_dispnet_amd/csrc/dn_lds3_wgrad.hip
@@ -1,6 +1,6 @@
 #include <stdlib.h>
 
-#include "dn_device.h"
+#include "dn_bn_bwd.h"
 
 namespace dn {
 
@@ -196,13 +196,18 @@
   }
 }
 
+struct StemBnb {
+  const float *y, *scale, *shift, *mean, *invstd, *gamma, *dgamma, *dbeta;
+  float inv_count;
+};
 constexpr int WS_GSTR = 272;
 constexpr int WS_GPIECE = 64 * WS_GSTR;
 constexpr int WS_ICOLS = 36;
 constexpr int WS_IPLANE = 10 * WS_ICOLS;
 constexpr int WGS_LDS = 3 * WS_GPIECE + 3 * WS_IPLANE * 4;
 
-__global__ void __launch_bounds__(256, 2) lds3_wgrad_stem_kernel(const IgemmParams p, const WgGeo geo) {
+template <bool BNB>
+__global__ void __launch_bounds__(256, 2) lds3_wgrad_stem_kernel(const IgemmParams p, const WgGeo geo, const StemBnb bnb) {
   extern __shared__ __align__(16) char lds[];
   char* Gp = lds;
   float* Ip = reinterpret_cast<float*>(lds + 3 * WS_GPIECE);
@@ -230,17 +235,34 @@
 
   f32x4 vg[8];
   float vi[4];
+  f32x4 vy[BNB ? 8 : 1];
+  unsigned glive = 0;
+  f32x4 bsc, bsh, bmu, bis, bga, bdg, bdb;
+  __amdgpu_buffer_rsrc_t ry = rg;
+  if constexpr (BNB) {
+    ry = __builtin_amdgcn_make_buffer_rsrc(const_cast<float*>(bnb.y), 0, 0x80000000u, 0x00020000);
+    const int c = 4 * (tid & 15);
+    bsc = *reinterpret_cast<const f32x4*>(bnb.scale + c), bsh = *reinterpret_cast<const f32x4*>(bnb.shift + c);
+    bmu = *reinterpret_cast<const f32x4*>(bnb.mean + c), bis = *reinterpret_cast<const f32x4*>(bnb.invstd + c);
+    bga = *reinterpret_cast<const f32x4*>(bnb.gamma + c), bdg = *reinterpret_cast<const f32x4*>(bnb.dgamma + c);
+    bdb = *reinterpret_cast<const f32x4*>(bnb.dbeta + c);
+  }
   auto issue_g = [&](int t, int h) __attribute__((always_inline)) {
     const int txb = t % geo.tilesX, q1 = t / geo.tilesX;
     const int tyb = q1 % geo.tilesY, n = q1 / geo.tilesY;
-    const int pxg = tid & 15, cq = tid >> 4, row = pxg >> 2, cgp = pxg & 3;
+    const int cq = tid & 15, pxg = tid >> 4, row = pxg >> 2, cgp = pxg & 3;
     const int gy = tyb * WG_TH + 4 * h + row;
+    if constexpr (BNB) glive = 0;
 #pragma unroll
     for (int i = 0; i < 8; ++i) {
       const int gx = txb * WG_TW + 8 * cgp + i;
       const bool ok = gy < p.GH && gx < p.GW;
       const int off = (((n * p.GH + gy) * p.GW + gx) * p.Ntot + 4 * cq) * 4;
       vg[i] = __builtin_bit_cast(f32x4, __builtin_amdgcn_raw_buffer_load_b128(rg, ok ? off : -1, 0, 0));
+      if constexpr (BNB) {
+        vy[i] = __builtin_bit_cast(f32x4, __builtin_amdgcn_raw_buffer_load_b128(ry, ok ? off : -1, 0, 0));
+        glive |= ok ? 1u << i : 0u;
+      }
     }
   };
   auto issue_img = [&](int t) __attribute__((always_inline)) {
@@ -258,7 +280,17 @@
     }
   };
   auto store_g = [&]() __attribute__((always_inline)) {
-    const int pxg = tid & 15, cq = tid >> 4;
+    const int cq = tid & 15, pxg = tid >> 4;
+    if constexpr (BNB) {
+#pragma unroll
+      for (int i = 0; i < 8; ++i)
+#pragma unroll
+        for (int e = 0; e < 4; ++e) {
+          const float z = bn_relu_mask(vy[i][e], bsc[e], bsh[e]) ? vg[i][e] : 0.f;
+          const float dz = bn_bwd_value(z, vy[i][e], bmu[e], bis[e], bga[e], bdg[e], bdb[e], bnb.inv_count);
+          vg[i][e] = (glive >> i) & 1 ? dz : 0.f;
+        }
+    }
 #pragma unroll
     for (int e = 0; e < 4; ++e) {
       const float v[8] = {vg[0][e], vg[1][e], vg[2][e], vg[3][e], vg[4][e], vg[5][e], vg[6][e], vg[7][e]};
@@ -292,12 +324,12 @@
     for (int h = 0; h < 2; ++h) {
       store_g();
       if (h == 0) store_img();
-      __syncthreads();
       if (h == 0) issue_g(t, 1);
       else if (t + nlocal < band_hi) {
         issue_g(t + nlocal, 0);
         issue_img(t + nlocal);
       }
+      __syncthreads();
       const int r = 4 * h + wave;
       bf16x8 b[2][3];
 #pragma unroll
@@ -371,6 +403,12 @@
 
 bool lds3_wgrad_eligible(const dn_conv_desc* d, const IgemmParams& p) { return lds3_wgrad_form(d, p) != 0; }
 
+bool lds3_wgrad_applies_bn_bwd(const dn_conv_desc* d, const IgemmParams& p) {
+  if (knobs().no_stem_bnb_fuse || lds3_wgrad_form(d, p) != 3) return false;
+  return d->bnb_y && d->bnb_scale && d->bnb_shift && d->bnb_mean && d->bnb_invstd && d->bnb_gamma &&
+         (reinterpret_cast<uintptr_t>(d->bnb_y) & 15) == 0;
+}
+
 size_t lds3_wgrad_workspace_bytes(const IgemmParams& p) {
   return (size_t)lds3_wgrad_blocks(p) * p.Npad * p.ph[0].nchunks * kChunk * sizeof(float);
 }
@@ -385,10 +423,17 @@
   geo.slab = (long long)p.Npad * p.ph[0].nchunks * kChunk;
   const int blocks = lds3_wgrad_blocks(p);
   hipError_t e = hipSuccess;
-  if (form == 3) {
-    e = hipFuncSetAttribute(reinterpret_cast<const void*>(lds3_wgrad_stem_kernel), hipFuncAttributeMaxDynamicSharedMemorySize, WGS_LDS);
-    if (e == hipSuccess) DN_LAUNCH(lds3_wgrad_stem_kernel, dim3(blocks), dim3(256), (size_t)WGS_LDS, stream, p, geo);
-    set_last_kernel("dn::lds3_wgrad_stem_kernel");
+  if (form == 3 && lds3_wgrad_applies_bn_bwd(d, p)) {
+    DN_REQUIRE(d->bnb_dgamma && d->bnb_dbeta, DN_ERR_BAD_ARG, "dn_conv2d_wgrad: bnb_y needs the finished sums bnb_dgamma / bnb_dbeta");
+    const StemBnb bnb{d->bnb_y, d->bnb_scale, d->bnb_shift, d->bnb_mean, d->bnb_invstd, d->bnb_gamma, d->bnb_dgamma, d->bnb_dbeta,
+                      (float)(1.0 / (double)p.M)};
+    e = hipFuncSetAttribute(reinterpret_cast<const void*>(lds3_wgrad_stem_kernel<true>), hipFuncAttributeMaxDynamicSharedMemorySize, WGS_LDS);
+    if (e == hipSuccess) DN_LAUNCH(lds3_wgrad_stem_kernel<true>, dim3(blocks), dim3(256), (size_t)WGS_LDS, stream, p, geo, bnb);
+    set_last_kernel("dn::lds3_wgrad_stem_kernel<true>");
+  } else if (form == 3) {
+    e = hipFuncSetAttribute(reinterpret_cast<const void*>(lds3_wgrad_stem_kernel<false>), hipFuncAttributeMaxDynamicSharedMemorySize, WGS_LDS);
+    if (e == hipSuccess) DN_LAUNCH(lds3_wgrad_stem_kernel<false>, dim3(blocks), dim3(256), (size_t)WGS_LDS, stream, p, geo, StemBnb{});
+    set_last_kernel("dn::lds3_wgrad_stem_kernel<false>");
   } else if (form == 2) {
     e = hipFuncSetAttribute(reinterpret_cast<const void*>(lds3_wgrad16_kernel<true>), hipFuncAttributeMaxDynamicSharedMemorySize, WG16_LDS);
     if (e == hipSuccess) DN_LAUNCH(lds3_wgrad16_kernel<true>, dim3(blocks), dim3(256), (size_t)WG16_LDS, stream, p, geo);
diff --git a/supervised_dispnet_amd/csrc/dn_plan.hip b/supervised_dispnet_amd/csrc/dn_plan.hip
--- a/supervised_dispnet_amd/csrc/dn_plan.hip
+++ b/supervised_dispnet_amd/csrc/dn_plan.hip
@@ -94,6 +94,7 @@
   k->no_lds3 = on("DN_NO_LDS3");
   k->no_x3_wgrad = on("DN_NO_X3_WGRAD");
   k->no_tap_windows = on("DN_NO_TAP_WINDOWS");
+  k->no_stem_bnb_fuse = on("DN_NO_STEM_BNB_FUSE");
   k->wino_wg_target = num("DN_WINO_WG_TARGET", 0);
   k->wino_nmajor = num("DN_WINO_NMAJOR", 1);
   k->no_riding_fences = on("DN_NO_RIDING_FENCES");
@@ -372,7 +373,7 @@
 
 extern "C" {
 
-int dn_version(void) { return 21; }
+int dn_version(void) { return 22; }
 
 void dn_reload_knobs(void) {
   std::lock_guard<std::mutex> lock(dn::g_knobs_mu);
diff --git a/supervised_dispnet_amd/csrc/dn_pointwise.hip b/supervised_dispnet_amd/csrc/dn_pointwise.hip
--- a/supervised_dispnet_amd/csrc/dn_pointwise.hip
+++ b/supervised_dispnet_amd/csrc/dn_pointwise.hip
@@ -1,4 +1,4 @@
-#include "dn_device.h"
+#include "dn_bn_bwd.h"
 #include "dn_fold.h"
 
 namespace dn {
@@ -403,14 +403,6 @@
   }
 }
 
-__device__ __forceinline__ float bn_bwd_value(float z, float yv, float mu, float is, float ga, float dg, float db, float inv_count) {
-#pragma clang fp contract(off)
-  const float xhat = (yv - mu) * is;
-  float t = __builtin_fmaf(-db, inv_count, z);
-  t = __builtin_fmaf(-(xhat * dg), inv_count, t);
-  return (ga * is) * t;
-}
-
 __global__ void __launch_bounds__(kThreads) bn_bwd_apply_kernel(float* __restrict__ dz_dy, const float* __restrict__ y,
                                                                 const float* __restrict__ mean, const float* __restrict__ invstd,
                                                                 const float* __restrict__ gamma, const float* __restrict__ dgamma,
@@ -451,7 +443,7 @@
                 db = *reinterpret_cast<const f32x4*>(dbeta + c);
 #pragma unroll
     for (int e = 0; e < 4; ++e) {
-      const float z = (yv[e] * sc[e] + sh[e] > 0.f) ? dz[e] : 0.f;
+      const float z = bn_relu_mask(yv[e], sc[e], sh[e]) ? dz[e] : 0.f;
       dz[e] = bn_bwd_value(z, yv[e], mu[e], is[e], ga[e], dg[e], db[e], inv_count);
     }
     *reinterpret_cast<f32x4*>(da_dy + o) = dz;
@@ -487,7 +479,7 @@
       if (i < total) {
 #pragma unroll
         for (int e = 0; e < 4; ++e) {
-          const float z = (yv[u][e] * sc[e] + sh[e] > 0.f) ? dz[u][e] : 0.f;
+          const float z = bn_relu_mask(yv[u][e], sc[e], sh[e]) ? dz[u][e] : 0.f;
           dz[u][e] = bn_bwd_value(z, yv[u][e], mu[e], is[e], ga[e], dg[e], db[e], inv_count);
         }
         *reinterpret_cast<f32x4*>(da_dy + i * 4) = dz[u];
@@ -1023,6 +1015,15 @@
   return DN_OK;
 }
 
+int dn_bn_bwd_sums_finalize(const float* partial, int32_t partial_rows, int32_t partial_stride, int32_t partial_offset, int32_t C,
+                            float* dgamma, float* dbeta, dn_stream_t stream) {
+  DN_REQUIRE(partial, DN_ERR_BAD_ARG, "dn_bn_bwd_sums_finalize: bad argument");
+  int rc = bn_bwd_sums_to_params(partial, partial_rows, partial_stride, partial_offset, C, dgamma, dbeta, as_stream(stream),
+                                 "dn_bn_bwd_sums_finalize");
+  if (rc != DN_OK) return rc;
+  return check_launch("bn_bwd_sums_finalize");
+}
+
 int dn_bn_bwd_apply_relu(float* da_dy, const float* y, const float* scale, const float* shift, const float* mean, const float* invstd,
                          const float* gamma, const float* partial, int32_t partial_rows, int32_t partial_stride, int32_t partial_offset,
                          int64_t rows, int32_t C, float* dgamma, float* dbeta, dn_stream_t stream) {
diff --git a/supervised_dispnet_amd/engine.py b/supervised_dispnet_amd/engine.py
--- a/supervised_dispnet_amd/engine.py
+++ b/supervised_dispnet_amd/engine.py
@@ -320,7 +320,7 @@
 class Act:
     __slots__ = ("t", "N", "H", "W", "C", "scale", "shift", "mean", "invstd", "grad", "grad_is_dz", "partial",
                  "partial_rows", "partial_stride", "partial_offset", "needs_grad", "strides", "no_relu", "planar", "pool_src", "sums_ready",
-                 "recip_t", "bn_owner", "sums_final", "seed_borrow", "grad_borrowed")
+                 "recip_t", "bn_owner", "sums_final", "seed_borrow", "grad_borrowed", "grad_writers")
 
     def __init__(self, t, N, H, W, C, strides=None, needs_grad=True):
         self.t = t
@@ -340,6 +340,7 @@
         self.sums_final = None
         self.seed_borrow = False
         self.grad_borrowed = False
+        self.grad_writers = 0
         self.needs_grad = needs_grad
         self.strides = strides or (H * W * C, W * C, C, 1)
 
@@ -654,22 +655,56 @@
     return y, partial, rows
 
 
-def conv_wgrad(layer, pieces, dy, out_hw, out=None, sink=None, first=None):
+class BnBwdPending:
+    __slots__ = ("g", "y", "bn", "dgamma", "dbeta", "sink")
+
+    def __init__(self, g, y, bn, dgamma, dbeta, sink):
+        self.g, self.y, self.bn, self.dgamma, self.dbeta, self.sink = g, y, bn, dgamma, dbeta, sink
+
+    def double(self):
+        y, d = self.y, torch.float64
+        yv, g = y.t.to(d), self.g.to(d)
+        z = torch.where(yv * y.scale.to(d) + y.shift.to(d) > 0, g, torch.zeros_like(g))
+        xhat = (yv - y.mean.to(d)) * y.invstd.to(d)
+        inv = 1.0 / y.rows
+        return (self.bn.weight.detach().to(d) * y.invstd.to(d)) * (z - self.dbeta.to(d) * inv - xhat * self.dgamma.to(d) * inv)
+
+
+def _wgrad_desc(layer, pieces, out_hw, bnb=None):
     a0 = pieces[0].act
     IH = a0.H * (2 if pieces[0].up else 1)
     IW = a0.W * (2 if pieces[0].up else 1)
     OH, OW = out_hw
-    kind = CONVT_FWD if layer.transposed else CONV_FWD
-    d = layer._desc(kind, a0.N, IH, IW, OH, OW)
+    d = layer._desc(CONVT_FWD if layer.transposed else CONV_FWD, a0.N, IH, IW, OH, OW)
     d.n_in = len(pieces)
     for i, p in enumerate(pieces):
         _fill_operand(d.in_[i], p)
     d.n_out = 1
     d.out[0].C = layer.Cout
+    if bnb is not None:
+        y, bn, dgamma, dbeta = bnb[:4]
+        d.bnb_y, d.bnb_scale, d.bnb_shift = y.t.data_ptr(), y.scale.data_ptr(), y.shift.data_ptr()
+        d.bnb_mean, d.bnb_invstd, d.bnb_gamma = y.mean.data_ptr(), y.invstd.data_ptr(), bn.weight.data_ptr()
+        d.bnb_dgamma = dgamma.data_ptr() if dgamma is not None else None
+        d.bnb_dbeta = dbeta.data_ptr() if dbeta is not None else None
+    return d
+
+
+def conv_wgrad(layer, pieces, dy, out_hw, out=None, sink=None, first=None):
+    bnb = None
+    if isinstance(dy, BnBwdPending):
+        bnb, dy = dy, dy.g
+    a0 = pieces[0].act
+    IH = a0.H * (2 if pieces[0].up else 1)
+    IW = a0.W * (2 if pieces[0].up else 1)
+    OH, OW = out_hw
+    d = _wgrad_desc(layer, pieces, out_hw, (bnb.y, bnb.bn, bnb.dgamma, bnb.dbeta) if bnb is not None else None)
     lib = _lib.load()
     nbytes = lib.dn_conv_wgrad_workspace_bytes(C.byref(d))
     if nbytes == 0:
         raise _lib.DispnetHipError("dn_conv_wgrad_workspace_bytes: " + _lib.last_error())
+    if bnb is not None and lib.dn_conv_wgrad_applies_bn_bwd(C.byref(d)) != 1:
+        raise _lib.DispnetHipError("conv_wgrad: the weight gradient of this layer does not apply the BatchNorm backward")
 
     def launch():
         ws = torch.empty(nbytes // 4, dtype=torch.float32, device=dy.device)
@@ -680,6 +715,9 @@
                                                              layer.Cin, layer.Cout, a0.N, IH, IW),
                     4 * (sum(p.act.rows * p.act.C for p in pieces) + dy.numel())):
             _lib.call("dn_conv2d_wgrad", C.byref(d), dy.data_ptr(), dw.data_ptr(), ws.data_ptr(), nbytes, _stream())
+        if bnb is not None:
+            bnb.sink.put(bnb.bn.weight, bnb.dgamma)
+            bnb.sink.put(bnb.bn.bias, bnb.dbeta)
         if sink is not None:
             sink.put(layer.m.weight, dw)
         return dw
@@ -707,6 +745,10 @@
         if p.act.scale is not None:
             cross_stream_use(p.act.scale, side)
             cross_stream_use(p.act.shift, side)
+    if bnb is not None:
+        y = bnb.y
+        for t in (y.t, y.scale, y.shift, y.mean, y.invstd, bnb.dgamma, bnb.dbeta):
+            cross_stream_use(t, side)
     if out is None:
         cross_stream_use(dw, main)
     return dw
@@ -748,6 +790,7 @@
             else:
                 a.sums_ready = False
                 a.sums_final = None
+            a.grad_writers = 1 if first else a.grad_writers + 1
             _fill_result(d.out[i], a.grad, a.C, IH, IW, not first)
     d.w_packed = layer.packed(kind, d).data_ptr()
     d.bias = None
@@ -800,11 +843,13 @@
                 first = a.grad is None
                 if first:
                     a.grad = a.new_like()
+                a.grad_writers = 1 if first else a.grad_writers + 1
                 _lib.call("dn_reflect_fold", tmp.data_ptr(), N, IH, IW, a.C, rp, a.grad.data_ptr(), 0 if first else 1, _stream())
                 continue
         first = a.grad is None
         if first:
             a.grad = a.new_like()
+        a.grad_writers = 1 if first else a.grad_writers + 1
         if a.C == 1:
             _lib.call("dn_upsample2x_nearest_bwd", cur.data_ptr(), N, a.H, a.W, a.grad.data_ptr(), 0 if first else 1, _stream())
         else:
@@ -880,7 +925,7 @@
         return self.grads.get(id(param))
 
 
-def bn_backward(y, bn, sink, training):
+def bn_backward(y, bn, sink, training, defer_apply=None):
     g, y_t, Cn, dev = y.grad, y.t, y.C, y.t.device
     if not training:
         raise NotImplementedError("backward through eval-mode BatchNorm (frozen statistics) is not implemented")
@@ -913,6 +958,12 @@
             dgamma = torch.empty(Cn, dtype=torch.float32, device=dev)
         if dbeta is None:
             dbeta = torch.empty(Cn, dtype=torch.float32, device=dev)
+    if (defer_apply is not None and y.pool_src is None and relu_pending and not BN_MATERIALIZE_DZ and y.grad_writers == 1
+            and not y.grad_borrowed and defer_apply(y)):
+        if final is None:
+            _lib.call("dn_bn_bwd_sums_finalize", y.partial.data_ptr(), y.partial_rows, y.partial_stride, y.partial_offset, Cn,
+                      dgamma.data_ptr(), dbeta.data_ptr(), _stream())
+        return BnBwdPending(g, y, bn, dgamma, dbeta, sink)
     if y.pool_src is not None:
         dpooled, pidx = y.pool_src
         hbm_call("dn::bn_bwd_apply_pool_kernel", y.rows * Cn * 8 + y.rows * Cn * 5 // 4, "dn_bn_bwd_apply_pool", dpooled.data_ptr(),
@@ -981,11 +1032,16 @@
     def backward():
         if y.grad is None:
             return
-        g = bn_backward(y, bn, sink, training)
+        if not xa.needs_grad:
+            g = bn_backward(y, bn, sink, training, defer_apply=lambda ya: _lib.load().dn_conv_wgrad_applies_bn_bwd(
+                C.byref(_wgrad_desc(layer, [x_piece], (OH, OW), (ya, bn, None, None)))) == 1)
+        else:
+            g = bn_backward(y, bn, sink, training)
         if layer.m.bias is not None:
             sink.put_zero(layer.m.bias)
         conv_wgrad(layer, [x_piece], g, (OH, OW), out=sink.dest(layer.m.weight), sink=sink)
-        conv_dgrad(layer, g, xa.N, OH, OW, [x_piece], (xa.H, xa.W))
+        if xa.needs_grad:
+            conv_dgrad(layer, g, xa.N, OH, OW, [x_piece], (xa.H, xa.W))
         y.grad = None
 
     tape.push(backward)
```

Result: no change. 2056 (median of 6 runs) (+0.2%).
